# Godotcoffee/AlignGraph2

Measured on AMD Instinct MI355X. Metric: aligned-read-bases/sec through PAGraph build+traverse, higher is better.
Workload: dtype u32

## Files before the change

### aligngraph2_amd/csrc/hip/k5_walk_aux.hip

```cpp
#include <algorithm>
#include <cmath>
#include <cstring>
#include <string>
#include <vector>

#include "pag_device.hpp"
#include "pag_travel.hpp"
#include "trav_device.hpp"
#include "trav_hook.hpp"

namespace pagdev {


__global__ void k_ranges(TravGraph G, TravContig *ctgs, uint32_t n) {
    uint32_t i = blockIdx.x * blockDim.x + threadIdx.x;
    if (i >= n) return;
    auto lower = [&](uint32_t x) {
        uint64_t lo = 0, hi = G.n_pos;
        while (lo < hi) {
            uint64_t mid = (lo + hi) >> 1;
            if ((uint32_t)(G.upos[mid] >> 32) < x) lo = mid + 1;
            else hi = mid;
        }
        return (uint32_t)lo;
// ... 176 lines not shown
    const uint32_t j = blockIdx.y;
    if (j >= n) return;
    const TravPackDesc D = descs[j];
    uint32_t *o = out + D.off;
    const uint32_t lane = lane_id();
    const uint64_t n_arrays = D.seq_x ? 5 : 3;
    uint32_t *agg = o + n_arrays * D.len;
    uint32_t *xagg = agg + ((D.len + 63) / 64) * 5;
    for (uint64_t i0 = (uint64_t)blockIdx.x * blockDim.x + (threadIdx.x & ~63u); i0 < D.len; i0 += (uint64_t)gridDim.x * blockDim.x) {
        const uint64_t i = i0 + lane;
        const bool valid = i < D.len;
        uint32_t v = 0, st = 0, c = 0, xl = 0, xh = 0;
        if (valid) {
            v = D.seq_v[i];
            st = D.seq_s[i];
            c = (uint32_t)(G.upos[v] >> 32);
            o[i] = v;
            o[D.len + i] = st;
            o[2 * D.len + i] = c;
            if (D.seq_x) {
                const uint64_t x = D.seq_x[i];
                xl = (uint32_t)x;
                xh = (uint32_t)(x >> 32);
                o[3 * D.len + i] = xl;
                o[4 * D.len + i] = xh;
            }
        }
        const uint32_t mx = wave_max_u32(valid ? c : 0u);
        const uint32_t m0 = wave_max_u32(valid && c == 0u ? v + 1u : 0u);
        const uint32_t lo = wave_min_u32(valid ? c : 0xFFFFFFFFu);
        const uint32_t lnz = wave_min_u32(valid && c != 0u ? c : 0xFFFFFFFFu);
        const uint32_t sum = wave_sum(valid ? st : 0u);
        const uint64_t blk = i0 >> 6;
        if (lane == 0) {
            uint32_t *a = agg + blk * 5;
            a[0] = mx;
            a[1] = m0;
            a[2] = lo;
            a[3] = lnz;
            a[4] = sum;
        }
        if (D.seq_x) {
            const bool bd = valid && (xh >> 31) != 0u;
            const uint32_t elow = wave_min_u32(bd ? (xh & 0x7FFFFFFFu) : 0xFFFFFFFFu);
            const uint32_t xm0 = wave_min_u32(bd ? xl : 0xFFFFFFFFu);
            if (lane == 0) {
                xagg[blk * 2] = elow;
                xagg[blk * 2 + 1] = xm0;
            }
        }
    }
}

__global__ void k_gather_pc(TravGraph G, const uint32_t *__restrict__ seq_v, uint64_t len, uint32_t *__restrict__ out) {
    for (uint64_t i = (uint64_t)blockIdx.x * blockDim.x + threadIdx.x; i < len; i += (uint64_t)gridDim.x * blockDim.x)
        out[i] = (uint32_t)(G.upos[seq_v[i]] >> 32);
}

__global__ void k_commit(const uint32_t *__restrict__ seq_v, uint64_t len, uint32_t in_lo, uint32_t in_hi, uint32_t *gbits,
                         uint32_t *gset, uint32_t gmask) {
    for (uint64_t i = (uint64_t)blockIdx.x * blockDim.x + threadIdx.x; i < len; i += (uint64_t)gridDim.x * blockDim.x) {
        uint32_t u = seq_v[i];
        if (u >= in_lo && u < in_hi) atomicOr(&gbits[(u - in_lo) >> 5], 1u << ((u - in_lo) & 31u));
        else hs_insert(gset, gmask, u);
    }
}

__global__ void k_gather_path(TravGraph G, const uint32_t *__restrict__ seq_v, const uint32_t *__restrict__ seq_s, uint64_t len,
                              pag_path_node *__restrict__ out) {
    for (uint64_t i = (uint64_t)blockIdx.x * blockDim.x + threadIdx.x; i < len; i += (uint64_t)gridDim.x * blockDim.x) {
        uint32_t v = G.uold[seq_v[i]];
        uint64_t p = G.vpos[v];
        pag_path_node o;
        o.code = G.ncode[G.vnode[v]];
        o.ctg = (uint32_t)(p >> 32);
        o.ref = (uint32_t)p;
        o.cnt = G.vcnt[v];
        o.reserved = 0;
        o.step = (int32_t)seq_s[i];
        o.vid = v;
        out[i] = o;
    }
}

__global__ void k_gather_vertices(TravGraph G, const uint32_t *__restrict__ vids, uint32_t n, pag_path_node *__restrict__ out) {
    uint32_t i = blockIdx.x * blockDim.x + threadIdx.x;
    if (i >= n) return;
    uint32_t v = vids[i];
    uint64_t p = G.vpos[v];
    pag_path_node o;
    o.code = G.ncode[G.vnode[v]];
    o.ctg = (uint32_t)(p >> 32);
    o.ref = (uint32_t)p;
    o.cnt = G.vcnt[v];
    o.reserved = 0;
    o.step = 0;
    o.vid = v;
    out[i] = o;
}

void trav_launch_seed_first(TravGraph G, const TravContig *ctgs, uint32_t n, uint64_t dev, uint32_t *out, uint32_t stride,
                            hipStream_t s) {
    if (n) k_seed_first<<<dim3(n), dim3(64), 0, s>>>(G, ctgs, n, dev, out, stride);
}
void trav_launch_seed_window(TravGraph G, const TravContig *ctgs, const TravSeedReq *reqs, uint32_t n, uint64_t dev,
                             uint32_t *out, uint32_t stride, hipStream_t s) {
    if (n) k_seed_window<<<dim3(n, TRAV_SEED_PARTS), dim3(64), 0, s>>>(G, ctgs, reqs, n, dev, out, stride);
}
void trav_launch_checkpoints(TravGraph G, const TravContig *ctgs, const TravSeedReq *reqs, uint32_t n, uint64_t dev, uint32_t *out,
                             hipStream_t s) {
    if (n) k_checkpoints<<<dim3(n), dim3(64), 0, s>>>(G, ctgs, reqs, n, dev, out);
}
void trav_launch_id_bounds(TravGraph G, const uint32_t *coords, uint32_t n, uint32_t *out, hipStream_t s) {
    if (n) k_id_bounds<<<dim3((n + 63) / 64), dim3(64), 0, s>>>(G, coords, n, out);
}
void trav_launch_pack_paths(TravGraph G, const TravPackDesc *descs, uint32_t n, uint64_t max_len, uint32_t *out, hipStream_t s) {
    if (!n) return;
    const unsigned gx = (unsigned)std::min<uint64_t>(std::max<uint64_t>((max_len + 255) / 256, 1), 64);
    k_pack_paths<<<dim3(gx, n), dim3(256), 0, s>>>(G, descs, n, out);
}
void trav_launch_gather_pc(TravGraph G, const uint32_t *seq_v, uint64_t len, uint32_t *out, hipStream_t s) {
    if (len) k_gather_pc<<<dim3(grid_for(len)), dim3(256), 0, s>>>(G, seq_v, len, out);
}
void trav_launch_commit(const uint32_t *seq_v, uint64_t len, uint32_t in_lo, uint32_t in_hi, uint32_t *gbits, uint32_t *gset,
                        uint32_t gmask, hipStream_t s) {
    if (len) k_commit<<<dim3(grid_for(len)), dim3(256), 0, s>>>(seq_v, len, in_lo, in_hi, gbits, gset, gmask);
}
void trav_launch_ranges(TravGraph G, TravContig *ctgs, uint32_t n, hipStream_t s) {
    if (n) k_ranges<<<dim3((n + 63) / 64), dim3(64), 0, s>>>(G, ctgs, n);
}

__global__ void k_clear_ranges(const TravClear *__restrict__ ranges) {
    const TravClear c = ranges[blockIdx.y];
    uint8_t *p = as_global((uint8_t *)c.p);
    const uint64_t head = (16u - ((uintptr_t)p & 15u)) & 15u, h = head < c.bytes ? head : c.bytes;
    const uint64_t n16 = (c.bytes - h) >> 4, tail = (c.bytes - h) & 15u;
    uint4 *q = (uint4 *)(p + h);
    const uint4 w = make_uint4(c.word, c.word, c.word, c.word);
    for (uint64_t i = (uint64_t)blockIdx.x * blockDim.x + threadIdx.x; i < n16; i += (uint64_t)gridDim.x * blockDim.x) q[i] = w;
    if (blockIdx.x == 0) {
        auto byte_at = [&](const uint8_t *a) { return (uint8_t)(c.word >> (8u * (uint32_t)((uintptr_t)a & 3u))); };
        if (threadIdx.x < h) p[threadIdx.x] = byte_at(p + threadIdx.x);
        if (threadIdx.x < tail) p[h + (n16 << 4) + threadIdx.x] = byte_at(p + h + (n16 << 4) + threadIdx.x);
    }
}
int trav_clear_ranges(const TravClear *ranges_dev, size_t n, hipStream_t s) {
    for (size_t at = 0; at < n; at += 32768) {
        const uint32_t m = (uint32_t)std::min<size_t>(32768, n - at);
        k_clear_ranges<<<dim3(32, m), dim3(256), 0, s>>>(ranges_dev + at);
    }
    PAG_HIP_TRY(hipGetLastError());
    return PAG_OK;
}
void trav_launch_gather_path(TravGraph G, const uint32_t *seq_v, const uint32_t *seq_s, uint64_t len, pag_path_node *out,
                             hipStream_t s, unsigned max_blocks) {
    const unsigned grid = max_blocks ? std::min(grid_for(len), max_blocks) : grid_for(len);
    if (len) k_gather_path<<<dim3(grid), dim3(256), 0, s>>>(G, seq_v, seq_s, len, out);
}
__global__ void __launch_bounds__(256) k_concat_parts(const TravConcatPart *__restrict__ parts, uint32_t *__restrict__ out_v,
                                                      uint32_t *__restrict__ out_s, uint32_t first_step) {
    const TravConcatPart P = parts[blockIdx.y];
    for (uint64_t x = (uint64_t)blockIdx.x * blockDim.x + threadIdx.x; x < P.n; x += (uint64_t)gridDim.x * blockDim.x) {
        out_v[P.start + x] = P.v[x];
        out_s[P.start + x] = (P.start + x == 0) ? first_step : P.s[x];
    }
}
void trav_launch_concat_parts(const TravConcatPart *parts, uint32_t n_parts, uint32_t *out_v, uint32_t *out_s, uint32_t first_step,
                              hipStream_t s) {
    for (uint32_t at = 0; at < n_parts; at += 32768) {
        const uint32_t n = std::min<uint32_t>(32768, n_parts - at);
        k_concat_parts<<<dim3(16, n), dim3(256), 0, s>>>(parts + at, out_v, out_s, first_step);
    }
}
void trav_launch_gather_vertices(TravGraph G, const uint32_t *vids, uint32_t n, pag_path_node *out, hipStream_t s) {
    if (n) k_gather_vertices<<<dim3((n + 255) / 256), dim3(256), 0, s>>>(G, vids, n, out);
}

}

using namespace pagdev;

namespace {
int hook_contigs(const pag_debug_trav_contig *ctgs, uint32_t n_ctgs, uint64_t n_graph_nodes, const uint32_t *nodes, uint64_t n_node_words,
                 uint64_t n_gbits, const uint32_t *gset, uint64_t n_gset, const uint32_t *d_nodes, uint32_t *d_gbits, uint32_t *d_gset,
                 std::vector<TravContig> &tc) {
    if (n_ctgs && !ctgs) return PAG_EINVAL;
    for (uint64_t i = 0; i < n_node_words; ++i)
        if (nodes[i] != PAG_NONE && nodes[i] >= n_graph_nodes) return PAG_EINVAL;
    tc.assign(n_ctgs, TravContig{});
    for (uint32_t i = 0; i < n_ctgs; ++i) {
        const pag_debug_trav_contig &m = ctgs[i];
        TravContig &t = tc[i];
        if (m.n_kmers && (m.nodes_off > n_node_words || m.n_kmers > n_node_words - m.nodes_off)) return PAG_EINVAL;
        if (m.g_hi < m.g_lo || m.in_hi < m.in_lo) return PAG_EINVAL;
        t.nodes = d_nodes + m.nodes_off;
        t.n_kmers = m.n_kmers;
        t.ctg_left = m.ctg_left;
        t.ctg_right = m.ctg_right;
        t.in_lo = m.in_lo;
        t.in_hi = m.in_hi;
        t.g_lo = m.g_lo;
        t.g_hi = m.g_hi;
        t.gmask = m.gmask;
        if (m.gbits_off != PAG_DEBUG_NULL) {
            const uint64_t words = ((uint64_t)(m.g_hi - m.g_lo) + 31) / 32;
            if (m.gbits_off > n_gbits || words > n_gbits - m.gbits_off) return PAG_EINVAL;
            t.gbits = d_gbits + m.gbits_off;
        }
        if (m.gset_off != PAG_DEBUG_NULL) {
            const uint64_t cap = (uint64_t)m.gmask + 1;
            if ((cap & (cap - 1)) || m.gset_off > n_gset || cap > n_gset - m.gset_off) return PAG_EINVAL;
            bool free_slot = false;
            for (uint64_t x = 0; x < cap && !free_slot; ++x) free_slot = gset[m.gset_off + x] == HS_EMPTY;
            if (!free_slot) return PAG_EINVAL;
            t.gset = d_gset + m.gset_off;
        }
    }
    return PAG_OK;
}
}

extern "C" int pag_debug_trav_bounds(const pag_debug_trav_graph *g, const uint32_t *coords, uint32_t n, uint32_t *out, pag_debug_trav_contig *ctgs,
                                     uint32_t n_ctgs, int device) {
    if (!g || (g->n_pos && !g->upos) || (n && (!coords || !out)) || (n_ctgs && !ctgs)) return PAG_EINVAL;
    HookDev D;
    TravGraph G;
    int rc;
    if ((rc = D.open(device)) || (rc = hook_upload_graph(D, g, &G))) return rc;
    uint32_t *d_coords = nullptr, *d_out = nullptr;
    TravContig *d_tc = nullptr;
    std::vector<TravContig> tc(n_ctgs, TravContig{});
    for (uint32_t i = 0; i < n_ctgs; ++i) {
        tc[i].ctg_left = ctgs[i].ctg_left;
        tc[i].ctg_right = ctgs[i].ctg_right;
        tc[i].in_lo = ctgs[i].in_lo;
        tc[i].in_hi = ctgs[i].in_hi;
        tc[i].g_lo = ctgs[i].g_lo;
        tc[i].g_hi = ctgs[i].g_hi;
    }
    if ((rc = D.up(coords, n, &d_coords)) || (rc = D.up((const uint32_t *)out, n, &d_out)) || (rc = D.up((const TravContig *)tc.data(), n_ctgs, &d_tc))) return rc;
    trav_launch_id_bounds(G, d_coords, n, d_out, D.s);
    trav_launch_ranges(G, d_tc, n_ctgs, D.s);
    if ((rc = D.down(out, d_out, n)) || (rc = D.down(tc.data(), d_tc, n_ctgs)) || (rc = D.finish())) return rc;
    for (uint32_t i = 0; i < n_ctgs; ++i) {
        ctgs[i].in_lo = tc[i].in_lo;
        ctgs[i].in_hi = tc[i].in_hi;
        ctgs[i].g_lo = tc[i].g_lo;
        ctgs[i].g_hi = tc[i].g_hi;
    }
    return PAG_OK;
}

extern "C" int pag_debug_trav_seeds(const pag_debug_trav_graph *g, int which, const pag_debug_trav_contig *ctgs, uint32_t n_ctgs, const uint32_t *nodes,
                                    uint64_t n_node_words, const uint32_t *gbits, uint64_t n_gbits, const uint32_t *gset, uint64_t n_gset,
                                    const uint64_t *reqs, uint32_t n_req, uint64_t dev, uint32_t *out, uint64_t out_words, uint32_t stride, int device) {
    if (!g || which < 0 || which > 2 || !g->npos_off || (g->n_pos && (!g->vpos || !g->newid || !g->vcnt)) || (n_node_words && !nodes) ||
        (n_gbits && !gbits) || (n_gset && !gset) || !out)
        return PAG_EINVAL;
    const uint64_t need = which == 0 ? (uint64_t)n_ctgs * stride : which == 1 ? (uint64_t)n_req * TRAV_SEED_PARTS * stride : 3ull * n_req;
    if ((which != 2 && stride < 2) || out_words < need || (which != 0 && n_req && !reqs)) return PAG_EINVAL;
    std::vector<TravSeedReq> rq(which == 0 ? 0 : n_req);
    for (size_t r = 0; r < rq.size(); ++r) {
        if (reqs[4 * r] >= n_ctgs) return PAG_EINVAL;
        rq[r].ctg = (uint32_t)reqs[4 * r];
        rq[r].pad = 0;
        rq[r].left = reqs[4 * r + 1];
        rq[r].right = reqs[4 * r + 2];
        rq[r].pos = reqs[4 * r + 3];
    }
    HookDev D;
    TravGraph G;
    int rc;
    if ((rc = D.open(device)) || (rc = hook_upload_graph(D, g, &G))) return rc;
    uint32_t *d_nodes = nullptr, *d_gbits = nullptr, *d_gset = nullptr, *d_out = nullptr;
    TravContig *d_tc = nullptr;
    TravSeedReq *d_rq = nullptr;
    if ((rc = D.up(nodes, n_node_words, &d_nodes)) || (rc = D.up(gbits, n_gbits, &d_gbits)) || (rc = D.up(gset, n_gset, &d_gset)) ||
        (rc = D.up((const uint32_t *)out, out_words, &d_out)))
        return rc;
    std::vector<TravContig> tc;
    if ((rc = hook_contigs(ctgs, n_ctgs, g->n_nodes, nodes, n_node_words, n_gbits, gset, n_gset, d_nodes, d_gbits, d_gset, tc))) return rc;
    if ((rc = D.up((const TravContig *)tc.data(), n_ctgs, &d_tc)) || (rc = D.up((const TravSeedReq *)rq.data(), rq.size(), &d_rq))) return rc;
    if (which == 0) trav_launch_seed_first(G, d_tc, n_ctgs, dev, d_out, stride, D.s);
    else if (which == 1) trav_launch_seed_window(G, d_tc, d_rq, n_req, dev, d_out, stride, D.s);
    else trav_launch_checkpoints(G, d_tc, d_rq, n_req, dev, d_out, D.s);
    if ((rc = D.down(out, d_out, out_words))) return rc;
    return D.finish();
}

extern "C" int pag_debug_pack_paths(const pag_debug_trav_graph *g, const uint32_t *seq_v, const uint32_t *seq_s, const uint64_t *seq_x, uint64_t n_seq,
                                    const uint64_t *descs, uint32_t n, uint64_t max_len, uint32_t *out, uint64_t out_words, int device) {
    if (!g || !g->upos || (n_seq && (!seq_v || !seq_s)) || (n && !descs) || !out || n > 65535u) return PAG_EINVAL;
    for (uint64_t i = 0; i < n_seq; ++i)
        if (seq_v[i] >= g->n_pos) return PAG_EINVAL;
    for (uint32_t j = 0; j < n; ++j) {
        const uint64_t from = descs[4 * j], len = descs[4 * j + 1], off = descs[4 * j + 2];
        const bool leap = descs[4 * j + 3] != 0;
        if (from > n_seq || len > n_seq - from || len > max_len || (leap && !seq_x)) return PAG_EINVAL;
        if (off > out_words || trav_pack_words(len, leap) > out_words - off) return PAG_EINVAL;
    }
    HookDev D;
    TravGraph G;
    int rc;
    if ((rc = D.open(device)) || (rc = hook_upload_graph(D, g, &G))) return rc;
    uint32_t *d_v = nullptr, *d_s = nullptr, *d_out = nullptr;
    uint64_t *d_x = nullptr;
// ... 114 lines not shown
```

### aligngraph2_amd/csrc/hip/pag_api.hip

```cpp
#include <algorithm>
#include <cstdlib>
#include <cstring>
#include <new>
#include <string>
#include <thread>
#include <chrono>
#include <vector>

#include "pag_device.hpp"
#include "pagraph_debug.h"

using namespace pagdev;

#include "pag_graph_impl.hpp"
#include "walker_grid.hpp"

namespace {

template <typename T>
int stage(const T *src, uint64_t n, bool on_device, DevBuf &own, const T **out, hipStream_t s) {
    if (on_device) {
        *out = src;
        return PAG_OK;
    }
// ... 62 lines not shown
    if (threadIdx.x < 16) h[threadIdx.x] = 0;
    __syncthreads();
    for (uint64_t i = (uint64_t)blockIdx.x * blockDim.x + threadIdx.x; i < n; i += (uint64_t)gridDim.x * blockDim.x)
        atomicAdd(&h[((key[i] >> shift) & 7u) * 2u + (i < n1 ? 0u : 1u)], 1u);
    __syncthreads();
    if (threadIdx.x < 16 && h[threadIdx.x]) atomicAdd(&out[threadIdx.x], (unsigned long long)h[threadIdx.x]);
}

__global__ void edge_counts(const uint32_t *__restrict__ samples, uint64_t n, uint32_t *__restrict__ out) {
    uint64_t i = (uint64_t)blockIdx.x * blockDim.x + threadIdx.x;
    if (i < n) out[i] = samples[i] ? samples[i] - 1u : 0u;
}

}

extern "C" {

const char *pag_last_error(void) { return last_error(); }

int pag_device_available(void) { return pick_device(0) == PAG_OK ? 1 : 0; }

namespace {
__global__ void k_warm(uint32_t *p) {
    if (p) *p = 1u;
}
}
int pag_device_warm(int device_ordinal) {
    int rc = pick_device(device_ordinal);
    if (rc != PAG_OK) return rc;
    uint32_t *p = nullptr;
    if (hipMalloc((void **)&p, 256) != hipSuccess) return PAG_ENOMEM;
    k_warm<<<dim3(1), dim3(64)>>>(p);
    hipError_t e = hipDeviceSynchronize();
    hipFree(p);
    if (e != hipSuccess) {
        set_error("pag_device_warm: %s", hipGetErrorString(e));
        return PAG_EFAULT;
    }
    return PAG_OK;
}

pag_graph *pag_create(const uint64_t *codes, uint64_t n_codes, uint32_t k, int device_ordinal, int *err) {
    int rc = PAG_OK;
    pag_graph *g = nullptr;
    if (k == 0 || k > 16 || (!codes && n_codes)) {
        set_error("pag_create: k must be in 1..16 (got %u)", k);
        rc = PAG_EINVAL;
    }
    if (rc == PAG_OK) rc = pick_device(device_ordinal);
    if (rc == PAG_OK) {
        g = new (std::nothrow) pag_graph();
        if (!g) rc = PAG_ENOMEM;
    }
    if (rc == PAG_OK) {
        g->device = device_ordinal;
        g->k = k;
        const uint64_t space = 1ull << (2 * k);
        const uint64_t words = (space + 31) / 32;
        std::vector<uint32_t> bits((size_t)words, 0u);
        std::vector<uint64_t> outside;
        {
            unsigned T = std::max(1u, std::min(16u, std::thread::hardware_concurrency()));
            if (n_codes < (1u << 20)) T = 1;
            std::vector<std::vector<uint64_t>> out_t(T);
            auto work = [&](unsigned t) {
                const uint64_t lo = n_codes * t / T, hi = n_codes * (t + 1) / T;
                for (uint64_t i = lo; i < hi; ++i) {
                    const uint64_t c = codes[i];
                    if (c < space) __atomic_fetch_or(&bits[(size_t)(c >> 5)], 1u << (c & 31), __ATOMIC_RELAXED);
                    else out_t[t].push_back(c);
                }
            };
            std::vector<std::thread> pool;
            for (unsigned t = 1; t < T; ++t) pool.emplace_back(work, t);
            work(0);
            for (auto &th : pool) th.join();
            for (auto &v : out_t) outside.insert(outside.end(), v.begin(), v.end());
        }
        std::sort(outside.begin(), outside.end());
        outside.erase(std::unique(outside.begin(), outside.end()), outside.end());
        uint64_t in_space = 0;
        for (uint32_t wbits : bits) in_space += (uint64_t)__builtin_popcount(wbits);
        g->n_solid = in_space + outside.size();
        g->all_solid = in_space == space;
        hipError_t e = hipStreamCreate(&g->stream);
        if (e == hipSuccess) e = hipMalloc((void **)&g->solid_bits, (size_t)words * 4 + 64);
        if (e == hipSuccess) e = hipMemcpy(g->solid_bits, bits.data(), (size_t)words * 4, hipMemcpyHostToDevice);
        if (e != hipSuccess) {
            set_error("pag_create: %s", hipGetErrorString(e));
            rc = PAG_EFAULT;
        }
    }
    if (rc != PAG_OK && g) {
        pag_destroy(g);
        g = nullptr;
    }
    if (err) *err = rc;
    return g;
}

pag_graph *pag_create_from_bitmap(const uint32_t *bits, uint64_t n_solid, uint32_t k, int bits_on_device,
                                  int device_ordinal, int *err) {
    int rc = PAG_OK;
    pag_graph *g = nullptr;
    if (k == 0 || k > 16 || !bits) {
        set_error("pag_create_from_bitmap: k must be in 1..16 and bits non-null");
        rc = PAG_EINVAL;
    }
    if (rc == PAG_OK) rc = pick_device(device_ordinal);
    if (rc == PAG_OK) {
        g = new (std::nothrow) pag_graph();
        if (!g) rc = PAG_ENOMEM;
    }
    if (rc == PAG_OK) {
        g->device = device_ordinal;
        g->k = k;
        g->n_solid = n_solid;
        const uint64_t space = 1ull << (2 * k);
        const uint64_t words = (space + 31) / 32;
        g->all_solid = n_solid == space;
        hipError_t e = hipStreamCreate(&g->stream);
        if (e == hipSuccess) e = hipMalloc((void **)&g->solid_bits, (size_t)words * 4 + 64);
        if (e == hipSuccess)
            e = hipMemcpy(g->solid_bits, bits, (size_t)words * 4, bits_on_device ? hipMemcpyDeviceToDevice : hipMemcpyHostToDevice);
        if (e != hipSuccess) {
            set_error("pag_create_from_bitmap: %s", hipGetErrorString(e));
            rc = PAG_EFAULT;
        }
    }
    if (rc != PAG_OK && g) {
        pag_destroy(g);
        g = nullptr;
    }
    if (err) *err = rc;
    return g;
}

void pag_destroy(pag_graph *g) {
    if (!g) return;
    hipSetDevice(g->device);
    free_graph_results(g);
    for (auto &sl : g->pool)
        if (sl.p) hipFree(sl.p);
    for (auto &sl : g->cpool)
        if (sl.p) hipFree(sl.p);
    for (void *q : g->deferred) hipFree(q);
    if (g->wq_host) hipHostFree(g->wq_host);
    if (g->path_store) hipHostFree(g->path_store);
    if (g->deliver_stream) hipStreamDestroy(g->deliver_stream);
    if (g->pin_host) hipHostFree(g->pin_host);
    for (void *q : g->fetch_chunks) hipHostFree(q);
    g->fetch_chunks.clear();
    g->fetch_chunk_bytes.clear();
    if (g->walk_arena) hipFree(g->walk_arena);
    if (g->dump_tables) hipFree(g->dump_tables);
    if (g->dump_scratch) hipFree(g->dump_scratch);
    if (g->wq_next) hipFree(g->wq_next);
    for (hipStream_t ws : g->walk_streams) hipStreamDestroy(ws);
    if (g->solid_bits) hipFree(g->solid_bits);
    if (g->stream) hipStreamDestroy(g->stream);
    delete g;
}

uint64_t pag_solid_count(const pag_graph *g) { return g ? g->n_solid : 0; }

int pag_reset(pag_graph *g) {
    if (!g) return PAG_EINVAL;
    hipSetDevice(g->device);
    free_graph_results(g);
    g->stats = pag_build_stats{};
    return PAG_OK;
}

}

namespace {

struct Extracted {
    uint64_t T = 0, E = 0, T1 = 0, E1 = 0;
};

struct StreamBufs {
    DevBuf tk0, tv0, tk1, tv1, ek0, ev0, ek1, ev1, sorttmp;
    explicit StreamBufs(pag_graph *g)
        : tk0(g, ps::TK0), tv0(g, ps::TV0), tk1(g, ps::TK1), tv1(g, ps::TV1), ek0(g, ps::EK0), ev0(g, ps::EV0), ek1(g, ps::EK1), ev1(g, ps::EV1),
          sorttmp(g, ps::SORT_TMP) {}
    int alloc(uint64_t T, uint64_t E) {
        int rc;
        if ((rc = tk0.alloc((T + 1) * 4)) || (rc = tv0.alloc((T + 1) * 8)) || (rc = ek0.alloc((E + 1) * 4)) || (rc = ev0.alloc((E + 1) * 8)) ||
            (rc = tk1.alloc((T + 1) * 4)) || (rc = tv1.alloc((T + 1) * 12)) || (rc = ek1.alloc((E + 1) * 4)) || (rc = ev1.alloc((E + 1) * 12)))
            return rc;
        return sorttmp.alloc(sort_tmp_bytes(std::max(T, E)));
    }
};

int extract_stage(pag_graph *g, const pag_build_input *in, uint64_t emit_lo, uint64_t emit_hi, Extracted *out, hipEvent_t ev_begin,
                  hipEvent_t ev_end) {
    hipStream_t s = g->stream;
    const bool dev = in->on_device != 0;
    const uint32_t n_reads_all = (uint32_t)in->reads.n_seqs;
    const uint32_t n_reads = (uint32_t)(emit_hi - emit_lo);
    const uint64_t n_jobs = 4ull * n_reads;
    int rc;
    if (ev_begin) PAG_HIP_TRY(hipEventRecord(ev_begin, s));

    DevBuf b_roff(g, ps::IN_ROFF), b_rlen(g, ps::IN_RLEN), b_packed(g, ps::IN_PACKED), b_order(g, ps::IN_ORDER), b_aln1(g, ps::IN_ALN1), b_q1(g, ps::IN_Q1),
        b_d1(g, ps::IN_D1), b_aln2(g, ps::IN_ALN2), b_q2(g, ps::IN_Q2), b_d2(g, ps::IN_D2), b_ctg(g, ps::IN_CTG), b_eoff(g, ps::IN_EOFF), b_ent(g, ps::IN_ENT),
        b_ref(g, ps::IN_REF);
    const uint64_t *d_roff;
    const uint32_t *d_rlen, *d_order, *d_d1, *d_d2, *d_eoff, *d_ent;
    const uint8_t *d_packed;
    const pag_aln *d_aln1, *d_aln2;
    const uint64_t *d_q1, *d_q2;
    const pag_ctg *d_ctg;
    const pag_ref *d_ref;
    if ((rc = stage(in->reads.byte_off, n_reads_all, dev, b_roff, &d_roff, s))) return rc;
    if ((rc = stage(in->reads.len, n_reads_all, dev, b_rlen, &d_rlen, s))) return rc;
    if ((rc = stage(in->reads.packed, in->reads.packed_bytes, dev, b_packed, &d_packed, s))) return rc;
    if ((rc = stage(in->emit_order, n_reads_all, dev, b_order, &d_order, s))) return rc;
    if ((rc = stage(in->read_to_ctg.aln, in->read_to_ctg.n_aln, dev, b_aln1, &d_aln1, s))) return rc;
    if ((rc = stage(in->read_to_ctg.query_off, (uint64_t)n_reads_all + 1, dev, b_q1, &d_q1, s))) return rc;
    if ((rc = stage(in->read_to_ctg.diff, in->read_to_ctg.n_diff_words, dev, b_d1, &d_d1, s))) return rc;
    if ((rc = stage(in->read_to_ref.aln, in->read_to_ref.n_aln, dev, b_aln2, &d_aln2, s))) return rc;
    if ((rc = stage(in->read_to_ref.query_off, (uint64_t)n_reads_all + 1, dev, b_q2, &d_q2, s))) return rc;
    if ((rc = stage(in->read_to_ref.diff, in->read_to_ref.n_diff_words, dev, b_d2, &d_d2, s))) return rc;
    if ((rc = stage(in->ctgs, in->n_ctgs, dev, b_ctg, &d_ctg, s))) return rc;
    if ((rc = stage(in->ctg_ent_off, in->n_ctg_ent_off, dev, b_eoff, &d_eoff, s))) return rc;
    if ((rc = stage(in->ctg_ent, in->n_ctg_ent, dev, b_ent, &d_ent, s))) return rc;
    if ((rc = stage(in->refs, in->n_refs, dev, b_ref, &d_ref, s))) return rc;
    d_order += emit_lo;

    std::vector<pag_ref> refs_host((size_t)in->n_refs);
    if (in->n_refs) {
        if (dev) PAG_HIP_TRY(hipMemcpy(refs_host.data(), in->refs, in->n_refs * sizeof(pag_ref), hipMemcpyDeviceToHost));
        else std::memcpy(refs_host.data(), in->refs, in->n_refs * sizeof(pag_ref));
    }

    const uint64_t n_aln1 = in->read_to_ctg.n_aln, n_aln2 = in->read_to_ref.n_aln;
    DevBuf b_covok(g, ps::COV_OK), b_covtmp(g, ps::COV_TMP);
    if ((rc = b_covok.alloc(n_aln2 + 16))) return rc;
    size_t cov_bytes = cov_tmp_bytes(refs_host.data(), in->n_refs);
    if ((rc = b_covtmp.alloc(cov_bytes))) return rc;
    if ((rc = launch_cov_filter(d_aln2, n_aln2, d_ref, refs_host.data(), in->n_refs, in->cov_filter,
                                b_covok.as<uint8_t>(), b_covtmp.p, cov_bytes, s)))
        return rc;

    DevBuf b_cc(g, ps::CI_CC), b_cio1(g, ps::CI_OFF1), b_cio2(g, ps::CI_OFF2), b_ci1(g, ps::CI_1), b_ci2(g, ps::CI_2), b_scan(g, ps::X_SCAN), b_tot(g, ps::X_TOT);
    uint64_t n_alnmax = std::max(n_aln1, n_aln2);
    if ((rc = b_cc.alloc((n_alnmax + 1) * 4))) return rc;
    if ((rc = b_cio1.alloc((n_aln1 + 1) * 8))) return rc;
    if ((rc = b_cio2.alloc((n_aln2 + 1) * 8))) return rc;
    if ((rc = b_scan.alloc(scan_tmp_bytes(std::max<uint64_t>(n_alnmax, n_jobs) + 1)))) return rc;
    if ((rc = b_tot.alloc(64))) return rc;
    uint64_t *d_tot = b_tot.as<uint64_t>();
    uint64_t n_ci[2] = {0, 0};
    for (int pass = 0; pass < 2; ++pass) {
        const pag_aln *al = pass == 0 ? d_aln1 : d_aln2;
        uint64_t na = pass == 0 ? n_aln1 : n_aln2;
        DevBuf &off = pass == 0 ? b_cio1 : b_cio2;
        if (na) {
            chunk_counts<<<dim3((unsigned)((na + 255) / 256)), dim3(256), 0, s>>>(al, na, b_cc.as<uint32_t>());
            if ((rc = scan_u32_to_u64(b_cc.as<uint32_t>(), off.as<uint64_t>(), na, d_tot + pass, b_scan.p, s))) return rc;
            PAG_HIP_TRY(hipMemcpyAsync(&n_ci[pass], d_tot + pass, 8, hipMemcpyDeviceToHost, s));
        }
    }
    PAG_HIP_TRY(hipStreamSynchronize(s));
    for (int pass = 0; pass < 2; ++pass) {
        const pag_aln *al = pass == 0 ? d_aln1 : d_aln2;
        uint64_t na = pass == 0 ? n_aln1 : n_aln2;
        DevBuf &off = pass == 0 ? b_cio1 : b_cio2;
        DevBuf &ci = pass == 0 ? b_ci1 : b_ci2;
        if ((rc = ci.alloc((n_ci[pass] + 1) * sizeof(uint2)))) return rc;
        if ((rc = launch_colidx(al, na, pass == 0 ? d_d1 : d_d2, off.as<uint64_t>(), ci.as<uint2>(), s))) return rc;
    }

    DevBuf b_js(g, ps::K1_JS), b_jt(g, ps::K1_JT), b_je(g, ps::K1_JE), b_toff(g, ps::K1_TOFF), b_eoff2(g, ps::K1_EOFF);
    if ((rc = b_js.alloc((n_jobs + 1) * 4))) return rc;
    if ((rc = b_jt.alloc((n_jobs + 1) * 4))) return rc;
    if ((rc = b_je.alloc((n_jobs + 1) * 4))) return rc;
    if ((rc = b_toff.alloc((n_jobs + 1) * 8))) return rc;
    if ((rc = b_eoff2.alloc((n_jobs + 1) * 8))) return rc;
    DevBuf b_smask(g, ps::SOLID_MASK);
    if (!g->all_solid) {
        if ((rc = b_smask.alloc((in->reads.packed_bytes / 4 + 16) * 2 * sizeof(uint16_t) * solid_mask_slices()))) return rc;
    }
    ExtractArgs xa[2];
    for (int pass = 0; pass < 2; ++pass) {
        ExtractArgs &a = xa[pass];
        a = ExtractArgs{};
        a.read_off = d_roff;
        a.read_len = d_rlen;
        a.packed = d_packed;
        a.emit_order = d_order;
        a.n_reads = n_reads;
        a.aln = pass == 0 ? d_aln1 : d_aln2;
        a.query_off = pass == 0 ? d_q1 : d_q2;
        a.diff = pass == 0 ? d_d1 : d_d2;
        a.colidx_off = (pass == 0 ? b_cio1 : b_cio2).as<uint64_t>();
        a.colidx = (pass == 0 ? b_ci1 : b_ci2).as<uint2>();
        a.cov_ok = pass == 0 ? nullptr : b_covok.as<uint8_t>();
        a.pass = pass;
        a.topk = pass == 0 ? in->topk_ctg : in->topk_ref;
        a.ctgs = d_ctg;
        a.ctg_ent_off = d_eoff;
        a.ctg_ent = d_ent;
        a.refs = d_ref;
        a.solid_bits = g->solid_bits;
// ... 104 lines not shown
        return rc;
    PAG_HIP_TRY(hipEventRecord(ev[2], s));
    EdgeOut eo{b_eseg.as<uint32_t>(), ctr_dev + 4};
    if ((rc = launch_edges(ek->as<uint32_t>(), evb->as<uint64_t>(), e_scratch, E, eo, b_long.as<uint64_t>(),
                           b_lcnt.as<uint32_t>(), s, wide)))
        return rc;
    uint64_t ctr[8] = {0, 0, 0, 0, 0, 0, 0, 0};
    PAG_HIP_TRY(hipMemcpyAsync(ctr, b_ctr.p, 64, hipMemcpyDeviceToHost, s));
    PAG_HIP_TRY(hipEventRecord(ev[3], s));
    PAG_HIP_TRY(hipStreamSynchronize(s));

    pag_build_stats st{};
    const uint64_t T2 = T - T1, E2 = E - E1;
    const uint64_t L_ctg = ctr[0], L_all = ctr[1], U_all = ctr[4], U_1 = ctr[5];
    st.n_tuples[0] = T1;
    st.n_tuples[1] = T2;
    st.n_edges[0] = E1;
    st.n_edges[1] = E2;
    st.merge_edge[0] = E1 - U_1;
    st.total_pos[0] = T1;
    st.merge_pos[0] = T1 - L_ctg;
    st.merge_edge[1] = U_1 + E2 - U_all;
    st.total_pos[1] = L_ctg + T2;
    st.merge_pos[1] = L_ctg + T2 - L_all;
    st.n_nodes = ctr[2];
    st.n_pos = L_all;
    st.n_uniq_edges = U_all;
    float ms = 0.f;
    hipEventElapsedTime(&ms, ev[0], ev[1]);
    st.ms_sort = ms;
    hipEventElapsedTime(&ms, ev[1], ev[2]);
    st.ms_cluster = ms;
    hipEventElapsedTime(&ms, ev[2], ev[3]);
    st.ms_edges = ms;
    st.ms_sort_kernel = ms_scatter_t;
    st.sort_records = T;
    (void)passes;
    (void)ms_scatter_e;

    g->n_t = T;
    g->n_e = E;
    g->tkey = tk->as<uint32_t>();
    g->tval = tv->as<uint64_t>();
    g->tseg = b_tseg.as<uint32_t>();
    g->tcnt = b_tcnt.as<uint16_t>();
    g->ekey = ek->as<uint32_t>();
    g->eval = evb->as<uint64_t>();
    g->eseg = b_eseg.as<uint32_t>();
    g->stats = st;
    *st_out = st;
    return PAG_OK;
}

struct EventSet {
    hipEvent_t e[6] = {nullptr, nullptr, nullptr, nullptr, nullptr, nullptr};
    int create() {
        for (auto &x : e) PAG_HIP_TRY(hipEventCreate(&x));
        return PAG_OK;
    }
    ~EventSet() {
        for (auto x : e)
            if (x) hipEventDestroy(x);
    }
};

void keep_debug_streams(pag_graph *g, uint64_t T, uint64_t E) {
    const char *keep = std::getenv("PAG_DEBUG_KEEP_STREAMS");
    g->dbg_tkey.clear();
    g->dbg_tval.clear();
    g->dbg_ekey.clear();
    g->dbg_eval.clear();
    if (!(keep && keep[0] == '1')) return;
    g->dbg_tkey.resize((size_t)T);
    g->dbg_tval.resize((size_t)T);
    g->dbg_ekey.resize((size_t)E);
    g->dbg_eval.resize((size_t)E);
    hipStreamSynchronize(g->stream);
    const StreamPtrs x = streams_at(g, 1, 1);
    if (T) hipMemcpy(g->dbg_tkey.data(), x.tkey, T * 4, hipMemcpyDeviceToHost);
    if (T) hipMemcpy(g->dbg_tval.data(), x.tval, T * 8, hipMemcpyDeviceToHost);
    if (E) hipMemcpy(g->dbg_ekey.data(), x.ekey, E * 4, hipMemcpyDeviceToHost);
    if (E) hipMemcpy(g->dbg_eval.data(), x.eval, E * 8, hipMemcpyDeviceToHost);
}

int check_process_args(const pag_graph *g, const pag_build_input *in) {
    if (!g || !in) return PAG_EINVAL;
    if (in->outer_sample < 1 || in->outer_sample > 7) {
        set_error("outer_sample must be 1..7");
        return PAG_EINVAL;
    }
    if (in->reads.n_seqs >= 0x3FFFFFFFull) {
        set_error("too many reads for one launch");
        return PAG_EINVAL;
    }
    return PAG_OK;
}

}

extern "C" {

int pag_process(pag_graph *g, const pag_build_input *in, pag_build_stats *stats) {
    int rc = check_process_args(g, in);
    if (rc != PAG_OK) return rc;
    const bool timing = env_timing();
    const auto wall0 = std::chrono::steady_clock::now();
    auto wall_ms = [&]() { return std::chrono::duration<double, std::milli>(std::chrono::steady_clock::now() - wall0).count(); };
    PAG_HIP_TRY(hipSetDevice(g->device));
    free_graph_results(g);
    EventSet ev;
    if ((rc = ev.create())) return rc;
    Extracted x;
    if ((rc = extract_stage(g, in, 0, in->reads.n_seqs, &x, ev.e[0], ev.e[1]))) return rc;
    keep_debug_streams(g, x.T, x.E);
    pag_build_stats st{};
    if ((rc = build_stage(g, in->eps, x, &st, ev.e + 2))) return rc;
    float ms = 0.f;
    hipEventElapsedTime(&ms, ev.e[0], ev.e[1]);
    st.ms_extract = ms;
    hipEventElapsedTime(&ms, ev.e[0], ev.e[5]);
    st.ms_total = ms;
    if (timing) fprintf(stderr, "[timing] pag_process wall %.1f ms (device %.1f ms)\n", wall_ms(), (double)ms);
    g->stats = st;
    if (stats) *stats = st;
    return PAG_OK;
}

extern "C" int pag_reserve_walk_arena(pag_graph *g, uint64_t contig_bases) {
    if (!g) return PAG_EINVAL;
    PAG_HIP_TRY(hipSetDevice(g->device));
    size_t want = (size_t)contig_bases * 1200 + (64u << 20);
    size_t free_b = 0, total_b = 0;
    const size_t sharers = env_device_sharers();
    if (hipMemGetInfo(&free_b, &total_b) == hipSuccess) want = std::min(want, (free_b + g->walk_arena_cap) * 2 / 5 / sharers);
    {
        const size_t FETCH_CHUNK = 64u << 20;
        size_t have = 0;
        for (size_t b : g->fetch_chunk_bytes) have += b;
        const size_t per_base = 14 + (env_int("PAGRAPH_DEVICE_DUMPS", 0) == 1 ? 22 : 0) + (env_int("PAGRAPH_DEVICE_SEQS", 0) == 1 ? 2 : 0);
        const size_t want_pinned = std::min<size_t>((size_t)contig_bases * per_base, (size_t)4 << 30);
        while (have < want_pinned) {
            void *q = nullptr;
            if (hipHostMalloc(&q, FETCH_CHUNK, hipHostMallocDefault) != hipSuccess) {
                (void)hipGetLastError();
                break;
            }
            g->fetch_chunks.push_back(q);
            g->fetch_chunk_bytes.push_back(FETCH_CHUNK);
            have += FETCH_CHUNK;
        }
    }
    pagdev::WalkerGrid::prepare_streams(g, 4);
    if (g->walk_arena_cap >= want) return PAG_OK;
    if (g->walk_arena) hipFree(g->walk_arena);
    g->walk_arena = nullptr;
    g->walk_arena_cap = 0;
    if (hipMalloc(&g->walk_arena, want) != hipSuccess) {
        g->walk_arena = nullptr;
        (void)hipGetLastError();
        return PAG_OK;
    }
    g->walk_arena_cap = want;
    return PAG_OK;
}

static int log2_shards(uint32_t n) { return n == 1 ? 0 : n == 2 ? 1 : n == 4 ? 2 : n == 8 ? 3 : -1; }

int pag_shard_extract(pag_graph *g, const pag_build_input *in, uint32_t shard, uint32_t n_shards, uint64_t *counts) {
    int rc = check_process_args(g, in);
    if (rc != PAG_OK) return rc;
    if (log2_shards(n_shards) < 0 || shard >= n_shards) {
        set_error("pag_shard_extract: n_shards must be 1, 2, 4 or 8 (got %u) and shard below it", n_shards);
        return PAG_EINVAL;
    }
    const uint64_t n = in->reads.n_seqs;
    return pag_shard_extract_range(g, in, n * shard / n_shards, n * (shard + 1ull) / n_shards, n_shards, counts);
}

int pag_shard_extract_range(pag_graph *g, const pag_build_input *in, uint64_t lo, uint64_t hi, uint32_t n_shards, uint64_t *counts) {
    int rc = check_process_args(g, in);
    if (rc != PAG_OK) return rc;
    const int lg = log2_shards(n_shards);
    if (lg < 0 || !counts || 2 * (int)g->k < lg || lo > hi || hi > in->reads.n_seqs) {
        set_error("pag_shard_extract_range: n_shards must be 1, 2, 4 or 8 (got %u), the reads [%llu, %llu) of %llu", n_shards, (unsigned long long)lo,
                  (unsigned long long)hi, (unsigned long long)in->reads.n_seqs);
        return PAG_EINVAL;
    }
    PAG_HIP_TRY(hipSetDevice(g->device));
    free_graph_results(g);
    hipStream_t s = g->stream;
    Extracted x;
    if ((rc = extract_stage(g, in, lo, hi, &x, nullptr, nullptr))) return rc;
    keep_debug_streams(g, x.T, x.E);
    g->shard_x[0] = x.T;
    g->shard_x[1] = x.E;
    g->shard_in0[0] = g->shard_in0[1] = 1;
    for (uint32_t i = 0; i < 4 * n_shards; ++i) counts[i] = 0;
    if (n_shards == 1) {
        counts[0] = x.T1;
        counts[1] = x.T - x.T1;
        counts[2] = x.E1;
        counts[3] = x.E - x.E1;
        return PAG_OK;
    }
    const int shift = 2 * (int)g->k - lg;
    StreamBufs sb(g);
    DevBuf b_ctr(g, ps::CTR);
    if ((rc = sb.alloc(x.T, x.E)) || (rc = b_ctr.alloc(512))) return rc;
    unsigned long long *ctr = b_ctr.as<unsigned long long>();
    PAG_HIP_TRY(hipMemsetAsync(ctr, 0, 256, s));
    if (x.T) owner_counts<<<dim3(1024), dim3(256), 0, s>>>(sb.tk0.as<uint32_t>(), x.T, x.T1, shift, ctr);
    if (x.E) owner_counts<<<dim3(1024), dim3(256), 0, s>>>(sb.ek0.as<uint32_t>(), x.E, x.E1, shift, ctr + 16);
    int t_in0 = 1, e_in0 = 1;
    if ((rc = sort_pairs(sb.tk0.as<uint32_t>(), sb.tv0.as<uint64_t>(), sb.tk1.as<uint32_t>(), sb.tv1.as<uint64_t>(), x.T, lg, sb.sorttmp.p, &t_in0, s, nullptr,
                         nullptr, shift)))
        return rc;
    if ((rc = sort_pairs(sb.ek0.as<uint32_t>(), sb.ev0.as<uint64_t>(), sb.ek1.as<uint32_t>(), sb.ev1.as<uint64_t>(), x.E, lg, sb.sorttmp.p, &e_in0, s, nullptr,
                         nullptr, shift)))
        return rc;
    unsigned long long h[32];
    PAG_HIP_TRY(hipMemcpyAsync(h, ctr, 256, hipMemcpyDeviceToHost, s));
    PAG_HIP_TRY(hipStreamSynchronize(s));
    for (uint32_t o = 0; o < n_shards; ++o) {
        counts[4 * o + 0] = h[2 * o];
        counts[4 * o + 1] = h[2 * o + 1];
        counts[4 * o + 2] = h[16 + 2 * o];
        counts[4 * o + 3] = h[16 + 2 * o + 1];
    }
    g->shard_in0[0] = t_in0;
    g->shard_in0[1] = e_in0;
    return PAG_OK;
}

int pag_shard_extract_for(pag_graph *g, const pag_build_input *in, uint64_t lo, uint64_t hi, uint32_t n_shards, uint32_t owner, uint32_t *tkey,
                          uint64_t *tval, uint64_t t_cap, uint64_t t_at1, uint64_t t_at2, uint32_t *ekey, uint64_t *eval, uint64_t e_cap,
                          uint64_t e_at1, uint64_t e_at2, uint64_t *counts) {
    int rc = check_process_args(g, in);
    if (rc != PAG_OK) return rc;
    const int lg = log2_shards(n_shards);
    if (lg < 1 || owner >= n_shards || !counts || 2 * (int)g->k < lg || lo > hi || hi > in->reads.n_seqs) {
        set_error("pag_shard_extract_for: n_shards must be 2, 4 or 8 (got %u) and the owner below it (got %u), the reads [%llu, %llu) of %llu", n_shards,
                  owner, (unsigned long long)lo, (unsigned long long)hi, (unsigned long long)in->reads.n_seqs);
        return PAG_EINVAL;
    }
    PAG_HIP_TRY(hipSetDevice(g->device));
    free_graph_results(g);
    hipStream_t s = g->stream;
    Extracted x;
    if ((rc = extract_stage(g, in, lo, hi, &x, nullptr, nullptr))) return rc;
    g->shard_x[0] = x.T;
    g->shard_x[1] = x.E;
    g->shard_in0[0] = g->shard_in0[1] = 1;
    for (int q = 0; q < 4; ++q) counts[q] = 0;
    const uint32_t shift = (uint32_t)(2 * (int)g->k - lg);
    DevBuf b_tmp(g, ps::PICK_TMP);
    if ((rc = b_tmp.alloc(owner_pick_tmp_bytes(std::max(x.T, x.E))))) return rc;
    const StreamPtrs st = streams_at(g, 1, 1);
    if ((rc = owner_pick(st.tkey, st.tval, x.T, x.T1, shift, owner, tkey, tval, t_cap, t_at1, t_at2, counts, b_tmp.p, s))) return rc;
    if ((rc = owner_pick(st.ekey, st.eval, x.E, x.E1, shift, owner, ekey, eval, e_cap, e_at1, e_at2, counts + 2, b_tmp.p, s))) return rc;
    PAG_HIP_TRY(hipStreamSynchronize(s));
    return PAG_OK;
}

int pag_shard_take(pag_graph *g, uint32_t *tkey, uint64_t *tval, uint32_t *ekey, uint64_t *eval) {
    if (!g) return PAG_EINVAL;
    PAG_HIP_TRY(hipSetDevice(g->device));
    hipStream_t s = g->stream;
    const uint64_t T = g->shard_x[0], E = g->shard_x[1];
    const StreamPtrs x = streams_at(g, g->shard_in0[0], g->shard_in0[1]);
    if (T) PAG_HIP_TRY(hipMemcpyAsync(tkey, x.tkey, T * 4, hipMemcpyDeviceToDevice, s));
    if (T) PAG_HIP_TRY(hipMemcpyAsync(tval, x.tval, T * 8, hipMemcpyDeviceToDevice, s));
    if (E) PAG_HIP_TRY(hipMemcpyAsync(ekey, x.ekey, E * 4, hipMemcpyDeviceToDevice, s));
    if (E) PAG_HIP_TRY(hipMemcpyAsync(eval, x.eval, E * 8, hipMemcpyDeviceToDevice, s));
    PAG_HIP_TRY(hipStreamSynchronize(s));
    return PAG_OK;
}

int pag_shard_take_part(pag_graph *g, uint64_t t_off, uint64_t t_n, uint32_t *tkey, uint64_t *tval, uint64_t e_off, uint64_t e_n, uint32_t *ekey,
                        uint64_t *eval) {
    if (!g) return PAG_EINVAL;
    const uint64_t T = g->shard_x[0], E = g->shard_x[1];
    if (t_off > T || t_n > T - t_off || e_off > E || e_n > E - e_off || (t_n && (!tkey || !tval)) || (e_n && (!ekey || !eval))) {
        set_error("pag_shard_take_part: [%llu, +%llu) of %llu tuples, [%llu, +%llu) of %llu edges", (unsigned long long)t_off, (unsigned long long)t_n,
                  (unsigned long long)T, (unsigned long long)e_off, (unsigned long long)e_n, (unsigned long long)E);
        return PAG_EINVAL;
    }
    PAG_HIP_TRY(hipSetDevice(g->device));
    hipStream_t s = g->stream;
    const StreamPtrs x = streams_at(g, g->shard_in0[0], g->shard_in0[1]);
    if (t_n) PAG_HIP_TRY(hipMemcpyAsync(tkey, x.tkey + t_off, t_n * 4, hipMemcpyDeviceToDevice, s));
    if (t_n) PAG_HIP_TRY(hipMemcpyAsync(tval, x.tval + t_off, t_n * 8, hipMemcpyDeviceToDevice, s));
    if (e_n) PAG_HIP_TRY(hipMemcpyAsync(ekey, x.ekey + e_off, e_n * 4, hipMemcpyDeviceToDevice, s));
    if (e_n) PAG_HIP_TRY(hipMemcpyAsync(eval, x.eval + e_off, e_n * 8, hipMemcpyDeviceToDevice, s));
    PAG_HIP_TRY(hipStreamSynchronize(s));
    return PAG_OK;
}

int pag_shard_build(pag_graph *g, const uint32_t *tkey, const uint64_t *tval, uint64_t n_t, uint64_t t1, const uint32_t *ekey,
                    const uint64_t *eval, uint64_t n_e, uint64_t e1, uint32_t eps, pag_build_stats *stats) {
    if (!g || t1 > n_t || e1 > n_e || (n_t && (!tkey || !tval)) || (n_e && (!ekey || !eval))) return PAG_EINVAL;
    PAG_HIP_TRY(hipSetDevice(g->device));
    free_graph_results(g);
    hipStream_t s = g->stream;
    int rc;
    DevBuf b_tk0(g, ps::TK0), b_tv0(g, ps::TV0), b_ek0(g, ps::EK0), b_ev0(g, ps::EV0);
    if ((rc = b_tk0.alloc((n_t + 1) * 4)) || (rc = b_tv0.alloc((n_t + 1) * 8)) || (rc = b_ek0.alloc((n_e + 1) * 4)) || (rc = b_ev0.alloc((n_e + 1) * 8))) return rc;
    if (n_t) PAG_HIP_TRY(hipMemcpyAsync(b_tk0.p, tkey, n_t * 4, hipMemcpyDeviceToDevice, s));
    if (n_t) PAG_HIP_TRY(hipMemcpyAsync(b_tv0.p, tval, n_t * 8, hipMemcpyDeviceToDevice, s));
    if (n_e) PAG_HIP_TRY(hipMemcpyAsync(b_ek0.p, ekey, n_e * 4, hipMemcpyDeviceToDevice, s));
    if (n_e) PAG_HIP_TRY(hipMemcpyAsync(b_ev0.p, eval, n_e * 8, hipMemcpyDeviceToDevice, s));
    EventSet ev;
    if ((rc = ev.create())) return rc;
    Extracted x;
    x.T = n_t;
    x.E = n_e;
// ... 227 lines not shown
```

### aligngraph2_amd/csrc/hip/pag_graph_impl.hpp

```cpp
#pragma once
#include <algorithm>
#include <chrono>
#include <vector>

#include "pag_device.hpp"
#include "pag_travel.hpp"
#include "pool_slots.hpp"

struct pag_graph {
    int device = 0;
    hipStream_t stream = nullptr;
    uint32_t k = 0;
    uint64_t n_solid = 0;
    int all_solid = 0;
    uint32_t *solid_bits = nullptr;
    uint64_t n_t = 0, n_e = 0;
    uint32_t *tkey = nullptr;
    uint64_t *tval = nullptr;
    uint32_t *tseg = nullptr;
    uint16_t *tcnt = nullptr;
    uint32_t *ekey = nullptr;
    uint64_t *eval = nullptr;
    uint32_t *eseg = nullptr;
    pag_build_stats stats{};
    uint64_t shard_x[2] = {0, 0};
    int shard_in0[2] = {1, 1};
    struct SerialRun {
        bool valid = false;
        uint32_t n = 0;
        std::vector<uint64_t> counts;
        pag_build_stats total{};
    } serial;
    struct Slot {
        void *p = nullptr;
        size_t cap = 0;
    };
    Slot pool[pagdev::ps::COUNT];
    double alloc_ms = 0;
    uint64_t alloc_bytes = 0, alloc_calls = 0;
    std::vector<Slot> cpool;
    bool defer_free = false;
    std::vector<void *> deferred;
    void *wq_host = nullptr;
    size_t wq_bytes = 0;
    uint32_t *wq_next = nullptr;
    std::vector<hipStream_t> walk_streams;
    pagdev::TravGraph tg{};
    bool tg_ready = false;
    uint64_t tg_dev = 0;
    double tg_err = 0;
    pag_path_node *path_store = nullptr;
    size_t path_cap = 0;
    std::vector<uint64_t> path_off, path_len;
    hipStream_t deliver_stream = nullptr;
    std::vector<const pag_path_node *> path_ptr;
    std::vector<uint8_t> path_valid;
    std::vector<const char *> text_ptr;
    std::vector<uint64_t> text_len;
    std::vector<const char *> seq_ptr;
    std::vector<uint64_t> seq_len;
    const pag_seqs *seq_refs = nullptr;
    void *dump_tables = nullptr, *dump_scratch = nullptr;
    size_t dump_tables_cap = 0, dump_scratch_cap = 0;
    void *walk_arena = nullptr;
    size_t walk_arena_cap = 0, walk_arena_used = 0;
    std::vector<void *> fetch_chunks;
    std::vector<size_t> fetch_chunk_bytes;
    bool regional = false;
    std::vector<uint32_t> region_ref_iv;
    std::vector<uint8_t> region_ref_open;
    bool view_pruned = false, view_off = false;
    std::vector<int32_t> view_orient;
    uint64_t view_counts[3] = {0, 0, 0};
    uint64_t view_fallbacks = 0;
    double succ_per_vertex = 3.0;
    uint64_t n_zero_ctg = 0;
    void *pin_host = nullptr;
    size_t pin_bytes = 0;
    std::vector<uint32_t> dbg_tkey, dbg_ekey;
    std::vector<uint64_t> dbg_tval, dbg_eval;
};


namespace pagdev {

struct DevBuf {
    pag_graph *g = nullptr;
    pag_graph::Slot *sl = nullptr;
    void *p = nullptr;
    DevBuf() = default;
    DevBuf(pag_graph *gg, ps::Id s) : g(gg), sl(&gg->pool[s]) {}
    DevBuf(pag_graph *gg, pag_graph::Slot *slot) : g(gg), sl(slot) {}
    int alloc(size_t bytes) {
        if (bytes == 0) bytes = 16;
        if (sl->cap < bytes) {
            const auto t0 = std::chrono::steady_clock::now();
            if (sl->p) {
                if (g->defer_free) g->deferred.push_back(sl->p);
                else hipFree(sl->p);
            }
            sl->p = nullptr;
            sl->cap = 0;
            size_t want = bytes + std::min<size_t>(bytes / 8, (size_t)512 << 20) + 256;
            hipError_t e = hipMalloc(&sl->p, want);
            g->alloc_ms += std::chrono::duration<double, std::milli>(std::chrono::steady_clock::now() - t0).count();
            g->alloc_bytes += want;
            g->alloc_calls += 1;
            if (e != hipSuccess) {
                sl->p = nullptr;
                pagdev::set_error("hipMalloc(%zu) failed: %s", want, hipGetErrorString(e));
                return PAG_ENOMEM;
            }
            sl->cap = want;
        }
        p = sl->p;
        return PAG_OK;
    }
    template <typename T>
    T *as() const {
        return (T *)p;
    }
};


struct StreamPtrs {
    const uint32_t *tkey;
    const uint64_t *tval;
    const uint32_t *ekey;
    const uint64_t *eval;
};
inline StreamPtrs streams_at(const pag_graph *g, int t_in0, int e_in0) {
    return StreamPtrs{(const uint32_t *)g->pool[t_in0 ? ps::TK0 : ps::TK1].p, (const uint64_t *)g->pool[t_in0 ? ps::TV0 : ps::TV1].p,
                      (const uint32_t *)g->pool[e_in0 ? ps::EK0 : ps::EK1].p, (const uint64_t *)g->pool[e_in0 ? ps::EV0 : ps::EV1].p};
}

int shard_count_range(pag_graph *g, const pag_build_input *in, uint64_t lo, uint64_t hi, uint32_t n_shards, uint64_t *counts);

struct GraphArrays {
    void *p[ps::GRAPH_ARRS];
};
template <typename G>
GraphArrays arrays_of(const G &x) {
    return GraphArrays{{(void *)x.tkey, (void *)x.tval, (void *)x.tseg, (void *)x.tcnt, (void *)x.ekey, (void *)x.eval, (void *)x.eseg}};
}
template <typename G>
void point_at(G &x, const GraphArrays &a) {
    x.tkey = (decltype(x.tkey))a.p[ps::G_TKEY];
    x.tval = (decltype(x.tval))a.p[ps::G_TVAL];
    x.tseg = (decltype(x.tseg))a.p[ps::G_TSEG];
    x.tcnt = (decltype(x.tcnt))a.p[ps::G_TCNT];
    x.ekey = (decltype(x.ekey))a.p[ps::G_EKEY];
    x.eval = (decltype(x.eval))a.p[ps::G_EVAL];
    x.eseg = (decltype(x.eseg))a.p[ps::G_ESEG];
}
inline GraphArrays arrays_in(const pag_graph *g, ps::Id base) {
    GraphArrays a;
    for (int i = 0; i < ps::GRAPH_ARRS; ++i) a.p[i] = g->pool[ps::family(base, i)].p;
    return a;
}

}
```

### aligngraph2_amd/csrc/hip/pag_travel.hpp

```cpp
#pragma once
#include <hip/hip_runtime.h>
#include <stdint.h>

#include <vector>

#include "pagraph_hip.h"

namespace pagdev {

constexpr int TRAV_PROBE_GROUPS = 8;

struct TravGraph {
    uint64_t n_nodes, n_pos, n_edges;
    uint32_t *ncode;
    uint32_t *npos_off;
    uint32_t *nedge_off;
    uint64_t *vpos;
    uint16_t *vcnt;
    uint32_t *vnode;
    uint32_t *eto;
    uint32_t *estep;
    uint64_t *bitmap;
    uint32_t *rank;
    uint32_t *uold;
// ... 7 lines not shown
    uint32_t n_zero;
    const uint32_t *inc_iv;
    const uint8_t *inc_open;
    uint32_t inc_n, inc_margin;
};
constexpr uint32_t GRADE_POISON = 7u, GRADE_POISON_IF_LEAP = 6u;

struct alignas(16) SuccRec {
    uint32_t tgt;
    uint32_t pc;
    uint32_t meta;
    uint32_t toff;
};

struct TravContig {
    const uint32_t *nodes;
    uint32_t n_kmers;
    uint32_t ctg_left, ctg_right;
    uint32_t rev_left, rev_right;
    uint64_t split_size;
    double leap_min;
    const uint64_t *starts;
    const uint64_t *sizes;
    uint32_t n_ctgs;
    uint32_t in_lo, in_hi;
    uint32_t g_lo, g_hi;
    uint32_t *gbits;
    uint32_t *gset;
    uint32_t gmask;
    uint32_t gwin_lo, gwin_hi;
};

struct TravJob {
    uint32_t ctg;
    uint32_t start;
    uint64_t has_size;
    uint32_t *seq_v, *seq_s;
    uint64_t seq_cap;
    uint32_t *arena_v, *arena_s;
    uint64_t arena_cap;
    uint32_t *stamp;
    uint32_t stamp_stride;
    uint32_t *tbits;
    uint64_t *tset;
    uint32_t tmask;
    uint64_t *pset;
    uint32_t pmask;
    uint32_t exact;
    uint32_t mode;
    uint32_t stop_pc;
    uint64_t init_len;
    uint32_t win_low;
    uint32_t pad0;
    uint64_t *seq_x;
};
enum { TRAV_MODE_SPEC = 1, TRAV_MODE_RESUME = 2, TRAV_MODE_LEAP = 4, TRAV_MODE_UNTIL_LEAP = 8,
       TRAV_MODE_CANCELLED = 16 };

struct TravJobOut {
    uint64_t seq_len, seq_size;
    uint64_t n_classify, n_probe, n_records;
    uint32_t last_ctg;
    int overflow;
    uint64_t n_fill, n_out, n_main;
    uint32_t stopped;
    uint32_t max_back;
    uint32_t max_chosen;
    uint32_t wd_below_max;
    uint64_t max_probe;
    uint32_t wd_forced_min;
    uint32_t poison;
    uint64_t t_begin, t_end;
#ifdef PAG_WALK_PROF
    uint64_t prof_t[14];
    uint32_t prof_c[14];
#endif
};

struct TravPosted {
    TravJob J;
    TravContig C;
};
constexpr int TRAV_RINGS = 3;
struct TravQueue {
    uint32_t posted[TRAV_RINGS];
    uint32_t exit;
    uint32_t started, exited;
};

struct TravPackDesc {
    const uint32_t *seq_v, *seq_s;
    uint64_t len;
    uint64_t off;
    const uint64_t *seq_x;
};

inline uint64_t trav_pack_words(uint64_t len, bool leap) { return (leap ? 5 : 3) * len + ((len + 63) / 64) * (leap ? 7 : 5); }

constexpr uint32_t TRAV_SEED_PARTS = 16;

struct TravSeedReq {
    uint32_t ctg;
    uint32_t pad;
    uint64_t left, right, pos;
};

struct TravView {
    const uint32_t *civ, *riv;
    uint32_t n_civ, n_riv;
};
int trav_compact(const uint32_t *tkey, const uint64_t *tval, const uint32_t *tseg, const uint16_t *tcnt, uint64_t T,
                 const uint32_t *ekey, const uint64_t *eval, const uint32_t *eseg, uint64_t E, uint32_t k, uint64_t n_nodes,
                 uint64_t n_pos, uint64_t n_edges, TravGraph G, void *tmp, size_t tmp_bytes, hipStream_t s, const TravView *view = nullptr,
                 uint64_t *counts_out = nullptr);
int trav_zone_bands(const uint64_t *tval, uint64_t T, const uint32_t *zones_dev, uint32_t n_z, uint32_t *lo_dev, uint32_t *hi_dev, hipStream_t s);
size_t trav_compact_tmp_bytes(uint64_t T, uint64_t E, uint32_t k, uint64_t n_nodes);
struct TravCtgNodesJob {
    uint64_t byte_off;
    uint64_t out_off;
    uint32_t len;
    int32_t forward;
};
void trav_launch_ctg_nodes(const uint8_t *packed, const TravCtgNodesJob *jobs, uint32_t n_jobs, uint32_t max_len, uint32_t k, TravGraph G, uint32_t *out,
                           hipStream_t s);
void trav_launch_seed_first(TravGraph G, const TravContig *ctgs, uint32_t n, uint64_t dev, uint32_t *out, uint32_t stride,
                            hipStream_t s);
void trav_launch_seed_window(TravGraph G, const TravContig *ctgs, const TravSeedReq *reqs, uint32_t n, uint64_t dev,
                             uint32_t *out, uint32_t stride, hipStream_t s);
void trav_launch_checkpoints(TravGraph G, const TravContig *ctgs, const TravSeedReq *reqs, uint32_t n, uint64_t dev, uint32_t *out,
                             hipStream_t s);
void trav_launch_id_bounds(TravGraph G, const uint32_t *coords, uint32_t n, uint32_t *out, hipStream_t s);
void trav_launch_pack_paths(TravGraph G, const TravPackDesc *descs, uint32_t n, uint64_t max_len, uint32_t *out, hipStream_t s);
void trav_launch_gather_pc(TravGraph G, const uint32_t *seq_v, uint64_t len, uint32_t *out, hipStream_t s);
void trav_launch_walk(TravGraph G, const TravContig *ctgs, const TravJob *jobs, TravJobOut *outs, uint32_t n, uint32_t k,
                      hipStream_t s);
int trav_walk_waves_per_cu();
void trav_launch_walk_persistent(TravGraph G, const TravPosted *jobs, TravJobOut *outs, uint32_t *done, TravQueue *q,
                                 uint32_t *next, uint32_t cap, uint32_t k, uint32_t n_waves, uint64_t idle_ticks, hipStream_t s);
void trav_launch_commit(const uint32_t *seq_v, uint64_t len, uint32_t in_lo, uint32_t in_hi, uint32_t *gbits, uint32_t *gset,
                        uint32_t gmask, hipStream_t s);
void trav_launch_ranges(TravGraph G, TravContig *ctgs, uint32_t n, hipStream_t s);
int trav_mark_incomplete(TravGraph &G, uint32_t n_zero, const uint32_t *iv_host, const uint8_t *open_host, uint32_t n_iv, uint32_t dev, double err,
                         uint32_t *bits, void *tmp, hipStream_t s);
size_t trav_mark_incomplete_tmp_bytes(uint32_t n_iv);

int trav_order(TravGraph G, uint32_t *key, uint64_t *val, uint32_t *key2, uint64_t *val2, void *sort_tmp, uint64_t *n_zero, int ctg_bits,
               int ref_bits, hipStream_t s);
struct TravClear {
    void *p;
    uint64_t bytes;
    uint32_t word, pad;
};
int trav_clear_ranges(const TravClear *ranges_dev, size_t n, hipStream_t s);
int trav_successors_of(TravGraph G, uint32_t code, uint64_t pos, void *recs, uint64_t cap, unsigned long long *out, hipStream_t s);
constexpr uint32_t EMIT_CHUNK_SLOTS = 2048u, EMIT_GRID_THREADS = 2048u, EMIT_GRID_WAVES = 1024u;
constexpr uint64_t EMIT_SLACK_SLOTS = (uint64_t)(EMIT_GRID_THREADS + EMIT_GRID_WAVES) * 4u * EMIT_CHUNK_SLOTS;
int trav_succ_emit(TravGraph G, uint32_t dev, double err, uint32_t *key0, uint64_t *val0, uint32_t *key1, uint64_t *val1, uint64_t cap, void *sort_tmp,
                   unsigned long long *counters, uint32_t *heavy_list, uint32_t heavy_limit, uint64_t *n_slots, uint64_t *n_rec, uint64_t *n_heavy,
                   const uint32_t **sorted_key, const uint64_t **sorted_val, hipStream_t s);
int trav_succ_finish(TravGraph G, const uint32_t *key, const uint64_t *val, uint64_t n_rec, hipStream_t s);
void trav_launch_gather_path(TravGraph G, const uint32_t *seq_v, const uint32_t *seq_s, uint64_t len, pag_path_node *out,
                             hipStream_t s, unsigned max_blocks = 0);
void trav_launch_gather_vertices(TravGraph G, const uint32_t *vids, uint32_t n, pag_path_node *out, hipStream_t s);
struct TravConcatPart {
    const uint32_t *v, *s;
    uint64_t start, n;
};
void trav_launch_concat_parts(const TravConcatPart *parts, uint32_t n_parts, uint32_t *out_v, uint32_t *out_s, uint32_t first_step,
                              hipStream_t s);

size_t text_scratch_bytes(uint64_t n);
constexpr uint32_t DUMP_LDS_STARTS = 5632u, DUMP_MAX_SEQS = 99999999u;
struct DumpTables {
    const uint32_t *cstart, *csize, *rstart, *rsize;
    uint32_t nc, nr, in_lds;
};
#ifdef __HIPCC__
template <typename Starts>
__device__ __forceinline__ void single_to_dual(Starts starts, const uint32_t *__restrict__ sizes, uint32_t n, uint32_t single, int32_t *idx, int64_t *off) {
    if (single == 0u) {
        *idx = 0;
        *off = 0;
        return;
    }
    uint32_t lo = 0, hi = n ? n + 1u : 0u;
    while (lo < hi) {
        const uint32_t mid = (lo + hi) >> 1;
        if (starts[mid] <= single) lo = mid + 1u;
        else hi = mid;
    }
    const uint32_t i = lo ? lo - 1u : 0u;
    const int64_t start = n ? (int64_t)starts[i] : 0;
    const int64_t size2 = i < n ? 2 * (int64_t)sizes[i] : 0;
    int64_t o = (int64_t)single - start;
    if (o < 0 || o >= size2) {
        o -= size2;
        *idx = -(int32_t)(i + 1u);
    } else {
        *idx = (int32_t)(i + 1u);
    }
    *off = o;
}
#endif
bool dump_tables_build(const uint32_t *ctg_len, uint64_t n_ctgs, const uint32_t *ref_len, uint64_t n_refs, std::vector<uint32_t> &blob);
DumpTables dump_tables_at(const uint32_t *dev, uint64_t n_ctgs, uint64_t n_refs);
uint32_t dump_line_bound(uint32_t k, const std::vector<uint32_t> &blob, uint64_t n_ctgs, uint64_t n_refs);
int trav_launch_dump_path(TravGraph G, const uint32_t *seq_v, const uint32_t *seq_s, uint64_t len, uint32_t k, const DumpTables &T, void *scratch,
                          char *out, uint64_t cap, uint64_t *head_host, hipStream_t s, unsigned max_blocks);

struct SeqSources {
    const uint64_t *coff, *roff;
    const uint8_t *cpacked, *rpacked;
};
bool seqs_well_formed(const pag_seqs *q);
size_t seq_sources_bytes(const pag_seqs *ctgs, const pag_seqs *refs);
int seq_sources_upload(void *dev, const pag_seqs *ctgs, const pag_seqs *refs, SeqSources *out, hipStream_t s);
struct SeqParams {
    uint32_t k;
    uint64_t deviation;
    double error_rate;
};
int trav_launch_seq_path(TravGraph G, const uint32_t *seq_v, const uint32_t *seq_s, uint64_t len, const SeqParams &P, const DumpTables &T,
                         const SeqSources &S, void *scratch, char *out, uint64_t cap, uint64_t *head_host, hipStream_t s, unsigned max_blocks);

}
```

### aligngraph2_amd/csrc/hip/shard_serial.hip

```cpp
#include <algorithm>
#include <chrono>
#include <cstdio>
#include <cstring>
#include <vector>

#include "pag_graph_impl.hpp"
#include "pagraph_debug.h"
#include "serial_layout.hpp"

using namespace pagdev;

namespace {

double now_s() { return std::chrono::duration<double>(std::chrono::steady_clock::now().time_since_epoch()).count(); }

int grow_keeping(pag_graph *g, ps::Id id, size_t used, size_t need, size_t hint) {
    pag_graph::Slot &sl = g->pool[id];
    if (sl.p && sl.cap >= need) return PAG_OK;
    const auto t0 = std::chrono::steady_clock::now();
    const size_t want = std::max(need, hint) + 256;
    void *p = nullptr;
    hipError_t e = hipMalloc(&p, want);
    g->alloc_ms += std::chrono::duration<double, std::milli>(std::chrono::steady_clock::now() - t0).count();
    g->alloc_bytes += want;
    g->alloc_calls += 1;
    if (e != hipSuccess) {
        set_error("hipMalloc(%zu) failed: %s (a region of a serial-rank run)", want, hipGetErrorString(e));
        return PAG_ENOMEM;
    }
    if (used && sl.p) {
        e = hipMemcpyAsync(p, sl.p, used, hipMemcpyDeviceToDevice, g->stream);
        if (e == hipSuccess) e = hipStreamSynchronize(g->stream);
        if (e != hipSuccess) {
            hipFree(p);
            set_error("a region of a serial-rank run could not be moved: %s", hipGetErrorString(e));
            return PAG_EFAULT;
        }
    }
    if (sl.p) hipFree(sl.p);
    sl.p = p;
    sl.cap = want;
    return PAG_OK;
}

void free_slot(pag_graph::Slot &sl) {
    if (sl.p) hipFree(sl.p);
    sl.p = nullptr;
    sl.cap = 0;
}

void release_traversal(pag_graph *g) {
    hipStreamSynchronize(g->stream);
    g->tg_ready = false;
    for (int i = ps::TG_NCODE; i <= ps::WALK_SEQS; ++i) free_slot(g->pool[i]);
    if (g->walk_arena) hipFree(g->walk_arena);
    g->walk_arena = nullptr;
    g->walk_arena_cap = g->walk_arena_used = 0;
}

void release_build_keeping(pag_graph *g, const pag_build_input *in) {
    hipStreamSynchronize(g->stream);
    std::vector<const void *> keep;
    const GraphArrays held = arrays_of(*g);
    for (void *p : held.p) keep.push_back(p);
    if (in->on_device)
        for (const void *p : {(const void *)in->reads.byte_off, (const void *)in->reads.len, (const void *)in->reads.packed, (const void *)in->emit_order,
                              (const void *)in->read_to_ctg.aln, (const void *)in->read_to_ctg.query_off, (const void *)in->read_to_ctg.diff,
                              (const void *)in->read_to_ref.aln, (const void *)in->read_to_ref.query_off, (const void *)in->read_to_ref.diff,
                              (const void *)in->ctgs, (const void *)in->ctg_ent_off, (const void *)in->ctg_ent, (const void *)in->refs})
            keep.push_back(p);
    for (int i = 0; i < ps::COUNT; ++i) {
        pag_graph::Slot &sl = g->pool[i];
        if (!ps::released_after_import((ps::Id)i) || !sl.p) continue;
        const char *lo = (const char *)sl.p, *hi = lo + sl.cap;
        bool used = false;
        for (const void *p : keep) used = used || (p && (const char *)p >= lo && (const char *)p < hi);
        if (!used) free_slot(sl);
    }
}

void add_stats(pag_build_stats &st, const pag_build_stats &p) {
    for (int q = 0; q < 2; ++q) {
        st.merge_edge[q] += p.merge_edge[q];
        st.total_pos[q] += p.total_pos[q];
        st.merge_pos[q] += p.merge_pos[q];
        st.n_tuples[q] += p.n_tuples[q];
        st.n_edges[q] += p.n_edges[q];
    }
    st.n_nodes += p.n_nodes;
    st.n_pos += p.n_pos;
    st.n_uniq_edges += p.n_uniq_edges;
}

bool same_count_lines(const pag_build_stats &a, const pag_build_stats &b) {
    return !std::memcmp(a.merge_edge, b.merge_edge, sizeof a.merge_edge) && !std::memcmp(a.total_pos, b.total_pos, sizeof a.total_pos) &&
           !std::memcmp(a.merge_pos, b.merge_pos, sizeof a.merge_pos) && !std::memcmp(a.n_tuples, b.n_tuples, sizeof a.n_tuples) &&
           !std::memcmp(a.n_edges, b.n_edges, sizeof a.n_edges);
}

int serial_turn(pag_graph *g, const pag_build_input *in, const pag_region *regions, uint32_t n, uint32_t turn, pag_build_stats *total,
                pag_serial_stats *st_out, bool via_partition) {
    if (!g || !in || !regions || (n != 2 && n != 4 && n != 8) || turn >= n) {
        set_error("pag_shard_run_serial: n_ranks must be 2, 4 or 8 (got %u) and the turn below it (got %u)", n, turn);
        return PAG_EINVAL;
    }
    pag_graph::SerialRun &S = g->serial;
    if (turn != 0 && (!S.valid || S.n != n)) {
        set_error("pag_shard_run_serial: turn %u of %u without a turn 0 of the same block on this handle before it", turn, n);
        return PAG_EINVAL;
    }
    PAG_HIP_TRY(hipSetDevice(g->device));
    const uint64_t n_reads = in->reads.n_seqs;
    auto range_lo = [&](uint32_t r) { return n_reads * r / n; };
    pag_serial_stats st{};
    int rc;
    const double alloc_ms0 = g->alloc_ms;
    const uint64_t alloc_calls0 = g->alloc_calls, alloc_bytes0 = g->alloc_bytes;
    const double t_turn = now_s();
    S.valid = false;
    if (turn != 0) release_traversal(g);

    double t0 = now_s();
    if (turn == 0) {
        S.n = n;
        S.counts.assign((size_t)n * n * 4, 0);
        S.total = pag_build_stats{};
        for (uint32_t r = 0; r < n; ++r)
            if ((rc = shard_count_range(g, in, range_lo(r), range_lo(r + 1), n, S.counts.data() + (size_t)r * n * 4))) return rc;
        st.s_extract += now_s() - t0;
    }

    pag_build_stats tot{};
    uint64_t at_t = 0, at_e = 0;
    std::vector<uint64_t> full((size_t)4 * n);
    for (uint32_t o = 0; o < n; ++o) {
        t0 = now_s();
        const OwnerLayout L = owner_layout(S.counts.data(), n, o);
        DevBuf own_tk(g, ps::OWN_TK), own_tv(g, ps::OWN_TV), own_ek(g, ps::OWN_EK), own_ev(g, ps::OWN_EV);
        if ((rc = own_tk.alloc((L.n_t + 1) * 4)) || (rc = own_tv.alloc((L.n_t + 1) * 8)) || (rc = own_ek.alloc((L.n_e + 1) * 4)) ||
            (rc = own_ev.alloc((L.n_e + 1) * 8)))
            return rc;
        for (uint32_t r = 0; r < n; ++r) {
            const uint64_t *first = S.counts.data() + ((size_t)r * n + o) * 4;
            const RangeSlots at = range_slots(S.counts.data(), n, o, r);
            uint64_t c[4] = {0, 0, 0, 0};
            if (!via_partition) {
                if ((rc = pag_shard_extract_for(g, in, range_lo(r), range_lo(r + 1), n, o, own_tk.as<uint32_t>(), own_tv.as<uint64_t>(), L.n_t, at.t_at1,
                                                at.t_at2, own_ek.as<uint32_t>(), own_ev.as<uint64_t>(), L.n_e, at.e_at1, at.e_at2, c)))
                    return rc;
            } else {
                if ((rc = pag_shard_extract_range(g, in, range_lo(r), range_lo(r + 1), n, full.data()))) return rc;
                std::memcpy(c, full.data() + (size_t)o * 4, sizeof c);
                if (std::memcmp(c, first, sizeof c) == 0) {
                    const RangeSlots from = partitioned_slots(full.data(), n, o, 0 );
                    if ((rc = pag_shard_take_part(g, from.t_at1, c[0], own_tk.as<uint32_t>() + at.t_at1, own_tv.as<uint64_t>() + at.t_at1, from.e_at1, c[2],
                                                  own_ek.as<uint32_t>() + at.e_at1, own_ev.as<uint64_t>() + at.e_at1)) ||
                        (rc = pag_shard_take_part(g, from.t_at2, c[1], own_tk.as<uint32_t>() + at.t_at2, own_tv.as<uint64_t>() + at.t_at2, from.e_at2, c[3],
                                                  own_ek.as<uint32_t>() + at.e_at2, own_ev.as<uint64_t>() + at.e_at2)))
                        return rc;
                }
            }
            if (std::memcmp(c, first, sizeof c) != 0) {
                set_error("pag_shard_run_serial: read range %u is not reproducible: {%llu, %llu, %llu, %llu} records for owner %u in turn %u, "
                          "{%llu, %llu, %llu, %llu} when turn 0 counted them",
                          r, (unsigned long long)c[0], (unsigned long long)c[1], (unsigned long long)c[2], (unsigned long long)c[3], o, turn,
                          (unsigned long long)first[0], (unsigned long long)first[1], (unsigned long long)first[2], (unsigned long long)first[3]);
                return PAG_EFAULT;
            }
            st.tuples_in += c[0] + c[1];
            st.edges_in += c[2] + c[3];
        }
        const double t1 = now_s();
        pag_build_stats ost{};
        if ((rc = pag_shard_build(g, own_tk.as<uint32_t>(), own_tv.as<uint64_t>(), L.n_t, L.t1, own_ek.as<uint32_t>(), own_ev.as<uint64_t>(), L.n_e, L.e1,
                                  in->eps, &ost)))
            return rc;
        const double t2 = now_s();
        pag_shard_slice sel{};
        if ((rc = pag_shard_select(g, &regions[turn], &sel))) return rc;
        const double t3 = now_s();
        const GraphArrays from = arrays_of(sel);
        for (int a = 0; a < ps::GRAPH_ARRS; ++a) {
            const bool tup = a < ps::GRAPH_TUPLE_ARRS;
            const size_t esz = (size_t)ps::GRAPH_ESZ[a], have = (size_t)(tup ? at_t : at_e) * esz, add = (size_t)(tup ? sel.n_t : sel.n_e) * esz;
            const size_t need = have + add + esz;
            const size_t guess = (have + add) / (o + 1) * n;
            if ((rc = grow_keeping(g, ps::family(ps::IMPORT, a), have, need, guess + guess / 16))) return rc;
            if (add) PAG_HIP_TRY(hipMemcpyAsync((char *)g->pool[ps::family(ps::IMPORT, a)].p + have, from.p[a], add, hipMemcpyDeviceToDevice, g->stream));
            st.region_bytes += add;
        }
        PAG_HIP_TRY(hipStreamSynchronize(g->stream));
        at_t += sel.n_t;
        at_e += sel.n_e;
        add_stats(tot, sel.stats);
        st.s_extract += t1 - t0;
        st.s_build += t2 - t1;
        st.s_select += t3 - t2;
        st.s_import += now_s() - t3;
    }

    if (turn == 0) {
        S.total = tot;
    } else if (!same_count_lines(tot, S.total)) {
        set_error("pag_shard_run_serial: the count lines of turn %u {%llu %llu %llu | %llu %llu %llu} differ from those of turn 0 {%llu %llu %llu | %llu %llu %llu}",
                  turn, (unsigned long long)tot.merge_edge[0], (unsigned long long)tot.total_pos[0], (unsigned long long)tot.merge_pos[0],
                  (unsigned long long)tot.merge_edge[1], (unsigned long long)tot.total_pos[1], (unsigned long long)tot.merge_pos[1],
                  (unsigned long long)S.total.merge_edge[0], (unsigned long long)S.total.total_pos[0], (unsigned long long)S.total.merge_pos[0],
                  (unsigned long long)S.total.merge_edge[1], (unsigned long long)S.total.total_pos[1], (unsigned long long)S.total.merge_pos[1]);
        return PAG_EFAULT;
    }
// ... 32 lines not shown
```

### aligngraph2_amd/csrc/hip/walk_config.hpp

```cpp
#pragma once
#include <algorithm>
#include <cstdint>
#include <cstdlib>
#include <cstring>
#include <string>
#include <thread>

#include "pag_device.hpp"
namespace pagdev {

struct WalkConfig {
    bool view_whole = false;
    uint64_t view_halo = 100000;
    bool view_margin_set = false;
    uint64_t view_margin = 4000;
    uint32_t succ_heavy = 1024;
    bool timing = false;
    bool walk_debug = false;
    unsigned stitch_threads = 8;
    bool walk_trace = false;
    double idle_limit_ms = 60000.0;
    bool check_aggs = false;
    int debug_seqcap = 0;
    int debug_ring = 0;
    uint32_t debug_seed_stride = 0;
    bool debug_deliver_late = false;
    uint64_t debug_emit_cap = 0;
    bool pieces = true;
    bool leap_pieces = true;
    bool force_exact = false;
    uint64_t seg_len = 0;
    uint64_t seg_overlap = 1500;
    bool seg_safety_set = false;
    uint64_t seg_safety = 0;
    static bool u64(const char *name, uint64_t *out) {
        const char *e = std::getenv(name);
        if (!e) return false;
        *out = std::strtoull(e, nullptr, 10);
        return true;
    }
    static bool given(const char *name) {
        uint64_t x;
        return u64(name, &x);
    }
    static bool off(const char *name) {
        uint64_t x = 1;
        return u64(name, &x) && x == 0;
    }
    static WalkConfig from_env() {
        WalkConfig c;
        if (const char *e = std::getenv("PAG_TRAVEL_VIEW")) c.view_whole = std::strcmp(e, "whole") == 0;
        u64("PAG_VIEW_HALO", &c.view_halo);
        c.view_margin_set = u64("PAG_VIEW_MARGIN", &c.view_margin);
        c.timing = env_timing();
        c.walk_debug = given("PAG_WALK_DEBUG");
        c.walk_trace = given("PAG_WALK_TRACE");
        c.stitch_threads = std::min(c.stitch_threads, std::max(1u, std::thread::hardware_concurrency()));
        uint64_t x = 0;
        if (u64("PAG_WALK_IDLE_S", &x)) c.idle_limit_ms = (double)x * 1000.0;
        c.check_aggs = given("PAG_DEBUG_CHECK_AGGS");
        if (u64("PAG_DEBUG_SEQCAP", &x)) c.debug_seqcap = (int)std::max<uint64_t>(16, std::min<uint64_t>(x, 1u << 30));
        if (u64("PAG_DEBUG_RING", &x)) c.debug_ring = (int)std::max<uint64_t>(4, std::min<uint64_t>(x, 1u << 30));
        if (u64("PAG_DEBUG_SEED_STRIDE", &x) && x) {
            c.debug_seed_stride = 4;
            while (c.debug_seed_stride < std::min<uint64_t>(x, 1u << 28)) c.debug_seed_stride *= 2;
        }
        u64("PAG_DEBUG_EMIT_CAP", &c.debug_emit_cap);
        c.debug_deliver_late = given("PAG_DEBUG_DELIVER_LATE");
        c.pieces = !off("PAG_WALK_PIECES");
        c.leap_pieces = !off("PAG_LEAP_PIECES");
        c.force_exact = given("PAG_WALK_EXACT");
        u64("PAG_SEG_LEN", &c.seg_len);
        u64("PAG_SEG_OVERLAP", &c.seg_overlap);
        c.seg_safety_set = u64("PAG_SEG_SAFETY", &c.seg_safety);
        if (u64("PAG_SUCC_HEAVY", &x)) c.succ_heavy = (uint32_t)std::min<uint64_t>(1u << 24, x);
        return c;
    }
};

}
```

### aligngraph2_amd/csrc/hip/walk_session_jobs.hpp

```cpp
#pragma once

using namespace stitch;

struct WalkJobs {
    pag_graph *g;
    const pag_seqs *ctgs;
    const int32_t *orient;
    const uint32_t *ref_len;
    uint64_t n_refs;
    const pag_travel_params *prm;
    pag_travel_stats *stats;
    WalkJobs(pag_graph *g_, const pag_seqs *ctgs_, const int32_t *orient_, const uint32_t *ref_len_, uint64_t n_refs_, const pag_travel_params *prm_,
                pag_travel_stats *stats_)
        : g(g_), ctgs(ctgs_), orient(orient_), ref_len(ref_len_), n_refs(n_refs_), prm(prm_), stats(stats_), cfg(WalkConfig::from_env()),
          mapper(ctgs_->len, ctgs_->n_seqs), refMapper(ref_len_, n_refs_) {}

    hipStream_t s = nullptr;
    double t_begin = 0;
    const WalkConfig cfg;
    bool timing = false, wdebug = false, wtrace = false;
    struct TraceEv {
        double t;
        uint32_t what, ctg;
        int32_t kind, idx;
        uint64_t a, b, len, classify;
    };
    std::vector<TraceEv> trace;
    double lap_t = 0;
    std::vector<std::pair<const char *, double>> laps;
    uint32_t k = 0;
    uint64_t deviation = 0;
    double errorRate = 0, startSplit = 0;
    size_t topK = 0;
    void lap(const char *what) {
        if (!timing) return;
        const double t = now_ms();
        for (auto &l : laps)
            if (l.first == what) {
                l.second += t - lap_t;
                lap_t = t;
                return;
            }
        laps.emplace_back(what, t - lap_t);
        lap_t = t;
    }
    std::vector<void *> pinned_parked;
    void *pinned(size_t bytes) {
        if (g->pin_bytes < bytes) {
            if (g->pin_host) {
                if (g->defer_free) pinned_parked.push_back(g->pin_host);
                else hipHostFree(g->pin_host);
            }
            g->pin_host = nullptr;
            g->pin_bytes = 0;
            const size_t want = bytes + bytes / 4 + (1u << 20);
            if (hipHostMalloc(&g->pin_host, want, hipHostMallocDefault) != hipSuccess) {
                set_error("pag_travel: hipHostMalloc(%zu) failed", want);
                return nullptr;
            }
            g->pin_bytes = want;
        }
        return g->pin_host;
    }

    size_t fetch_chunk = 0, fetch_used = 0;
    static constexpr size_t FETCH_CHUNK = 64u << 20;
    void *fetch_alloc(size_t bytes) {
        bytes = (bytes + 255) & ~(size_t)255;
        for (; fetch_chunk < g->fetch_chunks.size(); ++fetch_chunk, fetch_used = 0)
            if (fetch_used + bytes <= g->fetch_chunk_bytes[fetch_chunk]) {
                void *q = (char *)g->fetch_chunks[fetch_chunk] + fetch_used;
                fetch_used += bytes;
                return q;
            }
        void *q = nullptr;
        const size_t want = std::max(FETCH_CHUNK, bytes);
        if (hipHostMalloc(&q, want, hipHostMallocDefault) != hipSuccess) {
            set_error("pag_travel: hipHostMalloc(%zu) failed", want);
            return nullptr;
        }
        g->fetch_chunks.push_back(q);
        g->fetch_chunk_bytes.push_back(want);
        fetch_used = bytes;
        return q;
    }

    TravGraph G{};
    double t_compact = 0;
    Mapper mapper, refMapper;
    uint32_t n_ctgs = 0, n_sel = 0;
    std::vector<CtgState> st;
    uint64_t nodes_total = 0;
    DevBuf b_packed, b_nodes, b_starts, b_sizes, b_tc, b_seedout, b_req, b_gset, b_gather, b_vids, b_gbits, b_ckreq, b_ckout;
    std::vector<TravContig> tc;
    static constexpr uint32_t SEED_STRIDE = 4096;
    void fill_contigs() {
        for (uint32_t i = 0; i < n_sel; ++i) {
            CtgState &cs = st[i];
            TravContig &t = tc[i];
            t.nodes = b_nodes.as<uint32_t>() + cs.nodesOff;
            t.n_kmers = cs.len >= k ? cs.len - k + 1 : 0;
            t.ctg_left = cs.ctgLeft;
            t.ctg_right = cs.ctgRight;
            t.rev_left = cs.revLeft;
            t.rev_right = cs.revRight;
            t.split_size = (uint64_t)(cs.len * startSplit);
            t.leap_min = 1 - startSplit;
            t.starts = b_starts.as<uint64_t>();
            t.sizes = b_sizes.as<uint64_t>();
            t.n_ctgs = n_ctgs;
            t.in_lo = cs.inLo;
            t.in_hi = cs.inHi;
            t.g_lo = cs.inLo;
            t.g_hi = cs.inHi;
            t.gbits = cs.committed ? cs.gbits : nullptr;
            t.gset = cs.committed ? cs.gset : nullptr;
            t.gmask = cs.gcap - 1;
            t.gwin_lo = cs.gwinLo;
            t.gwin_hi = cs.gwinHi;
        }
    }
    int upload_contigs() {
        fill_contigs();
        PAG_HIP_TRY(hipMemcpyAsync(b_tc.p, tc.data(), n_sel * sizeof(TravContig), hipMemcpyHostToDevice, s));
        return PAG_OK;
    }
    int fetch_vertices(const std::vector<uint32_t> &vids, std::vector<pag_path_node> &out) {
        out.resize(vids.size());
        if (vids.empty()) return PAG_OK;
        int r;
        if ((r = b_vids.alloc(vids.size() * 4)) || (r = b_gather.alloc(vids.size() * sizeof(pag_path_node)))) return r;
        PAG_HIP_TRY(hipMemcpyAsync(b_vids.p, vids.data(), vids.size() * 4, hipMemcpyHostToDevice, s));
        trav_launch_gather_vertices(G, b_vids.as<uint32_t>(), (uint32_t)vids.size(), b_gather.as<pag_path_node>(), s);
        PAG_HIP_TRY(hipMemcpyAsync(out.data(), b_gather.p, vids.size() * sizeof(pag_path_node), hipMemcpyDeviceToHost, s));
        PAG_HIP_TRY(hipStreamSynchronize(s));
        return PAG_OK;
    }

    uint64_t rounds = 0, jobs_total = 0, steps_total = 0, classify_total = 0, probe_total = 0, record_total = 0;
    double t_walk = 0;

    enum { CB_SEQV = 0, CB_SEQS, CB_ARV, CB_ARS, CB_TSET, CB_PSET, CB_STAMP, CB_TBITS, CB_SEQX, CB_N };
    enum { GRP_ROUND = 0, GRP_CHAIN0 = 1, GRP_FINAL = 9, GROUPS = 10 };
    DevBuf cbuf(uint32_t i, int grp, int b) { return DevBuf(g, &g->cpool[((size_t)i * GROUPS + grp) * CB_N + b]); }
    uint32_t QCAP = 32768;
    static constexpr uint32_t NR = TRAV_RINGS;
    TravQueue *hq = nullptr;
    TravPosted *hjobs = nullptr;
    TravJobOut *houts = nullptr;
    uint32_t *hdone = nullptr;
    double t_walk0 = 0, tw0 = 0;
    bool use_pieces = true, use_leap_pieces = true, force_exact = false;
    uint64_t seg_len_env = 0, seg_ov = 0;

    double t_st[4] = {0, 0, 0, 0};
    std::vector<stitch::RoundState> RS;
    struct JobRef {
        uint32_t ctg = 0;
        int kind = 0;
        int idx = 0;
        uint64_t init_len = 0;
        bool live = false;
        uint32_t epoch = 0;
    };
    std::vector<JobRef> jref;
    uint64_t n_orphans = 0;
    uint32_t n_posted[TRAV_RINGS] = {0, 0, 0}, n_live = 0, respeculated = 0;
    uint32_t scan_from[TRAV_RINGS] = {0, 0, 0};
    std::atomic<uint64_t> n_adopted{0}, n_merge_fail{0}, n_leap_adopted{0}, n_leap_refused[8];
    uint64_t n_seg_jobs = 0, n_resume_jobs = 0, n_leap_jobs = 0;
    WalkerGrid walkers;
    void shutdown_walker() {
        if (!walkers.up) return;
        walkers.shutdown();
        g->defer_free = false;
        for (void *q : g->deferred) hipFree(q);
        g->deferred.clear();
        for (void *q : pinned_parked) hipHostFree(q);
        pinned_parked.clear();
    }
    struct JobPlan {
        int kind, idx;
        uint64_t cap;
        uint32_t start_vid;
        uint32_t mode, stop_pc;
        const Chain *init;
        bool exact;
        uint32_t win_lo = 0, win_hi = 0;
        uint32_t win_low = 0;
    };
    bool need_publish = false;
    std::vector<TravClear> clears;
    void want_clear(void *p, size_t bytes, uint32_t byte_value) {
        if (bytes) clears.push_back(TravClear{p, (uint64_t)bytes, byte_value * 0x01010101u, 0u});
    }
    int flush_clears() {
        if (clears.empty()) return PAG_OK;
        TravClear *d = (TravClear *)fetch_alloc(clears.size() * sizeof(TravClear));
        if (!d) return PAG_ENOMEM;
        std::memcpy(d, clears.data(), clears.size() * sizeof(TravClear));
        const int r = trav_clear_ranges(d, clears.size(), s);
        clears.clear();
        return r;
    }
    struct Deferred {
        TravPosted P;
        JobRef jr;
    };
    std::vector<std::vector<Deferred>> deferred;
    bool defer_ring2 = false;
    struct Backlogged {
        TravPosted P;
        JobRef jr;
    };
    std::deque<Backlogged> backlog[TRAV_RINGS];
    bool place_job(uint32_t ring, const TravPosted &P, const JobRef &jr2) {
        const uint32_t jn = n_posted[ring], slot = ring * QCAP + jn % QCAP;
        if (jref[slot].live) return false;
        hjobs[slot] = P;
        hdone[slot] = 0;
        jref[slot] = jr2;
        if (jr2.kind == 0) RS[jr2.ctg].chains[(size_t)jr2.idx].job = (int)slot;
        n_posted[ring] += 1;
        return true;
    }
    int commit_job(uint32_t ring, const TravPosted &P, const JobRef &jr2, uint32_t mode, uint32_t stop_pc) {
        if (jr2.kind == 0) {
            Chain &ch = RS[jr2.ctg].chains[(size_t)jr2.idx];
            ch.job = 0x7FFFFFFF;
            ch.job_mode = mode;
            ch.job_stop = stop_pc;
        }
        n_live += 1;
        RS[jr2.ctg].live_jobs += 1;
        jobs_total += 1;
        if (wtrace) trace.push_back(TraceEv{now_ms() - tw0, 1u, jr2.ctg, (int32_t)jr2.kind, (int32_t)jr2.idx, ring, mode, jr2.init_len, 0});
        if (!backlog[ring].empty() || !place_job(ring, P, jr2)) backlog[ring].push_back(Backlogged{P, jr2});
        return PAG_OK;
    }
    bool is_orphan(const JobRef &jr) const { return jr.kind == 1 && jr.epoch != RS[jr.ctg].seg_epoch; }
    void flush_backlog() {
        for (uint32_t ring = 0; ring < TRAV_RINGS; ++ring)
            while (!backlog[ring].empty()) {
                if (is_orphan(backlog[ring].front().jr)) {
                    backlog[ring].pop_front();
                    n_live -= 1;
                    continue;
                }
                if (!place_job(ring, backlog[ring].front().P, backlog[ring].front().jr)) break;
                backlog[ring].pop_front();
                need_publish = true;
            }
    }
    void give_up_segments(uint32_t i) {
        RoundState &R = RS[i];
        if (R.live_jobs != 0)
            for (uint32_t ring = 0; ring < TRAV_RINGS; ++ring) {
                const uint32_t hi = n_posted[ring], lo = std::max(scan_from[ring], hi > QCAP ? hi - QCAP : 0u);
                for (uint32_t jn = lo; jn < hi; ++jn) {
                    const uint32_t q = jn % QCAP;
                    JobRef &jr = jref[ring * QCAP + q];
                    if (jr.live && jr.ctg == i && jr.kind == 1 && jr.epoch == R.seg_epoch) {
                        __atomic_fetch_or(&hjobs[ring * QCAP + q].J.mode, (uint32_t)TRAV_MODE_CANCELLED, __ATOMIC_RELEASE);
                        ++n_orphans;
                    }
                }
            }
        R.seg_epoch += 1;
        R.segs.clear();
        R.n_spec = 0;
        R.zone_end = 0;
        R.live_jobs = 0;
        R.kept = false;
    }
    int post_batch(uint32_t i, int grp, const std::vector<JobPlan> &plans) {
        if (plans.empty()) return PAG_OK;
        const double tp0 = now_ms();
        struct PostTimer {
            double t0, *acc;
            ~PostTimer() { *acc += now_ms() - t0; }
        } post_timer{tp0, &t_st[3]};
        CtgState &cs = st[i];
        RoundState &R = RS[i];
        const uint64_t PG = TRAV_PROBE_GROUPS;
        const size_t nj = plans.size();
        std::vector<uint64_t> o_seq(nj + 1, 0), o_oc(nj + 1, 0), o_st(nj + 1, 0), o_tb(nj + 1, 0), spans(nj, 0), o_x(nj + 1, 0);
        for (size_t j = 0; j < nj; ++j) {
            o_x[j + 1] = o_x[j] + ((plans[j].mode & TRAV_MODE_LEAP) ? plans[j].cap : 0);
            const uint32_t lo = plans[j].win_hi ? plans[j].win_lo : cs.inLo, hi = plans[j].win_hi ? plans[j].win_hi : cs.inHi;
            spans[j] = ((uint64_t)(hi - lo) + 1 + 3) & ~3ull;
            o_seq[j + 1] = o_seq[j] + plans[j].cap;
            o_oc[j + 1] = o_oc[j] + pow2_at_least((plans[j].mode & TRAV_MODE_LEAP) ? plans[j].cap + 8192 : plans[j].cap / 4 + 4096);
            o_st[j + 1] = o_st[j] + PG * spans[j];
            o_tb[j + 1] = o_tb[j] + spans[j] + 4;
        }
        DevBuf b_sv = cbuf(i, grp, CB_SEQV), b_ss = cbuf(i, grp, CB_SEQS), b_av = cbuf(i, grp, CB_ARV), b_as = cbuf(i, grp, CB_ARS),
               b_ts = cbuf(i, grp, CB_TSET), b_ps = cbuf(i, grp, CB_PSET), b_st = cbuf(i, grp, CB_STAMP), b_tb = cbuf(i, grp, CB_TBITS),
               b_sx = cbuf(i, grp, CB_SEQX);
        int r;
        {
            const size_t need[9] = {(size_t)o_seq[nj] * 4, (size_t)o_seq[nj] * 4, (size_t)o_seq[nj] * PG * 4, (size_t)o_seq[nj] * PG * 4,
                                    (size_t)o_oc[nj] * 8, (size_t)o_oc[nj] * PG * 8, (size_t)o_st[nj] * 4, (size_t)o_tb[nj] * 4, (size_t)o_x[nj] * 8};
            DevBuf *bufs[9] = {&b_sv, &b_ss, &b_av, &b_as, &b_ts, &b_ps, &b_st, &b_tb, &b_sx};
            size_t tot = 0;
            for (size_t q = 0; q < 9; ++q) tot += (need[q] + 16 + 255) & ~(size_t)255;
            if (g->walk_arena && g->walk_arena_used + tot <= g->walk_arena_cap) {
                for (size_t q = 0; q < 9; ++q) {
                    bufs[q]->p = (char *)g->walk_arena + g->walk_arena_used;
                    g->walk_arena_used += (need[q] + 16 + 255) & ~(size_t)255;
                }
            } else {
                R.slot_bufs = true;
                for (size_t q = 0; q < 9; ++q)
                    if ((r = bufs[q]->alloc(need[q]))) return r;
            }
        }
        want_clear(b_sx.p, o_x[nj] * 8, 0u);
        want_clear(b_ts.p, o_oc[nj] * 8, 0xFFu);
        want_clear(b_ps.p, o_oc[nj] * PG * 8, 0u);
        want_clear(b_st.p, o_st[nj] * 4, 0u);
        want_clear(b_tb.p, o_tb[nj] * 4, 0u);
        fill_contigs();
        for (size_t j = 0; j < nj; ++j) {
            const JobPlan &pl = plans[j];
            const uint32_t ring = pl.kind == 0 ? 0u : (R.round > 1 ? 1u : 2u);
            const uint64_t cap = pl.cap, oc = o_oc[j + 1] - o_oc[j];
            TravPosted P{};
            TravJob &J = P.J;
            J.ctg = i;
            J.start = pl.start_vid;
            J.has_size = R.has_size;
            J.seq_v = b_sv.as<uint32_t>() + o_seq[j];
            J.seq_s = b_ss.as<uint32_t>() + o_seq[j];
            J.seq_cap = cap;
            J.arena_v = b_av.as<uint32_t>() + o_seq[j] * PG;
            J.arena_s = b_as.as<uint32_t>() + o_seq[j] * PG;
            J.arena_cap = PG * cap;
            J.stamp = b_st.as<uint32_t>() + o_st[j];
            J.stamp_stride = (uint32_t)spans[j];
            J.tbits = b_tb.as<uint32_t>() + o_tb[j];
            J.tset = b_ts.as<uint64_t>() + o_oc[j];
            J.tmask = (uint32_t)oc - 1;
            J.pset = b_ps.as<uint64_t>() + o_oc[j] * PG;
            J.pmask = (uint32_t)oc - 1;
            J.exact = (pl.exact || force_exact) ? 1u : 0u;
            J.mode = pl.mode;
            J.stop_pc = pl.stop_pc;
            J.init_len = 0;
            J.win_low = pl.win_low;
            J.seq_x = (pl.mode & TRAV_MODE_LEAP) ? b_sx.as<uint64_t>() + o_x[j] : nullptr;
            if (pl.mode & TRAV_MODE_RESUME) {
                const uint64_t n0 = pl.init->len;
                if (n0 == 0 || n0 > cap) {
                    set_error("pag_travel: resume job with a %llu-vertex path in a %llu-vertex buffer", (unsigned long long)n0, (unsigned long long)cap);
                    return PAG_EFAULT;
                }
                J.init_len = n0;
                uint32_t *flat = (uint32_t *)fetch_alloc(n0 * 8);
                if (!flat) return PAG_ENOMEM;
                flatten_chain(*pl.init, flat, flat + n0, nullptr);
                PAG_HIP_TRY(hipMemcpyAsync(J.seq_v, flat, n0 * 4, hipMemcpyHostToDevice, s));
                PAG_HIP_TRY(hipMemcpyAsync(J.seq_s, flat + n0, n0 * 4, hipMemcpyHostToDevice, s));
            }
            P.C = tc[i];
            if (pl.win_hi) {
                P.C.in_lo = pl.win_lo;
                P.C.in_hi = pl.win_hi;
            }
            JobRef jr2;
            jr2.ctg = i;
            jr2.kind = pl.kind;
            jr2.idx = pl.idx;
            jr2.init_len = J.init_len;
            jr2.live = true;
            jr2.epoch = R.seg_epoch;
            if (pl.kind == 0) {
                if (pl.mode & TRAV_MODE_RESUME) ++n_resume_jobs;
            } else {
                ++n_seg_jobs;
                if (pl.mode & TRAV_MODE_LEAP) ++n_leap_jobs;
            }
            if (defer_ring2 && ring == 2u) {
                deferred[i].push_back(Deferred{P, jr2});
                continue;
            }
            int r2;
            if ((r2 = commit_job(ring, P, jr2, pl.mode, pl.stop_pc))) return r2;
        }
        need_publish = true;
        return PAG_OK;
    }
    int publish() {
        if (!need_publish) return PAG_OK;
        auto tmark = [&](const char *what) {
            if (wtrace) trace.push_back(TraceEv{now_ms() - tw0, 4u, n_live, 0, 0, (uint64_t)(uintptr_t)what, 0, clears.size(), 0});
        };
        tmark("publish: begin");
        int rcl;
        if ((rcl = flush_clears())) return rcl;
        tmark("publish: clears launched");
        PAG_HIP_TRY(hipStreamSynchronize(s));
        tmark("publish: stream idle");
        for (uint32_t r = NR; r-- > 0;) __atomic_store_n(&hq->posted[r], n_posted[r], __ATOMIC_RELEASE);
        need_publish = false;
        const int rcw = walkers.g ? walkers.ensure(n_live) : PAG_OK;
        tmark("publish: waves");
        return rcw;
    }
};
```

### aligngraph2_amd/csrc/hip/walk_session_loop.hpp

```cpp
#pragma once

struct WalkSession : WalkRounds {
    using WalkRounds::WalkRounds;

    int poll_finished(std::vector<uint32_t> &fin, bool &again) {
        int rc;
        again = false;
        for (uint32_t ring = 0; ring < NR; ++ring) {
            if (n_posted[ring] > QCAP && scan_from[ring] < n_posted[ring] - QCAP) scan_from[ring] = n_posted[ring] - QCAP;
            while (scan_from[ring] < n_posted[ring] && !jref[ring * QCAP + scan_from[ring] % QCAP].live) ++scan_from[ring];
            for (uint32_t jn = scan_from[ring]; jn < n_posted[ring]; ++jn) {
                const uint32_t slot = ring * QCAP + jn % QCAP;
                if (jref[slot].live && __atomic_load_n(&hdone[slot], __ATOMIC_ACQUIRE) != 0) fin.push_back(slot);
            }
        }
        if (!fin.empty()) {
            bool urgent = fin.size() >= 64 || (t_first_fin > 0 && now_ms() - t_first_fin > 1.0);
            for (size_t x = 0; x < fin.size() && !urgent; ++x) {
                const JobRef &jr = jref[fin[x]];
                if (jr.kind == 0) urgent = true;
                else
                    for (const Chain &ch : RS[jr.ctg].chains)
                        if (ch.waiting_seg == jr.idx) urgent = true;
            }
// ... 197 lines not shown
            for (Got &G2 : got) {
                const uint32_t slot = G2.jn;
                const JobRef &jr = jref[slot];
                const TravJobOut o = houts[slot];
                const uint32_t i = jr.ctg;
                if (jr.kind == 1) {
                    const Seg &sg = RS[i].segs[(size_t)jr.idx];
                    std::fprintf(stderr, "[walk] t=%.1f ms dev %.3f..%.3f contig %u segment %d done: %llu vertices, %s, %s (flags %d, outside %llu, classify %llu, back %u, chosen %u, probe %llu)\n", now_ms() - tw0,
                                 (double)(o.t_begin % 100000000000ull) * 1e-5, (double)(o.t_end % 100000000000ull) * 1e-5, i, jr.idx, (unsigned long long)o.seq_len, sg.stopped ? "stopped" : "ended", sg.usable ? "usable" : "NOT usable", o.overflow, (unsigned long long)o.n_out, (unsigned long long)o.n_classify,
                                 o.max_back, o.max_chosen, (unsigned long long)o.max_probe);
                } else if ((o.overflow & 7) == 0) {
                    std::fprintf(stderr, "[walk] t=%.1f ms dev %.3f..%.3f contig %u chain %d job done: +%llu vertices (%zu), %s (classify %llu)\n", now_ms() - tw0,
                                 (double)(o.t_begin % 100000000000ull) * 1e-5, (double)(o.t_end % 100000000000ull) * 1e-5, i, jr.idx, (unsigned long long)G2.len,
                                 RS[i].chains[(size_t)jr.idx].len, o.stopped ? "stopped" : "ended", (unsigned long long)o.n_classify);
#ifdef PAG_WALK_PROF
                    std::fprintf(stderr, "[walk]    prof mode %u main %llu fills %llu probes %llu:", hjobs[slot].J.mode, (unsigned long long)o.n_main,
                                 (unsigned long long)(o.n_fill & 0xFFFFFFFFull), (unsigned long long)o.n_probe);
                    for (int q = 0; q < 14; ++q) std::fprintf(stderr, " [%d] %.2f ms / %u", q, (double)o.prof_t[q] * 1e-5, o.prof_c[q]);
                    std::fprintf(stderr, "\n");
#endif
                }
            }
        std::sort(touched.begin(), touched.end());
        touched.erase(std::unique(touched.begin(), touched.end()), touched.end());
        {
            struct AdvTask {
                uint32_t i;
                int c;
                Next nx;
            };
            std::vector<AdvTask> tasks;
            for (uint32_t i : touched) {
                RoundState &R = RS[i];
                for (size_t c = 0; c < R.chains.size(); ++c) {
                    const Chain &ch = R.chains[c];
                    if (ch.final || ch.job >= 0) continue;
                    if (ch.waiting_seg >= 0 && !R.segs[(size_t)ch.waiting_seg].done) continue;
                    tasks.push_back(AdvTask{i, (int)c, Next{}});
                }
            }
            const unsigned nthr = (unsigned)std::min<size_t>(tasks.size() / 2, cfg.stitch_threads);
            const uint64_t fails_before = adv_stats.merge_fail;
            auto run = [&](std::atomic<size_t> &next, stitch::AdvanceStats &S) {
                for (size_t t = next.fetch_add(1); t < tasks.size(); t = next.fetch_add(1))
                    tasks[t].nx = advance_chain(RS[tasks[t].i], RS[tasks[t].i].chains[(size_t)tasks[t].c], merge_ctx(tasks[t].i), seg_ov, S);
            };
            std::atomic<size_t> next{0};
            if (nthr <= 1) {
                run(next, adv_stats);
            } else {
                std::vector<stitch::AdvanceStats> part(nthr);
                std::vector<std::thread> pool;
                for (unsigned t = 1; t < nthr; ++t) pool.emplace_back([&, t]() { run(next, part[t]); });
                run(next, part[0]);
                for (auto &th : pool) th.join();
                for (const stitch::AdvanceStats &S : part) {
                    adv_stats.adopted += S.adopted;
                    adv_stats.leap_adopted += S.leap_adopted;
                    adv_stats.merge_fail += S.merge_fail;
                    for (int w = 0; w < 8; ++w) adv_stats.leap_refused[w] += S.leap_refused[w];
                }
            }
            n_adopted = adv_stats.adopted;
            n_leap_adopted = adv_stats.leap_adopted;
            n_merge_fail = adv_stats.merge_fail;
            for (int w = 0; w < 8; ++w) n_leap_refused[w] = adv_stats.leap_refused[w];
            if (wdebug && adv_stats.merge_fail != fails_before)
                std::fprintf(stderr, "[walk] %llu segments were not adoptable, walking on exactly\n", (unsigned long long)(adv_stats.merge_fail - fails_before));
            for (const AdvTask &T : tasks)
                if (T.nx.what == Next::Resume && (rc = post_resume(T.i, T.c, T.nx.stop, T.nx.until_leap))) return fail(rc);
            if ((rc = flush_clears())) return fail(rc);
        }
        t_st[0] += ts1 - ts0;
        t_st[1] += ts2 - ts1;
        t_st[2] += now_ms() - ts2;
        lap("stitch");
        return PAG_OK;
    }
    void decide_rounds(const std::vector<uint32_t> &touched, std::vector<uint32_t> &batch) {
        for (uint32_t i : touched) {
            RoundState &R = RS[i];
            if (!R.active) continue;
            bool all = true;
            for (auto &ch : R.chains) all = all && ch.final;
            if (all && (R.live_jobs == 0 || !R.slot_bufs) && std::find(over_queue.begin(), over_queue.end(), i) == over_queue.end())
                over_queue.push_back(i);
        }
        {
            auto leaps = [&](uint32_t i) {
                for (const Chain &ch : RS[i].chains)
                    if (rounds::leaves_strand(mapper, rounds::end_coord(ch), st[i].chosenOne)) return true;
                return false;
            };
            const size_t take = over_queue.size();
            std::stable_partition(over_queue.begin(), over_queue.end(), [&](uint32_t i) { return !leaps(i); });
            batch.assign(over_queue.begin(), over_queue.begin() + (long)take);
            over_queue.erase(over_queue.begin(), over_queue.begin() + (long)take);
        }
    }
    struct Pick : rounds::Choice {
        uint64_t off = 0, len = 0;
    };
    int take_walks(const std::vector<uint32_t> &batch, std::vector<Pick> &picks) {
        int rc;
        {
            uint64_t tot = 0;
            for (uint32_t i : batch) {
                CtgState &cs = st[i];
                RoundState &R = RS[i];
                R.active = false;
                Pick &P = picks[i];
                static_cast<rounds::Choice &>(P) = rounds::choose(R.chains, cs.seeds, mapper, refMapper, cs.chosenOne, prm->min_len);
                if (P.chosen >= 0) {
                    P.len = R.chains[(size_t)P.chosen].len;
                    tot += P.len;
                }
                if (wtrace) trace.push_back(TraceEv{now_ms() - tw0, 2u, i, 0, P.chosen, R.round, P.leap ? 1u : 0u, P.chosen >= 0 ? R.chains[(size_t)P.chosen].len : 0, 0});
                if (wdebug && P.chosen >= 0) {
                    const Chain &ch = R.chains[(size_t)P.chosen];
                    const uint32_t last_ctg = rounds::end_coord(ch);
                    std::fprintf(stderr, "[walk] t=%.1f ms contig %u round %llu over: chain %d of %zu chosen, %llu vertices, size %llu, from offset %lld, ends at offset %lld (strand %u), mx %u%s\n",
                                 now_ms() - t_begin, i, (unsigned long long)R.round, P.chosen, R.chains.size(), (unsigned long long)ch.len, (unsigned long long)ch.size,
                                 (long long)cs.seeds[(size_t)P.chosen].ctg - (long long)cs.ctgLeft, last_ctg ? (long long)last_ctg - (long long)cs.ctgLeft : -1ll, cs.len,
                                 ch.mx_all >= cs.ctgLeft ? ch.mx_all - cs.ctgLeft : 0u, P.leap ? ", leap" : "");
                }
            }
            uint32_t *hp = (uint32_t *)pinned(tot * 4 + 256);
            if (!hp) return fail(PAG_ENOMEM);
            if ((rc = b_gather.alloc(tot * 4 + 64))) return fail(rc);
            struct CopyChunk {
                uint32_t i;
                const Chain::Part *pt;
                size_t x0, x1;
                LNode *dst;
                uint32_t *ids;
                std::vector<uint32_t> outside;
            };
            std::vector<CopyChunk> chunks;
            const size_t CHUNK = 1u << 17;
            uint64_t used = 0;
            for (uint32_t i : batch) {
                const Pick &P = picks[i];
                if (P.chosen < 0 || P.len == 0) continue;
                const Chain &ch = RS[i].chains[(size_t)P.chosen];
                CtgState &cs = st[i];
                std::vector<LNode> &base = cs.travel;
                const rounds::Trim trim = rounds::trim_path(base, ch.parts.front().pc[0], k);
                const size_t at0 = trim.at0;
                const int32_t dist = trim.dist;
                if (P.leap && !RS[i].slot_bufs && g->walk_arena && !cfg.debug_deliver_late) {
                    bool on_dev = true;
                    for (const Chain::Part &pt : ch.parts) on_dev = on_dev && pt.dv && pt.ds;
                    const size_t cap = at0 + P.len, need = (cap * 8 + 255) & ~(size_t)255;
                    TravConcatPart *cp = on_dev && g->walk_arena_used + need <= g->walk_arena_cap ? (TravConcatPart *)fetch_alloc(ch.parts.size() * sizeof(TravConcatPart)) : nullptr;
                    if (cp) {
                        CtgState::DevTail &T = cs.tail;
                        T.on = true;
                        T.d_ids = (uint32_t *)((char *)g->walk_arena + g->walk_arena_used);
                        g->walk_arena_used += need;
                        T.cap = cap;
                        T.m0 = at0;
                        T.n = P.len;
                        T.last_ctg = rounds::end_coord(ch);
                        T.step_bound = ch.size + (uint64_t)(dist > 0 ? dist : 0);
                        for (size_t x = 0; x < ch.parts.size(); ++x) cp[x] = TravConcatPart{ch.parts[x].dv, ch.parts[x].ds, ch.parts[x].start, ch.parts[x].n};
                        if (!g->deliver_stream && hipStreamCreateWithFlags(&g->deliver_stream, hipStreamNonBlocking) != hipSuccess) return fail(PAG_EFAULT);
                        trav_launch_concat_parts(cp, (uint32_t)ch.parts.size(), T.d_ids + at0, T.d_ids + cap + at0, (uint32_t)dist, g->deliver_stream);
                        continue;
                    }
                }
                base.resize(at0 + P.len);
                LNode *dst = base.data() + at0;
                picks[i].off = used;
                used += P.len;
                uint32_t *ids = hp + P.off;
                for (const Chain::Part &pt : ch.parts)
                    for (size_t x0 = 0; x0 < pt.n; x0 += CHUNK)
                        chunks.push_back(CopyChunk{i, &pt, x0, std::min(pt.n, x0 + CHUNK), dst + pt.start, ids + pt.start, {}});
                if (ch.low_nz != 0xFFFFFFFFu) {
                    cs.gwinLo = std::min(cs.gwinLo, ch.low_nz);
                    cs.gwinHi = std::max(cs.gwinHi, ch.mx_all);
                }
                cs.gFreeHi = std::max(cs.gFreeHi, ch.m0_all);
                cs.varLen += rounds::var_len_gain(trim, ch.size, ch.parts.front().s[0]);
                cs.pendingFirst = at0;
                cs.pendingFirstStep = dist;
            }
            {
                std::atomic<size_t> nxt{0};
                auto worker = [&]() {
                    for (size_t c; (c = nxt.fetch_add(1)) < chunks.size();) {
                        CopyChunk &C = chunks[c];
                        const Chain::Part &pt = *C.pt;
                        const uint32_t in_lo = st[C.i].inLo, in_hi = st[C.i].inHi;
                        for (size_t x = C.x0; x < C.x1; ++x) {
                            const uint32_t v = pt.v[x];
                            C.dst[x] = LNode(v, (int32_t)pt.s[x], pt.pc[x]);
                            C.ids[x] = v;
                            if (v < in_lo || v >= in_hi) C.outside.push_back(v);
                        }
                    }
                };
                worker();
            }
            for (CopyChunk &C : chunks)
                if (!C.outside.empty()) st[C.i].outsideU.insert(st[C.i].outsideU.end(), C.outside.begin(), C.outside.end());
            for (uint32_t i : batch) {
                const Pick &P = picks[i];
                if (P.chosen < 0 || P.len == 0 || st[i].tail.on) continue;
                st[i].travel[st[i].pendingFirst].step = st[i].pendingFirstStep;
            }
            if (used) hipMemcpyAsync(b_gather.p, hp, used * 4, hipMemcpyHostToDevice, s);
            for (uint32_t i : batch) {
                const Pick &P = picks[i];
                if (P.chosen < 0 || P.len == 0 || st[i].tail.on) continue;
                CtgState &cs = st[i];
                if ((uint64_t)cs.outsideU.size() * 2 > cs.gcap) {
                    uint32_t ncap = cs.gcap;
                    while ((uint64_t)cs.outsideU.size() * 4 > ncap) ncap *= 2;
                    DevBuf b_ng = cbuf(i, GRP_FINAL, CB_TSET), b_ou = cbuf(i, GRP_FINAL, CB_PSET);
                    if ((rc = b_ng.alloc((size_t)ncap * 4)) || (rc = b_ou.alloc(cs.outsideU.size() * 4))) return fail(rc);
                    hipMemsetAsync(b_ng.p, 0xFF, (size_t)ncap * 4, s);
                    hipMemcpyAsync(b_ou.p, cs.outsideU.data(), cs.outsideU.size() * 4, hipMemcpyHostToDevice, s);
                    trav_launch_commit(b_ou.as<uint32_t>(), cs.outsideU.size(), 0u, 0u, nullptr, b_ng.as<uint32_t>(), ncap - 1, s);
                    cs.gset = b_ng.as<uint32_t>();
                    cs.gcap = ncap;
                }
                trav_launch_commit(b_gather.as<uint32_t>() + P.off, P.len, cs.inLo, cs.inHi, cs.gbits, cs.gset, cs.gcap - 1, s);
                cs.committed = true;
            }
        }
        for (uint32_t i : batch) RS[i].chains.clear();
        lap("choose+gather");
        return PAG_OK;
    }
    void splice_batch(const std::vector<uint32_t> &batch, const std::vector<Pick> &picks, std::vector<TravSeedReq> &reqs, std::vector<uint32_t> &req_cs) {
        std::vector<TravSeedReq> slot_req(n_sel);
        std::vector<uint8_t> slot_has(n_sel, 0);
        auto splice = [&](uint32_t i) {
            CtgState &cs = st[i];
            const Pick &P = picks[i];
            const rounds::Stop stop = rounds::stop_rules(cs.ctgQ, cs.refQ, P, deviation);
            if (stop.done) {
                if (stop.finalLeap) cs.finalLeap = true;
                cs.done = true;
                return;
            }
            const rounds::Anchor an = rounds::last_on_strand(cs.travel, mapper, cs.chosenOne);
            const rounds::Window w = rounds::seed_window(an.pos, deviation);
            TravSeedReq r{};
            r.ctg = i;
            r.pos = an.pos;
            r.left = w.left;
            r.right = w.right;
            slot_req[i] = r;
            slot_has[i] = 1;
            cs.seeds.clear();
            cs.parentU = an.u;
            cs.haveParent = an.found;
        };
        {
            unsigned nthr = std::min<unsigned>((unsigned)batch.size(), std::max(1u, std::min(32u, std::thread::hardware_concurrency())));
            std::atomic<size_t> next{0};
            auto worker = [&]() {
                for (size_t x; (x = next.fetch_add(1)) < batch.size();) splice(batch[x]);
            };
            std::vector<std::thread> pool;
            for (unsigned t = 1; t < nthr; ++t) pool.emplace_back(worker);
            worker();
            for (auto &t : pool) t.join();
        }
        for (uint32_t i : batch)
            if (slot_has[i]) {
                reqs.push_back(slot_req[i]);
                req_cs.push_back(i);
            }
        for (uint32_t i : batch) {
            if (st[i].done) give_up_segments(i);
            else RS[i].kept = !RS[i].segs.empty();
        }
        lap("splice");
    }
    int reseed(std::vector<TravSeedReq> &reqs, const std::vector<uint32_t> &req_cs, std::vector<uint32_t> &next_round) {
        int rc;
        if (!reqs.empty()) {
            const uint32_t PARTS = TRAV_SEED_PARTS;
            uint32_t WSTRIDE = cfg.debug_seed_stride ? cfg.debug_seed_stride : 2048;
            std::vector<uint32_t> wb;
            for (;;) {
                const size_t words = (size_t)reqs.size() * PARTS * WSTRIDE;
                if ((rc = b_req.alloc(reqs.size() * sizeof(TravSeedReq))) || (rc = b_seedout.alloc(words * 4))) return fail(rc);
                uint32_t *hp = (uint32_t *)pinned(words * 4 + 256);
                if (!hp) return fail(PAG_ENOMEM);
                hipError_t he = hipMemcpyAsync(b_req.p, reqs.data(), reqs.size() * sizeof(TravSeedReq), hipMemcpyHostToDevice, s);
                if (upload_contigs() != PAG_OK) he = hipErrorUnknown;
                trav_launch_seed_window(G, b_tc.as<TravContig>(), b_req.as<TravSeedReq>(), (uint32_t)reqs.size(), deviation,
                                        b_seedout.as<uint32_t>(), WSTRIDE, s);
                if (he == hipSuccess) he = hipMemcpyAsync(hp, b_seedout.p, words * 4, hipMemcpyDeviceToHost, s);
                if (he == hipSuccess) he = hipStreamSynchronize(s);
                if (he != hipSuccess) {
                    set_error("pag_travel: seed search failed: %s", hipGetErrorString(he));
                    return fail(PAG_EFAULT);
                }
                uint32_t most = 0;
                for (size_t q = 0; q < reqs.size() * PARTS; ++q) most = std::max(most, hp[q * WSTRIDE]);
                if (most <= WSTRIDE - 1) {
                    wb.assign(hp, hp + words);
                    break;
                }
                if (most > (1u << 28)) {
                    set_error("pag_travel: seed window with %u candidates", most);
                    return fail(PAG_ENOMEM);
                }
                const uint32_t again = (uint32_t)pow2_at_least((uint64_t)most + 2);
                if (timing) std::fprintf(stderr, "[timing] seed windows: a part of %zu requests has %u candidates, searched again with stride %u -> %u\n", reqs.size(), most, WSTRIDE, again);
                WSTRIDE = again;
            }
            std::vector<uint32_t> vids;
            std::vector<size_t> cnt(reqs.size());
            for (size_t q = 0; q < reqs.size(); ++q)
                cnt[q] = rounds::window_candidates(&wb[q * PARTS * WSTRIDE], PARTS, WSTRIDE, vids);
            std::vector<pag_path_node> attrs;
            if ((rc = fetch_vertices(vids, attrs))) return fail(rc);
            {
                std::vector<uint32_t> pu(reqs.size());
                for (size_t q = 0; q < reqs.size(); ++q) pu[q] = st[req_cs[q]].parentU;
                std::vector<pag_path_node> pa(reqs.size());
                if ((rc = b_vids.alloc(pu.size() * 8)) || (rc = b_gather.alloc(pu.size() * sizeof(pag_path_node) + 64))) return fail(rc);
                hipMemcpyAsync(b_vids.p, pu.data(), pu.size() * 4, hipMemcpyHostToDevice, s);
                hipMemsetAsync(b_vids.as<uint32_t>() + pu.size(), 0, pu.size() * 4, s);
                trav_launch_gather_path(G, b_vids.as<uint32_t>(), b_vids.as<uint32_t>() + pu.size(), pu.size(), b_gather.as<pag_path_node>(), s);
                hipMemcpyAsync(pa.data(), b_gather.p, pa.size() * sizeof(pag_path_node), hipMemcpyDeviceToHost, s);
                if (hipStreamSynchronize(s) != hipSuccess) {
                    set_error("pag_travel: parent k-mer lookup failed");
                    return fail(PAG_EFAULT);
                }
                for (size_t q = 0; q < reqs.size(); ++q) st[req_cs[q]].parentCode = pa[q].code;
            }
            size_t at = 0;
            for (size_t q = 0; q < reqs.size(); ++q) {
                CtgState &cs = st[req_cs[q]];
                const std::string parent = cs.haveParent ? code2kmer(cs.parentCode, k) : std::string();
                rounds::order_seeds(attrs.data() + at, cnt[q], parent, k, topK, cs.seeds);
                at += cnt[q];
                if (cs.seeds.empty()) {
                    cs.done = true;
                    give_up_segments(req_cs[q]);
                }
                else next_round.push_back(req_cs[q]);
            }
        }
        return PAG_OK;
    }
    int event_loop() {
        int rc;
        t_progress = now_ms();
        t_first_fin = 0;
        t_last_news = now_ms();
        while (n_live || !over_queue.empty()) {
            std::vector<uint32_t> fin, touched, batch, req_cs, next_round;
            bool again = false;
            if ((rc = poll_finished(fin, again))) return rc;
            if (again) continue;
            auto mark = [&](const char *what) {
                if (wdebug) std::fprintf(stderr, "[walk] t=%.1f ms loop: %s (%zu jobs, %zu contigs decided, %u live)\n", now_ms() - tw0, what, fin.size(), batch.size(), n_live);
                if (wtrace) trace.push_back(TraceEv{now_ms() - tw0, 4u, n_live, 0, 0, (uint64_t)(uintptr_t)what, 0, fin.size(), batch.size()});
            };
            mark("polled");
            std::vector<Got> got;
            if ((rc = fetch_paths(fin, got))) return rc;
            mark("fetched");
            if ((rc = stitch_finished(got, touched))) return rc;
            mark("stitched");
            decide_rounds(touched, batch);
            flush_backlog();
            if (batch.empty()) {
                if ((rc = publish())) return fail(rc);
                mark("published");
                lap("round prep");
                continue;
            }
            std::vector<Pick> picks(n_sel);
            if ((rc = take_walks(batch, picks))) return rc;
            mark("walks taken");
            std::vector<TravSeedReq> reqs;
            splice_batch(batch, picks, reqs, req_cs);
            mark("spliced");
            if ((rc = reseed(reqs, req_cs, next_round))) return rc;
            mark("re-seeded");
            for (uint32_t i : batch)
                if (st[i].done && (rc = deliver_contig(i))) return fail(rc);
            mark("delivered");
            lap("reseed");
            if (!next_round.empty() && (rc = start_rounds(next_round))) return fail(rc);
            mark("next rounds posted");
            flush_backlog();
            if ((rc = publish())) return fail(rc);
            mark("published");
            lap("round prep");
        }
        return PAG_OK;
    }
    int finish() {
        int rc;
        shutdown_walker();
        g->defer_free = false;
        for (void *q : pinned_parked) hipHostFree(q);
        pinned_parked.clear();
        t_walk = now_ms() - tw0;
        lap("walk");
        if (wtrace) {
            uint64_t d0 = ~0ull;
            for (const TraceEv &e : trace)
                if (e.what == 0u) d0 = std::min(d0, e.a);
            std::fprintf(stderr, "[trace] walks %.2f ms, %zu events; device times relative to the first job's begin\n", t_walk, trace.size());
            for (const TraceEv &e : trace) {
                if (e.what == 0u)
                    std::fprintf(stderr, "[trace] done t=%.2f ctg %u %s %d dev %.2f..%.2f len %llu classify %llu\n", e.t, e.ctg, e.kind ? "seg" : "chain", e.idx, (double)(e.a - d0) * 1e-5,
                                 (double)(e.b - d0) * 1e-5, (unsigned long long)e.len, (unsigned long long)e.classify);
                else if (e.what == 4u)
                    std::fprintf(stderr, "[trace] loop t=%.2f %s jobs %llu decided %llu live %u\n", e.t, (const char *)(uintptr_t)e.a, (unsigned long long)e.len, (unsigned long long)e.classify, e.ctg);
                else if (e.what == 1u)
                    std::fprintf(stderr, "[trace] post t=%.2f ctg %u %s %d ring %llu mode %llu init %llu\n", e.t, e.ctg, e.kind ? "seg" : "chain", e.idx, (unsigned long long)e.a, (unsigned long long)e.b,
                                 (unsigned long long)e.len);
                else
                    std::fprintf(stderr, "[trace] over t=%.2f ctg %u round %llu chain %d len %llu%s\n", e.t, e.ctg, (unsigned long long)e.a, e.idx, (unsigned long long)e.len, e.b ? " leap" : "");
            }
            trace.clear();
        }
        if (timing || wdebug) {
            std::fprintf(stderr, "[timing] stitch: bookkeeping %.1f ms, paths %.1f ms, chains %.1f ms; posting jobs (all callers) %.1f ms; fetch memory: chunk %zu of %zu; walk arena: %.2f of %.2f GB used\n", t_st[0], t_st[1], t_st[2], t_st[3],
                         fetch_chunk + 1, g->fetch_chunks.size(), g->walk_arena_used / 1e9, g->walk_arena_cap / 1e9);
            std::fprintf(stderr, "[timing] leaping zone: %llu segment jobs, %llu adopted, refused by reason (unusable, no junction, not a boundary, cannot leap yet, window top, window bottom, contig-following record, coordinate-free record): %llu %llu %llu %llu %llu %llu %llu %llu\n",
                         (unsigned long long)n_leap_jobs, (unsigned long long)n_leap_adopted.load(), (unsigned long long)n_leap_refused[0].load(), (unsigned long long)n_leap_refused[1].load(), (unsigned long long)n_leap_refused[2].load(),
                         (unsigned long long)n_leap_refused[3].load(), (unsigned long long)n_leap_refused[4].load(), (unsigned long long)n_leap_refused[5].load(), (unsigned long long)n_leap_refused[6].load(), (unsigned long long)n_leap_refused[7].load());
            {
                size_t n_tail = 0, n_tail_behind = 0;
                for (const CtgState &cs : st) n_tail += cs.tail.on, n_tail_behind += cs.tail.on && cs.tail.m0;
                std::fprintf(stderr, "[timing] last rounds put together on the device: %zu of %u contigs (%zu behind an earlier round's path)\n", n_tail, n_sel, n_tail_behind);
            }
            std::fprintf(stderr, "[timing] pieces: %llu segment jobs, %llu resume jobs, %llu vertices adopted, %llu segments not adoptable\n", (unsigned long long)n_seg_jobs,
                         (unsigned long long)n_resume_jobs, (unsigned long long)n_adopted.load(), (unsigned long long)n_merge_fail.load());
        }

        for (uint32_t i = 0; i < n_sel; ++i)
            if (!st[i].delivered) rounds::filter_travel(st[i].travel, st[i].finalLeap, mapper, st[i].ci, startSplit);
        {
            uint64_t tot = 0;
            for (auto &cs : st)
                if (!cs.delivered) tot += cs.travel.size();
            if (g->path_cap < tot + 1) {
                if (g->path_store) hipHostFree(g->path_store);
                g->path_store = nullptr;
                g->path_cap = 0;
                const size_t want = tot + tot / 8 + 1024;
                if (hipHostMalloc((void **)&g->path_store, want * sizeof(pag_path_node), hipHostMallocDefault) != hipSuccess) {
                    set_error("pag_travel: hipHostMalloc for %zu path records failed", want);
                    return fail(PAG_ENOMEM);
                }
                g->path_cap = want;
            }
            uint32_t *hp = (uint32_t *)pinned(tot * 8 + 256);
            if (!hp) return fail(PAG_ENOMEM);
            uint64_t at = 0;
            size_t scratch_bytes = 0;
            for (auto &cs : st) {
                if (cs.delivered) continue;
                const size_t slot2 = 2 * (size_t)cs.ci + (cs.forward ? 0 : 1);
                if (!cs.travel.empty()) scratch_bytes += render_scratch_bytes(cs.travel.size());
                g->path_off[slot2] = at;
                g->path_len[slot2] = cs.travel.size();
                g->path_valid[slot2] = 1;
                for (size_t x = 0; x < cs.travel.size(); ++x) {
                    hp[at + x] = cs.travel[x].u;
                    hp[tot + at + x] = (uint32_t)cs.travel[x].step;
                }
                at += cs.travel.size();
            }
            DevBuf b_fin(g, ps::WALK_FIN);
            if ((rc = b_fin.alloc(tot * 8 + 64)) || (rc = b_gather.alloc(tot * sizeof(pag_path_node) + 64))) return fail(rc);
            if (tot) {
                PAG_HIP_TRY(hipMemcpyAsync(b_fin.p, hp, tot * 8, hipMemcpyHostToDevice, s));
                trav_launch_gather_path(G, b_fin.as<uint32_t>(), b_fin.as<uint32_t>() + tot, tot, b_gather.as<pag_path_node>(), s);
                PAG_HIP_TRY(hipMemcpyAsync(g->path_store, b_gather.p, tot * sizeof(pag_path_node), hipMemcpyDeviceToHost, s));
            }
            if (scratch_bytes) {
                if (g->dump_scratch_cap < scratch_bytes) {
                    if (g->dump_scratch) PAG_HIP_TRY(hipFree(g->dump_scratch));
                    g->dump_scratch = nullptr;
                    g->dump_scratch_cap = 0;
                    PAG_HIP_TRY(hipMalloc(&g->dump_scratch, scratch_bytes + scratch_bytes / 4));
                    g->dump_scratch_cap = scratch_bytes + scratch_bytes / 4;
                }
                size_t sat = 0;
                for (auto &cs : st) {
                    if (cs.delivered || cs.travel.empty()) continue;
                    const size_t slot2 = 2 * (size_t)cs.ci + (cs.forward ? 0 : 1);
                    const uint32_t *ids = b_fin.as<uint32_t>() + g->path_off[slot2];
                    auto carve = [&](size_t bytes) {
                        void *q = (char *)g->dump_scratch + sat;
                        sat += bytes;
                        return q;
                    };
                    const uint64_t bases = render_seq ? (uint64_t)k + positive_steps(cs.travel, 1, cs.travel.size()) : 0;
                    if ((rc = render_texts(slot2, ids, ids + tot, cs.travel.size(), bases, carve, s, 0u))) return fail(rc);
                    if (render) ++n_epilogue_texts;
                    if (render_seq) ++n_epilogue_seqs;
                }
            }
            PAG_HIP_TRY(hipStreamSynchronize(s));
            if (g->deliver_stream) PAG_HIP_TRY(hipStreamSynchronize(g->deliver_stream));
            resolve_texts();
            for (TextKind kind : {TEXT_DUMP, TEXT_SEQ}) {
                const TextKindOf K = text_kind(kind);
                if (!timing || !K.on) continue;
                size_t n_text = 0, n_none = 0;
                for (auto &cs : st) {
                    const size_t slot2 = 2 * (size_t)cs.ci + (cs.forward ? 0 : 1);
                    if (g->path_len[slot2]) (K.ptr[slot2] ? n_text : n_none) += 1;
                }
                std::fprintf(stderr, K.timing, n_text, K.n_epilogue, n_none);
            }
        }
        lap("epilogue");
        if (timing) {
            std::fprintf(stderr, "[timing] walks redone without speculation: %u\n", respeculated);
            std::fprintf(stderr, "[timing] segment jobs left behind by rounds that were decided without them: %llu\n", (unsigned long long)n_orphans);
            std::fprintf(stderr, "[timing] pag_travel laps:");
            for (auto &l : laps) std::fprintf(stderr, " %s %.1f ms;", l.first, l.second);
            std::fprintf(stderr, "\n");
        }
        if (stats) {
            stats->ms_compact = t_compact;
            stats->ms_walk = t_walk;
            stats->ms_total = now_ms() - t_begin;
            stats->rounds = rounds;
            stats->jobs = jobs_total;
            stats->walk_steps = steps_total;
            stats->classify_calls = classify_total;
            stats->probes = probe_total;
            stats->records = record_total;
        }
        return PAG_OK;
    }
    int run() {
        int rc;
        if ((rc = begin()) || (rc = setup_contigs())) return rc;
        if (n_sel == 0) return PAG_OK;
        if ((rc = first_seeds()) || (rc = setup_rings()) || (rc = reserve_arena()) || (rc = post_first_rounds()) || (rc = event_loop())) return rc;
        return finish();
    }
};
```

### aligngraph2_amd/csrc/hip/walk_session_rounds.hpp

```cpp
#pragma once

struct WalkRounds : WalkJobs {
    using WalkJobs::WalkJobs;


    uint32_t first_stop(const stitch::RoundState &R) const { return stitch::stop_for(R, 0, seg_ov); }
    struct RoundPlan {
        std::vector<uint32_t> ck_x;
        size_t n_spec_ck = 0;
        uint32_t x0 = 0xFFFFFFFFu, seed_lo = 0, seed_hi = 0;
        size_t req_off = 0, co_off = 0;
        bool has_co = false;
        bool kept = false;
        uint32_t kept_stop = 0;
    };
    void plan_rounds(const std::vector<uint32_t> &which, std::vector<RoundPlan> &RP, std::vector<TravSeedReq> &reqs) {
        for (size_t w = 0; w < which.size(); ++w) {
            const uint32_t i = which[w];
            RoundPlan &P = RP[w];
            std::vector<uint32_t> &ck_x = P.ck_x;
            size_t &n_spec_ck = P.n_spec_ck;
            uint32_t &x0 = P.x0;
            CtgState &cs = st[i];
            RoundState &R = RS[i];
// ... 162 lines not shown
                if (P.kept || first_stop(R) != 0u) window(nq, &seed_lo, &seed_hi);
            }
            std::vector<JobPlan> plans;
            const uint64_t cap_full = cs.seqCap;
            for (size_t sd = 0; sd < cs.seeds.size(); ++sd) {
                const uint32_t stop = P.kept ? P.kept_stop : (R.segs.empty() ? 0u : first_stop(R));
                JobPlan pl{0, (int)sd, cap_full, cs.seeds[sd].vid, 0u, stop, nullptr, false};
                if (stop != 0u && seed_hi != 0u && cs.seeds[sd].ctg <= stop) {
                    pl.win_lo = seed_lo;
                    pl.win_hi = seed_hi;
                    pl.cap = std::min<uint64_t>(cap_full, ((uint64_t)stop - cs.seeds[sd].ctg) / 2 + 8192);
                }
                plans.push_back(pl);
            }
            std::vector<size_t> seg_order;
            for (size_t q = R.segs.size(); q-- > 0;)
                if (R.segs[q].leap && R.segs[q].stop == 0u) {
                    seg_order.push_back(q);
                    break;
                }
            for (size_t q = 0; q < R.segs.size(); ++q)
                if (seg_order.empty() || q != seg_order[0]) seg_order.push_back(q);
            for (int pass = 0; pass < 2 && !P.kept; ++pass)
                for (size_t q : seg_order) {
                    if (R.segs[q].leap != (pass == 0)) continue;
                    const uint64_t spanc = (R.segs[q].stop ? (uint64_t)R.segs[q].stop : (uint64_t)cs.ctgRight) - R.segs[q].x;
                    const uint64_t cap = std::min<uint64_t>(cap_full, spanc / 2 + 8192);
                    JobPlan pl{1, (int)q, cap, R.segs[q].vid, (uint32_t)(R.segs[q].leap ? TRAV_MODE_LEAP : TRAV_MODE_SPEC), R.segs[q].stop, nullptr, false, R.segs[q].win_lo, R.segs[q].win_hi};
                    pl.win_low = R.segs[q].leap ? R.segs[q].win_low : 0u;
                    plans.push_back(pl);
                }
            if (wdebug)
                std::fprintf(stderr, "[walk] t=%.1f ms contig %u round %u: %zu seeds, %zu segments%s, cut zone ends at %u (strand %u..%u)\n", now_ms() - t_walk0, i,
                             R.round, cs.seeds.size(), R.segs.size(), P.kept ? " kept from an earlier round" : "", R.zone_end, cs.ctgLeft, cs.ctgRight);
            if ((r = post_batch(i, GRP_ROUND, plans))) return r;
        }
        return PAG_OK;
    }
    int start_rounds(const std::vector<uint32_t> &which) {
        std::vector<RoundPlan> RP(which.size());
        std::vector<TravSeedReq> reqs;
        std::vector<uint32_t> out, co, ids;
        int r;
        plan_rounds(which, RP, reqs);
        if ((r = find_checkpoints(reqs, out))) return r;
        make_segments(which, RP, out, co);
        if ((r = find_id_bounds(co, ids))) return r;
        if ((r = post_round_jobs(which, RP, ids))) return r;
        return flush_clears();
    }

    int post_resume(uint32_t i, int c, uint32_t stop, bool until_leap = false) {
        CtgState &cs = st[i];
        Chain &ch = RS[i].chains[(size_t)c];
        const uint64_t cap = std::max<uint64_t>(cs.seqCap * ch.grow, ch.len + cs.seqCap / 4 + 4096);
        std::vector<JobPlan> plans{JobPlan{0, c, cap, cs.seeds[(size_t)c].vid, (uint32_t)(TRAV_MODE_RESUME | (until_leap ? TRAV_MODE_UNTIL_LEAP : 0)), stop, &ch, ch.exact}};
        return post_batch(i, GRP_CHAIN0 + c, plans);
    }

    stitch::MergeCtx merge_ctx(uint32_t i) {
        MergeCtx M;
        M.k = k;
        M.deviation = deviation;
        M.split = (uint64_t)(st[i].len * startSplit);
        M.has_size = RS[i].has_size;
        M.round = RS[i].round;
        if (st[i].committed) {
            M.g_lo = st[i].gwinLo;
            M.g_hi = st[i].gwinHi;
            M.g_free_hi = st[i].gFreeHi;
        }
        return M;
    }
    stitch::AdvanceStats adv_stats;

    int fail(int rc2) {
        shutdown_walker();
        g->defer_free = false;
        for (void *q : pinned_parked) hipHostFree(q);
        pinned_parked.clear();
        if (g->deliver_stream) hipStreamSynchronize(g->deliver_stream);
        hipStreamSynchronize(s);
        std::fill(g->path_valid.begin(), g->path_valid.end(), (uint8_t)0);
        std::fill(g->path_ptr.begin(), g->path_ptr.end(), nullptr);
        std::fill(g->text_ptr.begin(), g->text_ptr.end(), nullptr);
        std::fill(g->text_len.begin(), g->text_len.end(), (uint64_t)0);
        std::fill(g->seq_ptr.begin(), g->seq_ptr.end(), nullptr);
        std::fill(g->seq_len.begin(), g->seq_len.end(), (uint64_t)0);
        text_pending.clear();
        return rc2;
    }

    static constexpr unsigned DELIVER_BLOCKS = 24;
    bool render = false, render_seq = false;
    DumpTables dump_tab{};
    uint32_t dump_bound = 0;
    std::vector<uint32_t> dump_blob;
    SeqSources seq_src{};
    enum TextKind { TEXT_DUMP, TEXT_SEQ };
    struct TextPending {
        TextKind kind;
        size_t slot2;
        char *buf;
        uint64_t cap;
    };
    std::vector<TextPending> text_pending;
    size_t n_epilogue_texts = 0, n_epilogue_seqs = 0;
    struct TextKindOf {
        bool on;
        std::vector<const char *> &ptr;
        std::vector<uint64_t> &len;
        size_t &n_epilogue;
        const char *timing;
    };
    TextKindOf text_kind(TextKind kind) {
        if (kind == TEXT_DUMP)
            return {render, g->text_ptr, g->text_len, n_epilogue_texts, "[timing] dump text: %zu contigs rendered (%zu of them in the epilogue), %zu left to the host\n"};
        return {render_seq, g->seq_ptr, g->seq_len, n_epilogue_seqs, "[timing] sequence text: %zu paths rendered (%zu of them in the epilogue), %zu left to the host\n"};
    }
    int setup_render() {
        render = render_seq = false;
        const bool want_dumps = (prm->reserved & PAG_TRAVEL_RENDER_DUMPS) != 0;
        const pag_seqs *refs = g->seq_refs;
        bool want_seqs = (prm->reserved & PAG_TRAVEL_RENDER_SEQS) != 0 && refs && refs->n_seqs == n_refs && seqs_well_formed(refs) && seqs_well_formed(ctgs);
        for (uint64_t r = 0; want_seqs && r < n_refs; ++r) want_seqs = refs->len[r] == ref_len[r];
        if ((!want_dumps && !want_seqs) || !dump_tables_build(ctgs->len, ctgs->n_seqs, ref_len, n_refs, dump_blob)) return PAG_OK;
        const size_t bytes = dump_blob.size() * 4 + 16;
        if (g->dump_tables_cap < bytes) {
            if (g->dump_tables) PAG_HIP_TRY(hipFree(g->dump_tables));
            g->dump_tables = nullptr;
            g->dump_tables_cap = 0;
            PAG_HIP_TRY(hipMalloc(&g->dump_tables, bytes + bytes / 4));
            g->dump_tables_cap = bytes + bytes / 4;
        }
        if (!dump_blob.empty()) PAG_HIP_TRY(hipMemcpyAsync(g->dump_tables, dump_blob.data(), dump_blob.size() * 4, hipMemcpyHostToDevice, s));
        dump_tab = dump_tables_at((const uint32_t *)g->dump_tables, ctgs->n_seqs, n_refs);
        dump_bound = dump_line_bound(k, dump_blob, ctgs->n_seqs, n_refs);
        render = want_dumps;
        if (want_seqs) {
            DevBuf b_seqs(g, ps::WALK_SEQS);
            int rc2;
            if ((rc2 = b_seqs.alloc(seq_sources_bytes(ctgs, refs))) || (rc2 = seq_sources_upload(b_seqs.p, ctgs, refs, &seq_src, s))) return rc2;
            render_seq = true;
        }
        return PAG_OK;
    }
    static uint64_t positive_steps(const std::vector<LNode> &seq, size_t from, size_t to) {
        uint64_t b = 0;
        for (size_t x = from; x < to; ++x) b += seq[x].step > 0 ? (uint64_t)seq[x].step : 0ull;
        return b;
    }
    size_t render_scratch_bytes(size_t m) const { return ((render ? 1 : 0) + (render_seq ? 1 : 0)) * text_scratch_bytes(m); }
    void *arena_scratch(size_t need) {
        if (!g->walk_arena || g->walk_arena_used + need > g->walk_arena_cap) return nullptr;
        void *q = (char *)g->walk_arena + g->walk_arena_used;
        g->walk_arena_used += need;
        return q;
    }
    template <typename Scratch>
    int render_texts(size_t slot2, const uint32_t *d_v, const uint32_t *d_s, size_t m, uint64_t bases, Scratch scratch, hipStream_t st, unsigned max_blocks) {
        for (TextKind kind : {TEXT_DUMP, TEXT_SEQ}) {
            if (!text_kind(kind).on) continue;
            void *sc = scratch(text_scratch_bytes(m));
            const uint64_t cap = kind == TEXT_DUMP ? (uint64_t)m * dump_bound : bases;
            char *buf = sc ? (char *)fetch_alloc(256 + cap + 16) : nullptr;
            if (!buf) continue;
            ((uint64_t *)buf)[0] = ~0ull;
            ((uint64_t *)buf)[1] = 0;
            const int rc2 = kind == TEXT_DUMP ? trav_launch_dump_path(G, d_v, d_s, m, k, dump_tab, sc, buf + 256, cap, (uint64_t *)buf, st, max_blocks)
                                              : trav_launch_seq_path(G, d_v, d_s, m, SeqParams{k, (uint64_t)deviation, errorRate}, dump_tab, seq_src, sc, buf + 256, cap,
                                                                     (uint64_t *)buf, st, max_blocks);
            if (rc2) return rc2;
            text_pending.push_back(TextPending{kind, slot2, buf, cap});
        }
        return PAG_OK;
    }
    void resolve_texts() {
        for (const TextPending &t : text_pending) {
            const uint64_t total = ((const volatile uint64_t *)t.buf)[0], bad = ((const volatile uint64_t *)t.buf)[1];
            if (total > t.cap || bad) continue;
            const TextKindOf K = text_kind(t.kind);
            K.ptr[t.slot2] = t.buf + 256;
            K.len[t.slot2] = total;
        }
        text_pending.clear();
    }
    int deliver_contig(uint32_t i) {
        CtgState &cs = st[i];
        if (cs.delivered || !cs.done) return PAG_OK;
        if (cs.tail.on) {
            const CtgState::DevTail &T = cs.tail;
            const size_t m0 = T.m0, m = m0 + T.n - (rounds::pumped(mapper, T.last_ctg, cs.ci, startSplit) ? 1 : 0);
            const size_t slot2 = 2 * (size_t)cs.ci + (cs.forward ? 0 : 1);
            cs.delivered = true;
            g->path_off[slot2] = 0;
            g->path_len[slot2] = m;
            g->path_valid[slot2] = 1;
            if (m == 0) return PAG_OK;
            pag_path_node *dst = (pag_path_node *)fetch_alloc(m * sizeof(pag_path_node));
            if (!dst) return PAG_ENOMEM;
            if (m0) {
                uint32_t *hp = (uint32_t *)fetch_alloc(m0 * 8);
                if (!hp) return PAG_ENOMEM;
                for (size_t x = 0; x < m0; ++x) {
                    hp[x] = cs.travel[x].u;
                    hp[m0 + x] = (uint32_t)cs.travel[x].step;
                }
                PAG_HIP_TRY(hipMemcpyAsync(T.d_ids, hp, m0 * 4, hipMemcpyHostToDevice, g->deliver_stream));
                PAG_HIP_TRY(hipMemcpyAsync(T.d_ids + T.cap, hp + m0, m0 * 4, hipMemcpyHostToDevice, g->deliver_stream));
            }
            trav_launch_gather_path(G, T.d_ids, T.d_ids + T.cap, m, dst, g->deliver_stream, n_live ? DELIVER_BLOCKS : 0u);
            g->path_ptr[slot2] = dst;
            return render_texts(slot2, T.d_ids, T.d_ids + T.cap, m, render_seq ? (uint64_t)k + T.step_bound + positive_steps(cs.travel, 0, m0) : 0,
                                [&](size_t bytes) { return arena_scratch(bytes); }, g->deliver_stream, n_live ? DELIVER_BLOCKS : 0u);
        }
        if (cfg.debug_deliver_late) return PAG_OK;
        const size_t n = cs.travel.size();
        const size_t need = ((n * 8 + 255) & ~(size_t)255) + 512 + render_scratch_bytes(n);
        if (!g->walk_arena || g->walk_arena_used + need > g->walk_arena_cap) return PAG_OK;
        rounds::filter_travel(cs.travel, cs.finalLeap, mapper, cs.ci, startSplit);
        const size_t m = cs.travel.size();
        const size_t slot2 = 2 * (size_t)cs.ci + (cs.forward ? 0 : 1);
        cs.delivered = true;
        g->path_off[slot2] = 0;
        g->path_len[slot2] = m;
        g->path_valid[slot2] = 1;
        if (m == 0) return PAG_OK;
        uint32_t *hp = (uint32_t *)fetch_alloc(m * 8);
        pag_path_node *dst = (pag_path_node *)fetch_alloc(m * sizeof(pag_path_node));
        if (!hp || !dst) return PAG_ENOMEM;
        for (size_t x = 0; x < m; ++x) {
            hp[x] = cs.travel[x].u;
            hp[m + x] = (uint32_t)cs.travel[x].step;
        }
        uint32_t *d_ids = (uint32_t *)((char *)g->walk_arena + g->walk_arena_used);
        g->walk_arena_used += (m * 8 + 255) & ~(size_t)255;
        if (!g->deliver_stream) PAG_HIP_TRY(hipStreamCreateWithFlags(&g->deliver_stream, hipStreamNonBlocking));
        PAG_HIP_TRY(hipMemcpyAsync(d_ids, hp, m * 8, hipMemcpyHostToDevice, g->deliver_stream));
        trav_launch_gather_path(G, d_ids, d_ids + m, m, dst, g->deliver_stream, n_live ? DELIVER_BLOCKS : 0u);
        g->path_ptr[slot2] = dst;
        return render_texts(slot2, d_ids, d_ids + m, m, render_seq ? (uint64_t)k + positive_steps(cs.travel, 1, m) : 0, [&](size_t bytes) { return arena_scratch(bytes); },
                            g->deliver_stream, n_live ? DELIVER_BLOCKS : 0u);
    }

    double t_progress = 0, t_first_fin = 0;
    double t_last_news = 0;
    void idle_wait(double us) {
        const double t0w = now_ms();
        if (t0w - t_last_news > 5.0) {
            std::this_thread::sleep_for(std::chrono::microseconds((long)us));
            return;
        }
        while ((now_ms() - t0w) * 1000.0 < us) {
            for (int q = 0; q < 32; ++q) __builtin_ia32_pause();
        }
    }
    std::vector<uint32_t> over_queue;

    int begin() {
        PAG_HIP_TRY(hipSetDevice(g->device));
        s = g->stream;
        t_begin = now_ms();
        timing = cfg.timing;
        wdebug = cfg.walk_debug;
        wtrace = cfg.walk_trace;
        lap_t = t_begin;
        k = g->k;
        deviation = prm->deviation;
        errorRate = prm->error_rate;
        startSplit = prm->start_split;
        topK = std::min<uint32_t>(prm->ref_threads, 8u);
        int rc;
        if ((rc = trav_prepare_graph(g, ctgs->len, ctgs->n_seqs, ref_len, n_refs, deviation, errorRate, &G, &t_compact, orient, startSplit))) return rc;
        lap("compact");
        return PAG_OK;
    }
    int setup_contigs() {
        int rc;
        n_ctgs = (uint32_t)ctgs->n_seqs;
        g->path_off.assign(2 * (size_t)n_ctgs, 0);
        g->path_len.assign(2 * (size_t)n_ctgs, 0);
        g->path_valid.assign(2 * (size_t)n_ctgs, 0);
        g->path_ptr.assign(2 * (size_t)n_ctgs, nullptr);
        g->text_ptr.assign(2 * (size_t)n_ctgs, nullptr);
        g->text_len.assign(2 * (size_t)n_ctgs, 0);
        g->seq_ptr.assign(2 * (size_t)n_ctgs, nullptr);
        g->seq_len.assign(2 * (size_t)n_ctgs, 0);
        for (uint32_t c2 = 0; c2 < 2 * n_ctgs; ++c2) {
            const uint32_t c = c2 >> 1;
            const bool fwd = (c2 & 1u) == 0;
            const int32_t o = orient[c];
            if (!(o == PAG_ORIENT_BOTH || (fwd && o == PAG_ORIENT_FORWARD) || (!fwd && o == PAG_ORIENT_REVERSE))) continue;
            CtgState cs;
            cs.ci = c;
            cs.forward = fwd;
            cs.chosenOne = cs.forward ? (int64_t)c + 1 : -(int64_t)c - 1;
            cs.len = ctgs->len[c];
            cs.ctgLeft = (uint32_t)mapper.dualToSingle(cs.chosenOne, 0);
            cs.ctgRight = (uint32_t)mapper.dualToSingle(cs.chosenOne, cs.len);
            cs.revLeft = (uint32_t)mapper.dualToSingle(-cs.chosenOne, 0);
            cs.revRight = (uint32_t)mapper.dualToSingle(-cs.chosenOne, cs.len);
            cs.nodesOff = nodes_total;
            cs.seqCap = (uint64_t)cs.len / 2 + 8192;
            if (cfg.debug_seqcap) cs.seqCap = (uint64_t)cfg.debug_seqcap;
            nodes_total += cs.len >= k ? cs.len - k + 1 : 0;
            st.push_back(std::move(cs));
        }
        n_sel = (uint32_t)st.size();
        if (n_sel == 0) return PAG_OK;

        b_packed = DevBuf(g, ps::WALK_PACKED), b_nodes = DevBuf(g, ps::WALK_NODES), b_starts = DevBuf(g, ps::WALK_STARTS), b_sizes = DevBuf(g, ps::WALK_SIZES);
        b_tc = DevBuf(g, ps::WALK_TC), b_seedout = DevBuf(g, ps::WALK_SEEDOUT), b_req = DevBuf(g, ps::WALK_REQ), b_gset = DevBuf(g, ps::WALK_GSET);
        b_gather = DevBuf(g, ps::WALK_GATHER), b_vids = DevBuf(g, ps::WALK_VIDS), b_gbits = DevBuf(g, ps::WALK_GBITS);
        b_ckreq = DevBuf(g, ps::WALK_CKREQ), b_ckout = DevBuf(g, ps::WALK_CKOUT);
        if ((rc = b_packed.alloc(ctgs->packed_bytes + 64)) || (rc = b_nodes.alloc((nodes_total + 1) * 4)) ||
            (rc = b_starts.alloc(mapper.starts.size() * 8 + 8)) || (rc = b_sizes.alloc(mapper.sizes.size() * 8 + 8)) ||
            (rc = b_tc.alloc(n_sel * sizeof(TravContig))))
            return rc;
        PAG_HIP_TRY(hipMemcpyAsync(b_packed.p, ctgs->packed, ctgs->packed_bytes, hipMemcpyHostToDevice, s));
        PAG_HIP_TRY(hipMemcpyAsync(b_starts.p, mapper.starts.data(), mapper.starts.size() * 8, hipMemcpyHostToDevice, s));
        PAG_HIP_TRY(hipMemcpyAsync(b_sizes.p, mapper.sizes.data(), mapper.sizes.size() * 8, hipMemcpyHostToDevice, s));
        if ((rc = setup_render())) return rc;
        {
            std::vector<TravCtgNodesJob> cj;
            uint32_t max_len = 0;
            for (auto &cs : st) {
                cj.push_back(TravCtgNodesJob{ctgs->byte_off[cs.ci], cs.nodesOff, (uint32_t)cs.len, cs.forward ? 1 : 0});
                max_len = std::max<uint32_t>(max_len, (uint32_t)cs.len);
            }
            DevBuf b_cj(g, ps::WALK_CJ);
            if ((rc = b_cj.alloc(cj.size() * sizeof(TravCtgNodesJob)))) return rc;
            PAG_HIP_TRY(hipMemcpyAsync(b_cj.p, cj.data(), cj.size() * sizeof(TravCtgNodesJob), hipMemcpyHostToDevice, s));
            PAG_HIP_TRY(hipStreamSynchronize(s));
            trav_launch_ctg_nodes(b_packed.as<uint8_t>(), b_cj.as<TravCtgNodesJob>(), (uint32_t)cj.size(), max_len, k, G, b_nodes.as<uint32_t>(), s);
        }

        tc.assign(n_sel, TravContig{});
        {
            for (auto &cs : st) cs.gcap = 1024;
            if ((rc = upload_contigs())) return rc;
            trav_launch_ranges(G, b_tc.as<TravContig>(), n_sel, s);
            PAG_HIP_TRY(hipMemcpyAsync(tc.data(), b_tc.p, n_sel * sizeof(TravContig), hipMemcpyDeviceToHost, s));
            PAG_HIP_TRY(hipStreamSynchronize(s));
            uint64_t tot_set = 0, tot_bits = 0;
            for (uint32_t i = 0; i < n_sel; ++i) {
                CtgState &cs = st[i];
                cs.inLo = tc[i].in_lo;
                cs.inHi = tc[i].in_hi;
                cs.gcap = (uint32_t)pow2_at_least(cs.seqCap / 2 + 8192);
                tot_set += cs.gcap;
                tot_bits += ((uint64_t)(cs.inHi - cs.inLo) + 31) / 32 + 1;
            }
            if ((rc = b_gset.alloc(tot_set * 4)) || (rc = b_gbits.alloc(tot_bits * 4))) return rc;
            PAG_HIP_TRY(hipMemsetAsync(b_gset.p, 0xFF, tot_set * 4, s));
            PAG_HIP_TRY(hipMemsetAsync(b_gbits.p, 0, tot_bits * 4, s));
            uint64_t o1 = 0, o2 = 0;
            for (auto &cs : st) {
                cs.gset = b_gset.as<uint32_t>() + o1;
                o1 += cs.gcap;
                cs.gbits = b_gbits.as<uint32_t>() + o2;
                o2 += ((uint64_t)(cs.inHi - cs.inLo) + 31) / 32 + 1;
            }
        }

        lap("contig tables");
        return PAG_OK;
    }
    int first_seeds() {
        int rc;
        if ((rc = b_seedout.alloc((uint64_t)n_sel * SEED_STRIDE * 4))) return rc;
        if ((rc = upload_contigs())) return rc;
        trav_launch_seed_first(G, b_tc.as<TravContig>(), n_sel, deviation, b_seedout.as<uint32_t>(), SEED_STRIDE, s);
        std::vector<uint32_t> seedbuf((size_t)n_sel * SEED_STRIDE);
        PAG_HIP_TRY(hipMemcpyAsync(seedbuf.data(), b_seedout.p, seedbuf.size() * 4, hipMemcpyDeviceToHost, s));
        PAG_HIP_TRY(hipStreamSynchronize(s));
        {
            std::vector<uint32_t> vids;
            std::vector<size_t> cnt(n_sel);
            for (uint32_t i = 0; i < n_sel; ++i) {
                const uint32_t *o = &seedbuf[(size_t)i * SEED_STRIDE];
                size_t n = std::min<size_t>(std::min<size_t>(o[0], (SEED_STRIDE - 2) / 2), topK);
                cnt[i] = n;
                for (size_t j = 0; j < n; ++j) vids.push_back(o[1 + 2 * j]);
            }
            std::vector<pag_path_node> attrs;
            if ((rc = fetch_vertices(vids, attrs))) return rc;
            size_t at = 0;
            for (uint32_t i = 0; i < n_sel; ++i) {
                st[i].seeds.assign(attrs.begin() + at, attrs.begin() + at + cnt[i]);
                at += cnt[i];
                if (st[i].seeds.empty()) st[i].done = true;
            }
        }

        lap("first seeds");
        return PAG_OK;
    }
    int setup_rings() {
        if (g->cpool.size() < (size_t)n_sel * GROUPS * CB_N) g->cpool.resize((size_t)n_sel * GROUPS * CB_N);
        {
            const uint64_t sl = std::max<uint64_t>(128, cfg.seg_len ? cfg.seg_len : 12000);
            const uint64_t ll = std::max<uint64_t>(128, sl / 2);
            uint64_t est = 0;
            for (uint32_t i = 0; i < n_sel; ++i) est += (uint64_t)st[i].len / sl + (uint64_t)st[i].len / ll + 32;
            while (QCAP < 2 * est && QCAP < (1u << 24)) QCAP *= 2;
            if (cfg.debug_ring) QCAP = (uint32_t)cfg.debug_ring;
        }
        const size_t q_need = 256 + NR * (size_t)QCAP * (sizeof(TravPosted) + sizeof(TravJobOut) + sizeof(uint32_t)) + 256;
        if (g->wq_bytes < q_need) {
            if (g->wq_host) hipHostFree(g->wq_host);
            g->wq_host = nullptr;
            g->wq_bytes = 0;
            PAG_HIP_TRY(hipHostMalloc(&g->wq_host, q_need, hipHostMallocCoherent | hipHostMallocMapped));
            g->wq_bytes = q_need;
        }
        if (!g->wq_next) PAG_HIP_TRY(hipMalloc((void **)&g->wq_next, 256));
        hq = (TravQueue *)g->wq_host;
        hjobs = (TravPosted *)((char *)g->wq_host + 256);
        houts = (TravJobOut *)(hjobs + NR * (size_t)QCAP);
        hdone = (uint32_t *)(houts + NR * (size_t)QCAP);
        std::memset(g->wq_host, 0, 256);
        std::memset(hdone, 0, NR * (size_t)QCAP * sizeof(uint32_t));
        PAG_HIP_TRY(hipMemsetAsync(g->wq_next, 0, 256, s));
        PAG_HIP_TRY(hipStreamSynchronize(s));
        t_walk0 = now_ms();
        use_pieces = cfg.pieces;
        seg_len_env = cfg.seg_len;
        seg_ov = cfg.seg_overlap;
        force_exact = cfg.force_exact;
        RS.clear();
        RS.resize(n_sel);
        jref.assign(NR * (size_t)QCAP, JobRef{});
        for (auto &x : n_leap_refused) x = 0;
        use_leap_pieces = cfg.leap_pieces;
        deferred.clear();
        deferred.resize(n_sel);
        lap("rings");
        return PAG_OK;
    }
    int reserve_arena() {
        if (!pinned(64u << 20)) return PAG_ENOMEM;
        {
            size_t want = 0;
            for (uint32_t i = 0; i < n_sel; ++i) {
                const CtgState &cs = st[i];
                const size_t span = (size_t)(cs.inHi - cs.inLo) + 8, cap = cs.seqCap, oc = pow2_at_least(cap / 4 + 4096);
                const size_t chain = cap * 8 + cap * 8 * TRAV_PROBE_GROUPS + oc * 8 * (1 + TRAV_PROBE_GROUPS) + span * 4 * (1 + TRAV_PROBE_GROUPS);
                const size_t n_seg = cs.len / 12000 + 1, scap = 8192 + 8192, soc = pow2_at_least(scap / 4 + 4096), sspan = span / (n_seg ? n_seg : 1) * 2 + 4096;
                const size_t seg = scap * 8 + scap * 8 * TRAV_PROBE_GROUPS + soc * 8 * (1 + TRAV_PROBE_GROUPS) + sspan * 4 * (1 + TRAV_PROBE_GROUPS);
                const size_t n_lseg = cs.len / 8 / 6000 + 2, lcap = 3000 + 8192, loc = pow2_at_least(lcap + 8192), lspan = sspan;
                const size_t lseg = lcap * 8 + lcap * 8 * TRAV_PROBE_GROUPS + lcap * 8 + loc * 8 * (1 + TRAV_PROBE_GROUPS) + lspan * 4 * (1 + TRAV_PROBE_GROUPS);
                want += chain * 3 / 2 + (seg * (n_seg + 8) + lseg * n_lseg) * 3 / 2;
            }
            size_t free_b = 0, total_b = 0;
            const size_t sharers = env_device_sharers();
            if (hipMemGetInfo(&free_b, &total_b) == hipSuccess) want = std::min(want, (free_b + g->walk_arena_cap) * 2 / 5 / sharers);
            if (g->walk_arena_cap < want / 10 * 7) {
                if (g->walk_arena) hipFree(g->walk_arena);
                g->walk_arena = nullptr;
                g->walk_arena_cap = 0;
                if (hipMalloc(&g->walk_arena, want) == hipSuccess) g->walk_arena_cap = want;
                else g->walk_arena = nullptr;
            }
            g->walk_arena_used = 0;
        }
        lap("arena");
        return PAG_OK;
    }
    int post_first_rounds() {
        int rc;
        tw0 = now_ms();
        t_walk0 = tw0;
        g->defer_free = true;
        {
            std::vector<uint32_t> order(n_sel);
            for (uint32_t i = 0; i < n_sel; ++i) order[i] = i;
            std::stable_sort(order.begin(), order.end(), [&](uint32_t a2, uint32_t b2) { return st[a2].len > st[b2].len; });
            const uint32_t interleave = 16;
            defer_ring2 = true;
            {
                std::vector<uint32_t> first_rounds;
                for (uint32_t i : order)
                    if (!st[i].done) first_rounds.push_back(i);
                if ((rc = start_rounds(first_rounds))) return fail(rc);
            }
            lap("first rounds planned");
            defer_ring2 = false;
            {
                std::vector<size_t> at(n_sel, 0);
                std::vector<uint32_t> share(n_sel, interleave);
                {
                    size_t least = 0;
                    for (uint32_t i : order)
                        if (!deferred[i].empty() && (least == 0 || deferred[i].size() < least)) least = deferred[i].size();
                    const size_t turns = least ? (least + interleave - 1) / interleave : 1;
                    for (uint32_t i : order)
                        if (!deferred[i].empty()) share[i] = (uint32_t)std::max<double>(1.0, std::ceil((double)deferred[i].size() / (double)turns));
                }
                for (uint32_t i : order) {
                    auto &dq = deferred[i];
                    if (at[i] < dq.size() && (dq[0].P.J.mode & TRAV_MODE_LEAP) && dq[0].P.J.stop_pc == 0u) {
                        if ((rc = commit_job(2u, dq[0].P, dq[0].jr, dq[0].P.J.mode, dq[0].P.J.stop_pc))) return fail(rc);
                        at[i] = 1;
                    }
                }
                for (bool more = true; more;) {
                    more = false;
                    for (uint32_t i : order) {
                        auto &dq = deferred[i];
                        for (uint32_t c = 0; c < share[i] && at[i] < dq.size(); ++c, ++at[i])
                            if ((rc = commit_job(2u, dq[at[i]].P, dq[at[i]].jr, dq[at[i]].P.J.mode, dq[at[i]].P.J.stop_pc))) return fail(rc);
                        more = more || at[i] < dq.size();
                    }
                }
                for (auto &dq : deferred) std::vector<Deferred>().swap(dq);
            }
        }
        lap("ring order");
        if (n_live) {
            walkers.init(g, G, hjobs, houts, hdone, hq, QCAP, k);
            walkers.trace = wtrace;
            if ((rc = publish())) return fail(rc);
            lap("marks cleared, rings published");
            if ((rc = walkers.ensure(n_live))) {
                g->defer_free = false;
                return rc;
            }
            if (wdebug) std::fprintf(stderr, "[walk] %u walker waves launched (at most %u), %u + %u + %u jobs posted\n", walkers.launched, walkers.max_waves, n_posted[0], n_posted[1], n_posted[2]);
        } else {
            g->defer_free = false;
        }
        lap("round prep");
        return PAG_OK;
    }

};
```

Baseline: 4.190 billion.

## Split walk arena into bottom/top regions and track pre-zeroed extent to skip clears

Replaces the bump-pointer walk arena with a two-ended allocator. Buffers that must start zeroed come from the top, and only the part not already known to be clean is queued for clearing. With PAG_WALK_ARENA_CLEAN set, the used top region is zeroed at the end of a call on a low-priority stream so the next call can skip those clears. Publish also skips its stream synchronize when no work was queued since the last sync. Background clean-up is off by default, so the default path mainly changes clear bookkeeping and publish syncs, at the cost of added state and a debug check path.

```diff
diff --git a/aligngraph2_amd/csrc/hip/k5_walk_aux.hip b/aligngraph2_amd/csrc/hip/k5_walk_aux.hip
--- a/aligngraph2_amd/csrc/hip/k5_walk_aux.hip
+++ b/aligngraph2_amd/csrc/hip/k5_walk_aux.hip
@@ -352,6 +352,47 @@
     PAG_HIP_TRY(hipGetLastError());
     return PAG_OK;
 }
+__global__ void __launch_bounds__(256) k_fill_zero(uint4 *__restrict__ p, uint64_t n16) {
+    uint4 *q = as_global(p);
+    const uint4 z = make_uint4(0u, 0u, 0u, 0u);
+#pragma unroll 4
+    for (uint64_t i = (uint64_t)blockIdx.x * blockDim.x + threadIdx.x; i < n16; i += (uint64_t)gridDim.x * blockDim.x) q[i] = z;
+}
+int trav_fill_zero(void *p, uint64_t bytes, hipStream_t s) {
+    if (((uintptr_t)p & 15u) || (bytes & 15u)) {
+        set_error("trav_fill_zero: a range of %llu bytes at %p is not made of 16-byte lines", (unsigned long long)bytes, p);
+        return PAG_EINVAL;
+    }
+    const uint64_t n16 = bytes >> 4;
+    if (!n16) return PAG_OK;
+    int dev = 0, n_cu = 256;
+    if (hipGetDevice(&dev) != hipSuccess || hipDeviceGetAttribute(&n_cu, hipDeviceAttributeMultiprocessorCount, dev) != hipSuccess) n_cu = 256;
+    const unsigned grid = (unsigned)std::min<uint64_t>((n16 + 255) / 256, (uint64_t)std::max(1, n_cu) * 4u);
+    k_fill_zero<<<dim3(grid), dim3(256), 0, s>>>((uint4 *)p, n16);
+    PAG_HIP_TRY(hipGetLastError());
+    return PAG_OK;
+}
+__global__ void __launch_bounds__(256) k_check_zero(const TravClear *__restrict__ ranges, const uint8_t *base, unsigned long long *first_bad) {
+    const TravClear c = ranges[blockIdx.y];
+    const uint4 *q = (const uint4 *)c.p;
+    const uint64_t n16 = c.bytes >> 4;
+    for (uint64_t i = (uint64_t)blockIdx.x * blockDim.x + threadIdx.x; i < n16; i += (uint64_t)gridDim.x * blockDim.x) {
+        const uint4 w = q[i];
+        if ((w.x | w.y | w.z | w.w) == 0u) continue;
+        const uint32_t ws[4] = {w.x, w.y, w.z, w.w};
+        uint32_t b = 0;
+        while (((ws[b >> 2] >> (8u * (b & 3u))) & 0xFFu) == 0u) ++b;
+        atomicMin(first_bad, (unsigned long long)((const uint8_t *)(q + i) - base) + b);
+    }
+}
+int trav_check_zero(const TravClear *ranges_dev, size_t n, const void *base, unsigned long long *first_bad_dev, hipStream_t s) {
+    for (size_t at = 0; at < n; at += 32768) {
+        const uint32_t m = (uint32_t)std::min<size_t>(32768, n - at);
+        k_check_zero<<<dim3(32, m), dim3(256), 0, s>>>(ranges_dev + at, (const uint8_t *)base, first_bad_dev);
+    }
+    PAG_HIP_TRY(hipGetLastError());
+    return PAG_OK;
+}
 void trav_launch_gather_path(TravGraph G, const uint32_t *seq_v, const uint32_t *seq_s, uint64_t len, pag_path_node *out,
                              hipStream_t s, unsigned max_blocks) {
     const unsigned grid = max_blocks ? std::min(grid_for(len), max_blocks) : grid_for(len);
diff --git a/aligngraph2_amd/csrc/hip/pag_api.hip b/aligngraph2_amd/csrc/hip/pag_api.hip
--- a/aligngraph2_amd/csrc/hip/pag_api.hip
+++ b/aligngraph2_amd/csrc/hip/pag_api.hip
@@ -238,7 +238,9 @@
     for (void *q : g->fetch_chunks) hipHostFree(q);
     g->fetch_chunks.clear();
     g->fetch_chunk_bytes.clear();
-    if (g->walk_arena) hipFree(g->walk_arena);
+    pagdev::walk_arena_release(g);
+    if (g->clean_event) hipEventDestroy(g->clean_event);
+    if (g->clean_stream) hipStreamDestroy(g->clean_stream);
     if (g->dump_tables) hipFree(g->dump_tables);
     if (g->dump_scratch) hipFree(g->dump_scratch);
     if (g->wq_next) hipFree(g->wq_next);
@@ -649,15 +651,7 @@
     }
     pagdev::WalkerGrid::prepare_streams(g, 4);
     if (g->walk_arena_cap >= want) return PAG_OK;
-    if (g->walk_arena) hipFree(g->walk_arena);
-    g->walk_arena = nullptr;
-    g->walk_arena_cap = 0;
-    if (hipMalloc(&g->walk_arena, want) != hipSuccess) {
-        g->walk_arena = nullptr;
-        (void)hipGetLastError();
-        return PAG_OK;
-    }
-    g->walk_arena_cap = want;
+    if (!pagdev::walk_arena_acquire(g, want)) (void)hipGetLastError();
     return PAG_OK;
 }
 
diff --git a/aligngraph2_amd/csrc/hip/pag_graph_impl.hpp b/aligngraph2_amd/csrc/hip/pag_graph_impl.hpp
--- a/aligngraph2_amd/csrc/hip/pag_graph_impl.hpp
+++ b/aligngraph2_amd/csrc/hip/pag_graph_impl.hpp
@@ -6,6 +6,7 @@
 #include "pag_device.hpp"
 #include "pag_travel.hpp"
 #include "pool_slots.hpp"
+#include "walk_arena.hpp"
 
 struct pag_graph {
     int device = 0;
@@ -63,7 +64,11 @@
     void *dump_tables = nullptr, *dump_scratch = nullptr;
     size_t dump_tables_cap = 0, dump_scratch_cap = 0;
     void *walk_arena = nullptr;
-    size_t walk_arena_cap = 0, walk_arena_used = 0;
+    size_t walk_arena_cap = 0;
+    arena::WalkArena arena_state;
+    hipStream_t clean_stream = nullptr;
+    hipEvent_t clean_event = nullptr;
+    bool clean_pending = false;
     std::vector<void *> fetch_chunks;
     std::vector<size_t> fetch_chunk_bytes;
     bool regional = false;
@@ -123,6 +128,28 @@
 };
 
 
+inline void walk_arena_settle(pag_graph *g) {
+    if (g->clean_pending) hipEventSynchronize(g->clean_event);
+    g->clean_pending = false;
+}
+inline void walk_arena_release(pag_graph *g) {
+    walk_arena_settle(g);
+    if (g->walk_arena) hipFree(g->walk_arena);
+    g->walk_arena = nullptr;
+    g->walk_arena_cap = 0;
+    g->arena_state.reset(0);
+}
+inline bool walk_arena_acquire(pag_graph *g, size_t bytes) {
+    walk_arena_release(g);
+    if (hipMalloc(&g->walk_arena, bytes) != hipSuccess) {
+        g->walk_arena = nullptr;
+        return false;
+    }
+    g->walk_arena_cap = bytes;
+    g->arena_state.reset(bytes);
+    return true;
+}
+
 struct StreamPtrs {
     const uint32_t *tkey;
     const uint64_t *tval;
diff --git a/aligngraph2_amd/csrc/hip/pag_travel.hpp b/aligngraph2_amd/csrc/hip/pag_travel.hpp
--- a/aligngraph2_amd/csrc/hip/pag_travel.hpp
+++ b/aligngraph2_amd/csrc/hip/pag_travel.hpp
@@ -183,6 +183,8 @@
     uint32_t word, pad;
 };
 int trav_clear_ranges(const TravClear *ranges_dev, size_t n, hipStream_t s);
+int trav_fill_zero(void *p, uint64_t bytes, hipStream_t s);
+int trav_check_zero(const TravClear *ranges_dev, size_t n, const void *base, unsigned long long *first_bad_dev, hipStream_t s);
 int trav_successors_of(TravGraph G, uint32_t code, uint64_t pos, void *recs, uint64_t cap, unsigned long long *out, hipStream_t s);
 constexpr uint32_t EMIT_CHUNK_SLOTS = 2048u, EMIT_GRID_THREADS = 2048u, EMIT_GRID_WAVES = 1024u;
 constexpr uint64_t EMIT_SLACK_SLOTS = (uint64_t)(EMIT_GRID_THREADS + EMIT_GRID_WAVES) * 4u * EMIT_CHUNK_SLOTS;
diff --git a/aligngraph2_amd/csrc/hip/shard_serial.hip b/aligngraph2_amd/csrc/hip/shard_serial.hip
--- a/aligngraph2_amd/csrc/hip/shard_serial.hip
+++ b/aligngraph2_amd/csrc/hip/shard_serial.hip
@@ -53,9 +53,7 @@
     hipStreamSynchronize(g->stream);
     g->tg_ready = false;
     for (int i = ps::TG_NCODE; i <= ps::WALK_SEQS; ++i) free_slot(g->pool[i]);
-    if (g->walk_arena) hipFree(g->walk_arena);
-    g->walk_arena = nullptr;
-    g->walk_arena_cap = g->walk_arena_used = 0;
+    walk_arena_release(g);
 }
 
 void release_build_keeping(pag_graph *g, const pag_build_input *in) {
diff --git a/aligngraph2_amd/csrc/hip/walk_arena.hpp b/aligngraph2_amd/csrc/hip/walk_arena.hpp
--- /dev/null
+++ b/aligngraph2_amd/csrc/hip/walk_arena.hpp
@@ -0,0 +1,64 @@
+#pragma once
+#include <algorithm>
+#include <cstdint>
+
+namespace arena {
+
+struct Range {
+    uint64_t off = 0, bytes = 0;
+};
+
+struct WalkArena {
+    static constexpr uint64_t ALIGN = 256;
+    static uint64_t round(uint64_t bytes) { return (bytes + ALIGN - 1) & ~(ALIGN - 1); }
+
+    uint64_t end = 0;
+    uint64_t bottom = 0;
+    uint64_t top = 0;
+    uint64_t clean_lo = 0;
+
+    void reset(uint64_t bytes) {
+        end = bytes & ~(ALIGN - 1);
+        bottom = top = 0;
+        clean_lo = end;
+    }
+    void begin_call() { bottom = top = 0; }
+    void forget_clean() { clean_lo = end; }
+
+    uint64_t room() const { return end - bottom - top; }
+    uint64_t used() const { return bottom + top; }
+    bool fits(uint64_t bottom_bytes, uint64_t top_bytes) const {
+        const uint64_t r = room();
+        return bottom_bytes <= r && top_bytes <= r - bottom_bytes;
+    }
+
+    bool alloc_bottom(uint64_t bytes, uint64_t *off) {
+        const uint64_t sz = round(bytes);
+        if (sz < bytes || sz > room()) return false;
+        *off = bottom;
+        bottom += sz;
+        if (bottom > clean_lo) clean_lo = bottom;
+        return true;
+    }
+    bool alloc_top(uint64_t bytes, uint64_t *off, Range *clear) {
+        const uint64_t sz = round(bytes);
+        if (sz < bytes || sz > room()) return false;
+        top += sz;
+        *off = end - top;
+        const uint64_t dirty_end = std::min(*off + sz, clean_lo);
+        *clear = dirty_end > *off ? Range{*off, dirty_end - *off} : Range{};
+        return true;
+    }
+    Range clean_part(uint64_t off, uint64_t bytes) const {
+        const uint64_t sz = round(bytes), lo = std::max(off, clean_lo);
+        return lo < off + sz ? Range{lo, off + sz - lo} : Range{};
+    }
+
+    Range top_range() const { return Range{end - top, top}; }
+    void end_call(bool zeroed) {
+        if (zeroed) clean_lo = std::min(clean_lo, end - top);
+        else clean_lo = end;
+    }
+};
+
+}
diff --git a/aligngraph2_amd/csrc/hip/walk_config.hpp b/aligngraph2_amd/csrc/hip/walk_config.hpp
--- a/aligngraph2_amd/csrc/hip/walk_config.hpp
+++ b/aligngraph2_amd/csrc/hip/walk_config.hpp
@@ -26,6 +26,9 @@
     uint32_t debug_seed_stride = 0;
     bool debug_deliver_late = false;
     uint64_t debug_emit_cap = 0;
+    bool arena_clean = false;
+    uint64_t debug_walk_arena = 0;
+    bool debug_check_arena = false;
     bool pieces = true;
     bool leap_pieces = true;
     bool force_exact = false;
@@ -67,6 +70,9 @@
         }
         u64("PAG_DEBUG_EMIT_CAP", &c.debug_emit_cap);
         c.debug_deliver_late = given("PAG_DEBUG_DELIVER_LATE");
+        if (u64("PAG_WALK_ARENA_CLEAN", &x)) c.arena_clean = x != 0;
+        u64("PAG_DEBUG_WALK_ARENA", &c.debug_walk_arena);
+        c.debug_check_arena = u64("PAG_DEBUG_CHECK_ARENA", &x) && x == 1;
         c.pieces = !off("PAG_WALK_PIECES");
         c.leap_pieces = !off("PAG_LEAP_PIECES");
         c.force_exact = given("PAG_WALK_EXACT");
diff --git a/aligngraph2_amd/csrc/hip/walk_session_jobs.hpp b/aligngraph2_amd/csrc/hip/walk_session_jobs.hpp
--- a/aligngraph2_amd/csrc/hip/walk_session_jobs.hpp
+++ b/aligngraph2_amd/csrc/hip/walk_session_jobs.hpp
@@ -122,6 +122,7 @@
     }
     int upload_contigs() {
         fill_contigs();
+        stream_work = true;
         PAG_HIP_TRY(hipMemcpyAsync(b_tc.p, tc.data(), n_sel * sizeof(TravContig), hipMemcpyHostToDevice, s));
         return PAG_OK;
     }
@@ -201,7 +202,67 @@
         std::memcpy(d, clears.data(), clears.size() * sizeof(TravClear));
         const int r = trav_clear_ranges(d, clears.size(), s);
         clears.clear();
+        stream_work = true;
         return r;
+    }
+    bool stream_work = true;
+    bool arena_begun = false;
+    uint64_t found_clean_lo = 0;
+    std::vector<TravClear> zero_checks;
+    unsigned long long *d_first_bad = nullptr;
+    uint64_t n_top_cleared = 0, n_top_checked = 0, n_slot_batches = 0, n_publish_waited = 0, n_publish_free = 0;
+    int check_clean_ranges() {
+        if (zero_checks.empty()) return PAG_OK;
+        arena::WalkArena &A = g->arena_state;
+        if (!d_first_bad) {
+            uint64_t off = 0;
+            if (!A.alloc_bottom(256, &off)) {
+                set_error("pag_travel: PAG_DEBUG_CHECK_ARENA: no room in the walk arena for the check's result");
+                return PAG_ENOMEM;
+            }
+            d_first_bad = (unsigned long long *)((char *)g->walk_arena + off);
+        }
+        TravClear *d = (TravClear *)fetch_alloc(zero_checks.size() * sizeof(TravClear));
+        unsigned long long *bad = (unsigned long long *)fetch_alloc(256);
+        if (!d || !bad) return PAG_ENOMEM;
+        std::memcpy(d, zero_checks.data(), zero_checks.size() * sizeof(TravClear));
+        PAG_HIP_TRY(hipMemsetAsync(d_first_bad, 0xFF, 8, s));
+        int r;
+        if ((r = trav_check_zero(d, zero_checks.size(), g->walk_arena, d_first_bad, s))) return r;
+        PAG_HIP_TRY(hipMemcpyAsync(bad, d_first_bad, 8, hipMemcpyDeviceToHost, s));
+        PAG_HIP_TRY(hipStreamSynchronize(s));
+        zero_checks.clear();
+        if (*bad != ~0ull) {
+            set_error("pag_travel: walk arena: non-zero byte at offset %llu, in a buffer handed out as clean (clean extent from %llu of %llu bytes)", *bad,
+                      (unsigned long long)A.clean_lo, (unsigned long long)A.end);
+            return PAG_EFAULT;
+        }
+        return PAG_OK;
+    }
+    void finish_arena() {
+        if (!arena_begun) return;
+        arena_begun = false;
+        arena::WalkArena &A = g->arena_state;
+        bool zeroed = cfg.arena_clean;
+        if (zeroed && g->walk_arena && A.top) {
+            shutdown_walker();
+            zeroed = hipStreamSynchronize(s) == hipSuccess;
+            if (zeroed && !g->clean_stream) {
+                int lo = 0, hi = 0;
+                zeroed = hipDeviceGetStreamPriorityRange(&lo, &hi) == hipSuccess && hipStreamCreateWithPriority(&g->clean_stream, hipStreamNonBlocking, lo) == hipSuccess;
+            }
+            if (zeroed && !g->clean_event) zeroed = hipEventCreateWithFlags(&g->clean_event, hipEventDisableTiming) == hipSuccess;
+            const arena::Range r = A.top_range();
+            zeroed = zeroed && trav_fill_zero((char *)g->walk_arena + r.off, r.bytes, g->clean_stream) == PAG_OK &&
+                     hipEventRecord(g->clean_event, g->clean_stream) == hipSuccess;
+            if (zeroed) {
+                g->clean_pending = true;
+            } else {
+                (void)hipGetLastError();
+                if (g->clean_stream) hipStreamSynchronize(g->clean_stream);
+            }
+        }
+        A.end_call(zeroed);
     }
     struct Deferred {
         TravPosted P;
@@ -299,27 +360,43 @@
                b_sx = cbuf(i, grp, CB_SEQX);
         int r;
         {
-            const size_t need[9] = {(size_t)o_seq[nj] * 4, (size_t)o_seq[nj] * 4, (size_t)o_seq[nj] * PG * 4, (size_t)o_seq[nj] * PG * 4,
-                                    (size_t)o_oc[nj] * 8, (size_t)o_oc[nj] * PG * 8, (size_t)o_st[nj] * 4, (size_t)o_tb[nj] * 4, (size_t)o_x[nj] * 8};
-            DevBuf *bufs[9] = {&b_sv, &b_ss, &b_av, &b_as, &b_ts, &b_ps, &b_st, &b_tb, &b_sx};
-            size_t tot = 0;
-            for (size_t q = 0; q < 9; ++q) tot += (need[q] + 16 + 255) & ~(size_t)255;
-            if (g->walk_arena && g->walk_arena_used + tot <= g->walk_arena_cap) {
-                for (size_t q = 0; q < 9; ++q) {
-                    bufs[q]->p = (char *)g->walk_arena + g->walk_arena_used;
-                    g->walk_arena_used += (need[q] + 16 + 255) & ~(size_t)255;
+            const size_t need[CB_N] = {(size_t)o_seq[nj] * 4, (size_t)o_seq[nj] * 4, (size_t)o_seq[nj] * PG * 4, (size_t)o_seq[nj] * PG * 4,
+                                       (size_t)o_oc[nj] * 8, (size_t)o_oc[nj] * PG * 8, (size_t)o_st[nj] * 4, (size_t)o_tb[nj] * 4, (size_t)o_x[nj] * 8};
+            DevBuf *bufs[CB_N] = {&b_sv, &b_ss, &b_av, &b_as, &b_ts, &b_ps, &b_st, &b_tb, &b_sx};
+            arena::WalkArena &A = g->arena_state;
+            uint64_t from_bottom = 0, from_top = 0;
+            for (size_t q = 0; q < CB_N; ++q) (q < CB_PSET ? from_bottom : from_top) += arena::WalkArena::round(need[q] + 16);
+            if (g->walk_arena && A.fits(from_bottom, from_top)) {
+                for (size_t q = 0; q < CB_N; ++q) {
+                    uint64_t off = 0;
+                    arena::Range dirty;
+                    if (!(q < CB_PSET ? A.alloc_bottom(need[q] + 16, &off) : A.alloc_top(need[q] + 16, &off, &dirty))) {
+                        set_error("pag_travel: the walk arena refused %zu bytes it had room for (%llu of %llu bytes used)", need[q] + 16, (unsigned long long)A.used(),
+                                  (unsigned long long)A.end);
+                        return PAG_EFAULT;
+                    }
+                    bufs[q]->p = (char *)g->walk_arena + off;
+                    if (q < CB_PSET) continue;
+                    want_clear((char *)g->walk_arena + dirty.off, dirty.bytes, 0u);
+                    n_top_cleared += dirty.bytes;
+                    const arena::Range kept = A.clean_part(off, need[q] + 16);
+                    if (cfg.debug_check_arena && kept.bytes) {
+                        zero_checks.push_back(TravClear{(char *)g->walk_arena + kept.off, kept.bytes, 0u, 0u});
+                        n_top_checked += kept.bytes;
+                    }
                 }
             } else {
+                ++n_slot_batches;
                 R.slot_bufs = true;
-                for (size_t q = 0; q < 9; ++q)
+                for (size_t q = 0; q < CB_N; ++q)
                     if ((r = bufs[q]->alloc(need[q]))) return r;
-            }
-        }
-        want_clear(b_sx.p, o_x[nj] * 8, 0u);
+                want_clear(b_sx.p, o_x[nj] * 8, 0u);
+                want_clear(b_ps.p, o_oc[nj] * PG * 8, 0u);
+                want_clear(b_st.p, o_st[nj] * 4, 0u);
+                want_clear(b_tb.p, o_tb[nj] * 4, 0u);
+            }
+        }
         want_clear(b_ts.p, o_oc[nj] * 8, 0xFFu);
-        want_clear(b_ps.p, o_oc[nj] * PG * 8, 0u);
-        want_clear(b_st.p, o_st[nj] * 4, 0u);
-        want_clear(b_tb.p, o_tb[nj] * 4, 0u);
         fill_contigs();
         for (size_t j = 0; j < nj; ++j) {
             const JobPlan &pl = plans[j];
@@ -361,6 +438,7 @@
                 flatten_chain(*pl.init, flat, flat + n0, nullptr);
                 PAG_HIP_TRY(hipMemcpyAsync(J.seq_v, flat, n0 * 4, hipMemcpyHostToDevice, s));
                 PAG_HIP_TRY(hipMemcpyAsync(J.seq_s, flat + n0, n0 * 4, hipMemcpyHostToDevice, s));
+                stream_work = true;
             }
             P.C = tc[i];
             if (pl.win_hi) {
@@ -399,8 +477,15 @@
         int rcl;
         if ((rcl = flush_clears())) return rcl;
         tmark("publish: clears launched");
-        PAG_HIP_TRY(hipStreamSynchronize(s));
-        tmark("publish: stream idle");
+        if ((rcl = check_clean_ranges())) return rcl;
+        if (stream_work) {
+            PAG_HIP_TRY(hipStreamSynchronize(s));
+            stream_work = false;
+            ++n_publish_waited;
+            tmark("publish: stream idle");
+        } else {
+            ++n_publish_free;
+        }
         for (uint32_t r = NR; r-- > 0;) __atomic_store_n(&hq->posted[r], n_posted[r], __ATOMIC_RELEASE);
         need_publish = false;
         const int rcw = walkers.g ? walkers.ensure(n_live) : PAG_OK;
diff --git a/aligngraph2_amd/csrc/hip/walk_session_loop.hpp b/aligngraph2_amd/csrc/hip/walk_session_loop.hpp
--- a/aligngraph2_amd/csrc/hip/walk_session_loop.hpp
+++ b/aligngraph2_amd/csrc/hip/walk_session_loop.hpp
@@ -373,12 +373,11 @@
                     bool on_dev = true;
                     for (const Chain::Part &pt : ch.parts) on_dev = on_dev && pt.dv && pt.ds;
                     const size_t cap = at0 + P.len, need = (cap * 8 + 255) & ~(size_t)255;
-                    TravConcatPart *cp = on_dev && g->walk_arena_used + need <= g->walk_arena_cap ? (TravConcatPart *)fetch_alloc(ch.parts.size() * sizeof(TravConcatPart)) : nullptr;
+                    TravConcatPart *cp = on_dev && g->arena_state.fits(need, 0) ? (TravConcatPart *)fetch_alloc(ch.parts.size() * sizeof(TravConcatPart)) : nullptr;
                     if (cp) {
                         CtgState::DevTail &T = cs.tail;
                         T.on = true;
-                        T.d_ids = (uint32_t *)((char *)g->walk_arena + g->walk_arena_used);
-                        g->walk_arena_used += need;
+                        T.d_ids = (uint32_t *)arena_scratch(need);
                         T.cap = cap;
                         T.m0 = at0;
                         T.n = P.len;
@@ -431,6 +430,7 @@
                 if (P.chosen < 0 || P.len == 0 || st[i].tail.on) continue;
                 st[i].travel[st[i].pendingFirst].step = st[i].pendingFirstStep;
             }
+            stream_work = true;
             if (used) hipMemcpyAsync(b_gather.p, hp, used * 4, hipMemcpyHostToDevice, s);
             for (uint32_t i : batch) {
                 const Pick &P = picks[i];
@@ -630,6 +630,7 @@
         pinned_parked.clear();
         t_walk = now_ms() - tw0;
         lap("walk");
+        finish_arena();
         if (wtrace) {
             uint64_t d0 = ~0ull;
             for (const TraceEv &e : trace)
@@ -651,7 +652,11 @@
         }
         if (timing || wdebug) {
             std::fprintf(stderr, "[timing] stitch: bookkeeping %.1f ms, paths %.1f ms, chains %.1f ms; posting jobs (all callers) %.1f ms; fetch memory: chunk %zu of %zu; walk arena: %.2f of %.2f GB used\n", t_st[0], t_st[1], t_st[2], t_st[3],
-                         fetch_chunk + 1, g->fetch_chunks.size(), g->walk_arena_used / 1e9, g->walk_arena_cap / 1e9);
+                         fetch_chunk + 1, g->fetch_chunks.size(), g->arena_state.used() / 1e9, g->arena_state.end / 1e9);
+            std::fprintf(stderr, "[timing] walk arena ends: %llu bytes bottom-up, %llu top-down, %llu of those cleared up front, %llu read back as clean, clean extent found from %llu of %llu; %llu batches in the slots; publishes: %llu waited for the stream, %llu did not\n",
+                         (unsigned long long)g->arena_state.bottom, (unsigned long long)g->arena_state.top, (unsigned long long)n_top_cleared, (unsigned long long)n_top_checked,
+                         (unsigned long long)found_clean_lo, (unsigned long long)g->arena_state.end, (unsigned long long)n_slot_batches, (unsigned long long)n_publish_waited,
+                         (unsigned long long)n_publish_free);
             std::fprintf(stderr, "[timing] leaping zone: %llu segment jobs, %llu adopted, refused by reason (unusable, no junction, not a boundary, cannot leap yet, window top, window bottom, contig-following record, coordinate-free record): %llu %llu %llu %llu %llu %llu %llu %llu\n",
                          (unsigned long long)n_leap_jobs, (unsigned long long)n_leap_adopted.load(), (unsigned long long)n_leap_refused[0].load(), (unsigned long long)n_leap_refused[1].load(), (unsigned long long)n_leap_refused[2].load(),
                          (unsigned long long)n_leap_refused[3].load(), (unsigned long long)n_leap_refused[4].load(), (unsigned long long)n_leap_refused[5].load(), (unsigned long long)n_leap_refused[6].load(), (unsigned long long)n_leap_refused[7].load());
@@ -764,11 +769,16 @@
         }
         return PAG_OK;
     }
-    int run() {
+    int walk() {
         int rc;
         if ((rc = begin()) || (rc = setup_contigs())) return rc;
         if (n_sel == 0) return PAG_OK;
         if ((rc = first_seeds()) || (rc = setup_rings()) || (rc = reserve_arena()) || (rc = post_first_rounds()) || (rc = event_loop())) return rc;
         return finish();
     }
+    int run() {
+        const int rc = walk();
+        finish_arena();
+        return rc;
+    }
 };
diff --git a/aligngraph2_amd/csrc/hip/walk_session_rounds.hpp b/aligngraph2_amd/csrc/hip/walk_session_rounds.hpp
--- a/aligngraph2_amd/csrc/hip/walk_session_rounds.hpp
+++ b/aligngraph2_amd/csrc/hip/walk_session_rounds.hpp
@@ -338,10 +338,9 @@
     }
     size_t render_scratch_bytes(size_t m) const { return ((render ? 1 : 0) + (render_seq ? 1 : 0)) * text_scratch_bytes(m); }
     void *arena_scratch(size_t need) {
-        if (!g->walk_arena || g->walk_arena_used + need > g->walk_arena_cap) return nullptr;
-        void *q = (char *)g->walk_arena + g->walk_arena_used;
-        g->walk_arena_used += need;
-        return q;
+        uint64_t off = 0;
+        if (!g->walk_arena || !g->arena_state.alloc_bottom(need, &off)) return nullptr;
+        return (char *)g->walk_arena + off;
     }
     template <typename Scratch>
     int render_texts(size_t slot2, const uint32_t *d_v, const uint32_t *d_s, size_t m, uint64_t bases, Scratch scratch, hipStream_t st, unsigned max_blocks) {
@@ -403,7 +402,7 @@
         if (cfg.debug_deliver_late) return PAG_OK;
         const size_t n = cs.travel.size();
         const size_t need = ((n * 8 + 255) & ~(size_t)255) + 512 + render_scratch_bytes(n);
-        if (!g->walk_arena || g->walk_arena_used + need > g->walk_arena_cap) return PAG_OK;
+        if (!g->walk_arena || !g->arena_state.fits(arena::WalkArena::round(need) + 2 * arena::WalkArena::ALIGN, 0)) return PAG_OK;
         rounds::filter_travel(cs.travel, cs.finalLeap, mapper, cs.ci, startSplit);
         const size_t m = cs.travel.size();
         const size_t slot2 = 2 * (size_t)cs.ci + (cs.forward ? 0 : 1);
@@ -419,8 +418,7 @@
             hp[x] = cs.travel[x].u;
             hp[m + x] = (uint32_t)cs.travel[x].step;
         }
-        uint32_t *d_ids = (uint32_t *)((char *)g->walk_arena + g->walk_arena_used);
-        g->walk_arena_used += (m * 8 + 255) & ~(size_t)255;
+        uint32_t *d_ids = (uint32_t *)arena_scratch(m * 8);
         if (!g->deliver_stream) PAG_HIP_TRY(hipStreamCreateWithFlags(&g->deliver_stream, hipStreamNonBlocking));
         PAG_HIP_TRY(hipMemcpyAsync(d_ids, hp, m * 8, hipMemcpyHostToDevice, g->deliver_stream));
         trav_launch_gather_path(G, d_ids, d_ids + m, m, dst, g->deliver_stream, n_live ? DELIVER_BLOCKS : 0u);
@@ -642,13 +640,17 @@
             const size_t sharers = env_device_sharers();
             if (hipMemGetInfo(&free_b, &total_b) == hipSuccess) want = std::min(want, (free_b + g->walk_arena_cap) * 2 / 5 / sharers);
             if (g->walk_arena_cap < want / 10 * 7) {
-                if (g->walk_arena) hipFree(g->walk_arena);
-                g->walk_arena = nullptr;
-                g->walk_arena_cap = 0;
-                if (hipMalloc(&g->walk_arena, want) == hipSuccess) g->walk_arena_cap = want;
-                else g->walk_arena = nullptr;
-            }
-            g->walk_arena_used = 0;
+                if (!walk_arena_acquire(g, want)) (void)hipGetLastError();
+            }
+            arena::WalkArena &A = g->arena_state;
+            const uint64_t usable = cfg.debug_walk_arena ? std::min<uint64_t>(cfg.debug_walk_arena, g->walk_arena_cap) : g->walk_arena_cap;
+            if (A.end != (usable & ~(arena::WalkArena::ALIGN - 1))) A.reset(usable);
+            A.begin_call();
+            if (!cfg.arena_clean) A.forget_clean();
+            arena_begun = true;
+            found_clean_lo = A.clean_lo;
+            if (g->clean_pending) PAG_HIP_TRY(hipStreamWaitEvent(s, g->clean_event, 0));
+            stream_work = true;
         }
         lap("arena");
         return PAG_OK;
```

Result: slower. 4.147 billion (-1.0%).
